# egpbos/barcode

Hardware: AMD Instinct MI355X
Metric: HMC leapfrog steps/sec on 256^3 grid (higher is better)
Workload: dtype f64; 1 GPU; 256^3 grid, L=200 Mpc/h, Gaussian prior, Zel'dovich + plane-parallel RSD (reference behaviour of '2LPT+RSD', SURVEY M3), likelihood=1, mass kernel mk=3 (3 = SPH), calc_h=2, mass_type=1, fp64; one trajectory of 817 leapfrog steps per chain; grid=256, chains=1, parallelism=independent chains, 1 per GPU, rehearsal_single_device=False, steps_done=817, finite=True

## Files before the change

barcode_amd/csrc/bchmc.hip:

```cpp
#include "../../include/bchmc.h"
#include "kernels.hpp"
#include "fft_host.hpp"
#include "owned.hpp"
#include "pass_launch.hpp"
#include "launch_grid.hpp"
#include "eval_plan.hpp"
#include "interp_plan.hpp"

#include <rocfft/rocfft.h>
#include <rocprofiler-sdk-roctx/roctx.h>

#include <algorithm>
#include <chrono>
#include <cmath>
#include <cfloat>
#include <cstdarg>
#include <cstdio>
#include <cstdlib>
#include <climits>
#include <cstring>
#include <mutex>
#include <string>
#include <thread>
#include <type_traits>
#include <vector>

using namespace bchmc;
using namespace owned;

namespace {

struct ProfRec {
  int cls;
  Event a, b;
};

}

struct bchmc_handle {
  bchmc_config c{};
  Geo g{};
  bool f32 = false;
  size_t esz = 8;
  int mass_fs = 0, mass_rs = 0;
  PathSwitches sw;
  bool no_tiles_low = false;
  std::string err;
  RocfftUser fft_user;
  Stream stream;

  DevBytes work;
  FftInfo info;
  FftPlan r2c1, c2r1, r2c3, c2r3;

  DevBytes in_arr[6];
  bool have[6] = {false, false, false, false, false, false};
  DevBuf<double> wS, wM;

  DevBytes qk, pk, gk;
  DevBytes qk2, pk2;
  DevBytes Ck;
  bool ck_pair = false;
  DevBytes tC;
  DevBytes psi;
  DevBytes V;
  DevBytes vrec;
  bool ck_vpair = false;
  bool vrec_eval = false;
  bool v_in_vrec = false;
  DevBytes rho, plike;
  DevBuf<long long> rho_fix;
  DevBuf<int> fix_sat;
  long long fix_sat_limit = 1ll << 62;
  bool fix = false;
  DevBytes ioq, iop;
  DevBytes gprior, glike;
  DevBytes conv;
  DevBuf<double> convF;
  DevBuf<double> dstage;
  DevBytes cq, cp;
  DevBuf<double> part6;
  bool have_cq = false, have_cp = false, have_prop = false;
  DevBytes cg;
  bool cg_valid = false, prop_g_valid = false;
  double c_like = 0., prop_like = 0.;
  DevBuf<double> rho_part, partA;
  DevBuf<double> guard;
  DevBuf<int> stop;
  DevBuf<unsigned long long> steps_done;
  PinnedBuf<double> h_part;
  struct MtDraw {
    long long S = 0, C = 0, G = 0;
    int B = 0;
    DevBuf<uint32_t> poly, win, words, st;
    DevBuf<unsigned long long> nz, nzoff, acc, accoff, lastend;
    DevBuf<unsigned long long> res;
    PinnedBuf<unsigned long long> h_io;
    DevBuf<double> gauss;
    double setup_ms = 0.;
  } mt;
  struct Mock {
    DevBuf<unsigned long long> cnt, off, gsum, goff, res;
  } mock;
  DevBuf<double> spec_bins;
  DevBytes cross_ak;
  struct Ens {
    struct Slot {
      uint64_t count = 0;
      DevBuf<double> mean, m2;
    } slot[BCHMC_ENS_SLOTS];
    int ncu = 0;
  } ens;
  struct Tweb {
    DevBytes t[6];
    DevBytes xk;
    DevBuf<unsigned char> type;
    DevBuf<double> lam;
    DevBuf<unsigned long long> part;
    DevBuf<unsigned int> cnt;
    bool have_t = false;
    uint64_t samples = 0;
    bool have_par = false;
    double R = 0., lambda_th = 0.;
  } tw;
  struct Bispec {
    DevBytes d[kBispecMaxShell];
    DevBytes xk;
    DevBuf<double> part;
    DevBuf<double> tab;
    bool have_tab = false;
    double k_min = 0., dk = 0.;
    int n_shell = 0;
  } bs;
  struct Corr1 {
    uint64_t n_bin = 0;
    DevBuf<unsigned long long> acc;
    std::vector<double> rmode;
    std::vector<uint64_t> nmode;
  } corr1;
  struct Corr2 {
    uint64_t n_bin = 0;
    int n = 0;
    double l_max = 0.;
    DevBuf<int> idx;
    DevBuf<int2> slices;
    DevBuf<double> part;
    DevBuf<double> out;
    int nrows = 0, nsl = 0, npb = 0, max_rows = 0;
    std::vector<uint64_t> row_cnt, par_cnt;
    std::vector<int> par_bin;
    std::vector<double> rsum;
  } corr2;
  struct Spec2 {
    uint64_t n_bin = 0;
    DevBuf<int> idx;
    DevBuf<int2> slices;
    DevBuf<double> part;
    DevBuf<double> out;
    int nsl = 0, npb = 0;
    std::vector<uint64_t> row_cnt, par_w;
    std::vector<int> par_bin;
    std::vector<double> ksum;
  } spec2;
  struct Mp {
    DevBuf<int> rows;
    DevBuf<int4> cls;
    DevBuf<double> part;
    DevBuf<double> out;
    DevBytes xk;
    int ncls = 0;
    struct Geom {
      uint64_t n_bin = 0;
      std::vector<double> tmode, leg;
      std::vector<uint64_t> nmode;
    } fourier, real;
  } mp;
  struct Upres {
    int n_out = 0;
    Geo g{};
    DevBytes real, half;
    DevBytes work;
    FftInfo info;
    FftPlan r2c, c2r;
    DevBuf<int> cell;
    DevBuf<double> dx;
    Corr2 bins;
  } up;
  struct Cat {
    DevBuf<double> cols;
    DevBuf<int> tile_of;
    DevBuf<CatRec> rec;
    DevBuf<unsigned> cnt, off, cursor;
    DevBuf<CatItem> items;
    DevBuf<unsigned long long> stat;
    PinnedBuf<unsigned long long> h_stat;
  } cat;
  struct Pois {
    DevBuf<unsigned long long> off;
    DevBuf<unsigned long long> cnt, boff, gsum, goff;
    DevBuf<unsigned long long> res, stat;
    DevBuf<double> cols;
    long long cells = 0;
    bool valid = false;
    uint64_t seed = 0, n_part = 0;
    uint32_t stream = 0, n_in = 0;
    double d_in = 0.;
  } pois;
  struct Itp {
    DevBytes src;
    int fields_held = 0;
    DevBuf<double> cols;
    DevBuf<double> out;
    DevBuf<int> tile_of;
// ... 273 lines not shown
  h->sorted_valid = false;
}

int realloc_slots(bchmc_handle *h, long long want) {
  HIPCHK(hipStreamSynchronize(h->stream));
  SlotPolicy &sl = h->plan.slots;
  const bool verbose = env_on("BCHMC_VERBOSE");
  const long long cap = sl.clamp_to_budget(want);
  if (!cap) {
    if (verbose) fprintf(stderr, "bchmc: record slots stay at %lld per tile (memory budget %lld): overflowing evaluations "
                                 "run the two-pass sort\n", sl.cap_alloc, sl.cap_budget);
    sl.after_realloc(SlotGot::kOldSize, cap);
    return BCHMC_OK;
  }
  (void)h->srec.release();
  h->sorted_valid = false;
  for (SlotGot got : {SlotGot::kWanted, SlotGot::kOldSize, SlotGot::kRecordsOnly}) {
    const size_t nrec = record_count(h->g.N, sl.rung(got, cap), h->plan.tp.ntiles);
    if (h->srec.alloc(nrec * 4 * h->esz) == hipSuccess) {
      if (got == SlotGot::kWanted) {
        if (verbose) fprintf(stderr, "bchmc: record array reallocated for %lld slots per tile\n", cap);
      } else {
        if (verbose) fprintf(stderr, "bchmc: no memory for %lld record slots per tile: %s\n", cap,
                             got == SlotGot::kOldSize ? "kept the old size, overflowing steps run the two-pass sort"
                                                      : "one-pass binning given up");
      }
      sl.after_realloc(got, cap);
      return BCHMC_OK;
    }
    (void)hipGetLastError();
  }
  return h->fail(BCHMC_ERR_NOMEM, "no device memory for the particle records");
}

int adapt_slots(bchmc_handle *h, int sticky, int maxc, bool may_realloc) {
  if (!h->plan.tiled) return BCHMC_OK;
  SlotPolicy &sl = h->plan.slots;
  const int old = sl.cap;
  const SlotAction a = sl.observe(sticky, maxc, may_realloc);
  if (a.kind == SlotAction::kRealloc) CHK(realloc_slots(h, a.cap));
  if (sl.cap == old) return BCHMC_OK;
  if (env_on("BCHMC_VERBOSE"))
    fprintf(stderr, "bchmc: record slots per tile %d -> %lld (largest (tile, octant) population %d%s)\n", old,
            (long long)sl.cap, maxc, a.overflowed ? ", a segment overflowed" : "");
  repartition(h);
  return BCHMC_OK;
}

int read_ctl(bchmc_handle *h, unsigned long long *steps_done) {
  unsigned long long sd = 0;
  int words[2] = {0, 0}, sat = 0;
  const bool slots = h->plan.tiled && h->plan.slots.sort_direct;
  if (steps_done) HIPCHK(hipMemcpyAsync(&sd, h->steps_done, sizeof sd, hipMemcpyDeviceToHost, h->stream));
  if (h->fix_sat) HIPCHK(hipMemcpyAsync(&sat, h->fix_sat, sizeof(int), hipMemcpyDeviceToHost, h->stream));
  if (slots) HIPCHK(hipMemcpyAsync(words, slot_words(h), sizeof words, hipMemcpyDeviceToHost, h->stream));
  HIPCHK(hipStreamSynchronize(h->stream));
  if (steps_done) *steps_done = sd;
  if (slots) {
    if (words[0] || words[1]) HIPCHK(hipMemsetAsync(slot_words(h), 0, sizeof words, h->stream));
    if (const long long want = h->plan.slots.pending()) {
      CHK(realloc_slots(h, want));
      repartition(h);
    }
    CHK(adapt_slots(h, words[0], words[1], true));
  }
  if (sat) {
    HIPCHK(hipMemsetAsync(h->fix_sat, 0, sizeof(int), h->stream));
    return h->fail(BCHMC_ERR_STATE,
                   "deterministic mode: a density cell exceeded the fixed-point range (more than 2^16 maximal "
                   "contributions in one cell); the results since the last read-back are not valid");
  }
  return BCHMC_OK;
}

constexpr uint64_t kSlotPoll = 4;
int poll_slots(bchmc_handle *h, uint64_t k) {
  if (!h->h_slots) {
    HIPCHK(h->h_slots.alloc(4));
    for (Event &e : h->slot_ev) HIPCHK(e.create(hipEventDisableTiming));
  }
  if (k >= 2) {
    const int b = (int)((k - 1) & 1);
    HIPCHK(hipEventSynchronize(h->slot_ev[b]));
    CHK(adapt_slots(h, h->h_slots[2 * b], h->h_slots[2 * b + 1], false));
  }
  const int b = (int)(k & 1);
  HIPCHK(hipMemcpyAsync(h->h_slots + 2 * b, slot_words(h), 2 * sizeof(int), hipMemcpyDeviceToHost, h->stream));
  HIPCHK(hipMemsetAsync(slot_words(h), 0, 2 * sizeof(int), h->stream));
  HIPCHK(hipEventRecord(h->slot_ev[b], h->stream));
  return BCHMC_OK;
}

int make_plans_2d(bchmc_handle *h, size_t batch, FftPlan &r2c, FftPlan &c2r) {
  const Geo &g = h->g;
  const rocfft_precision prec = h->f32 ? rocfft_precision_single : rocfft_precision_double;
  const size_t len2[2] = {(size_t)g.n, (size_t)g.n};
  const size_t rs2[2] = {1, (size_t)g.n}, cs2[2] = {1, (size_t)g.nhp};
  rocfft_plan_description f2 = nullptr, i2 = nullptr;
  bool ok2 = rocfft_plan_description_create(&f2) == rocfft_status_success &&
             rocfft_plan_description_create(&i2) == rocfft_status_success;
  ok2 = ok2 && rocfft_plan_description_set_data_layout(f2, rocfft_array_type_real, rocfft_array_type_hermitian_interleaved,
                                                       nullptr, nullptr, 2, rs2, (size_t)g.n * g.n, 2, cs2,
                                                       (size_t)g.n * g.nhp) == rocfft_status_success;
  ok2 = ok2 && rocfft_plan_description_set_data_layout(i2, rocfft_array_type_hermitian_interleaved, rocfft_array_type_real,
                                                       nullptr, nullptr, 2, cs2, (size_t)g.n * g.nhp, 2, rs2,
                                                       (size_t)g.n * g.n) == rocfft_status_success;
  ok2 = ok2 && r2c.create(rocfft_plan_create, rocfft_placement_notinplace, rocfft_transform_type_real_forward, prec, 2,
                          len2, batch, f2) == rocfft_status_success;
  ok2 = ok2 && c2r.create(rocfft_plan_create, rocfft_placement_notinplace, rocfft_transform_type_real_inverse, prec, 2,
                          len2, batch, i2) == rocfft_status_success;
  if (f2) rocfft_plan_description_destroy(f2);
  if (i2) rocfft_plan_description_destroy(i2);
  if (ok2 && h->info) {
    size_t need = 0;
    for (const FftPlan *p : {&r2c, &c2r}) {
      size_t wb = 0;
      if (rocfft_plan_get_work_buffer_size(*p, &wb) != rocfft_status_success) ok2 = false;
      need = std::max(need, wb);
    }
    if (ok2 && need > h->work.capacity()) {
      DevBytes nw;
      (void)hipStreamSynchronize(h->stream);
      if (nw.alloc(need) == hipSuccess &&
          rocfft_execution_info_set_work_buffer(h->info, nw, need) == rocfft_status_success) {
        h->work = std::move(nw);
      } else {
        (void)hipGetLastError();
        ok2 = false;
      }
    }
  }
  if (!ok2) {
    r2c.reset();
    c2r.reset();
    return BCHMC_ERR_ROCFFT;
  }
  return BCHMC_OK;
}

PathSwitches read_path_switches() {
  PathSwitches s;
  s.no_planes = env_on("BCHMC_NO_PLANES");
  s.no_planes_ends = env_on("BCHMC_NO_PLANES_ENDS");
  s.no_fuse = env_on("BCHMC_NO_FUSE");
  s.no_alpt_planes = env_on("BCHMC_NO_ALPT_PLANES");
  s.no_zbin = env_on("BCHMC_NO_ZBIN");
  s.zbin_128 = env_on("BCHMC_ZBIN_128");
  s.yfwd_f64 = env_on("BCHMC_YFWD_F64");
  s.bx_v1 = env_on("BCHMC_BX_V1");
  s.bx_v2 = env_on("BCHMC_BX_V2");
  s.no_pair = env_on("BCHMC_NO_PAIR");
  s.no_vpair = env_on("BCHMC_NO_VPAIR");
  s.no_vrec = env_on("BCHMC_NO_VREC");
  return s;
}

PathFacts path_facts(bchmc_handle *h, int rsd) {
  PathFacts f;
  f.n = h->g.n, f.esz = (int)h->esz, f.Nhp = h->g.Nhp;
  f.planes_ok = h->planes_ok && h->xtw;
  f.tiled = h->plan.tiled, f.sort_direct = h->plan.slots.sort_direct, f.std81 = h->plan.std81;
  f.mk = h->c.mk, f.calc_h = h->c.calc_h, f.likelihood = h->c.likelihood, f.sfmodel = h->c.sfmodel;
  f.rsd_model = h->c.rsd_model, f.mass_rs = h->mass_rs != 0;
  if (alpt_planes_wanted(f, h->sw, rsd) && !h->c2r2d_2 && !h->alpt_plans_failed &&
      make_plans_2d(h, 2 * (size_t)h->g.n, h->r2c2d_2, h->c2r2d_2) != BCHMC_OK)
    h->alpt_plans_failed = true;
  f.alpt_plans = h->c2r2d_2 != nullptr;
  return f;
}

int host_sum(bchmc_handle *h, const double *d_part, double *out) {
  HIPCHK(hipMemcpyAsync(h->h_part, d_part, kRedBlocks * sizeof(double), hipMemcpyDeviceToHost, h->stream));
  HIPCHK(hipStreamSynchronize(h->stream));
  double s = 0.;
  for (int i = 0; i < kRedBlocks; i++) s += h->h_part[i];
  *out = s;
  return BCHMC_OK;
}

void par_memcpy(void *dst, const void *src, size_t bytes, int nt) {
  if (nt <= 1 || bytes < ((size_t)4 << 20)) {
    std::memcpy(dst, src, bytes);
    return;
  }
  std::vector<std::thread> th;
  const size_t per = ((bytes / (size_t)nt) + 4095) & ~(size_t)4095;
  for (int t = 1; t < nt; t++) {
    const size_t off = per * (size_t)t;
    if (off >= bytes) break;
    const size_t len = std::min(per, bytes - off);
    th.emplace_back([=] { std::memcpy((char *)dst + off, (const char *)src + off, len); });
  }
  std::memcpy(dst, src, std::min(per, bytes));
  for (auto &t : th) t.join();
}

int stg_init(bchmc_handle *h) {
  if (h->stg[0]) return BCHMC_OK;
  size_t chunk = (size_t)16 << 20;
  if (const char *ev = std::getenv("BCHMC_STAGE_MB")) chunk = (size_t)std::max(1, atoi(ev)) << 20;
  int nt = (int)std::min(8u, std::max(1u, std::thread::hardware_concurrency() / 2));
  if (const char *ev = std::getenv("BCHMC_STAGE_THREADS")) nt = std::max(1, atoi(ev));
  for (int b = 0; b < 2; b++) {
    HIPCHK(h->stg[b].alloc(chunk));
    HIPCHK(h->stg_ev[b].create(hipEventDisableTiming));
  }
  h->stg_chunk = chunk;
  h->stg_threads = nt;
  return BCHMC_OK;
}

int h2d(bchmc_handle *h, void *dst, const void *src, size_t bytes, hipStream_t stream = nullptr) {
  if (!stream) stream = h->stream;
  if (bytes <= ((size_t)1 << 20)) {
    HIPCHK(hipMemcpyAsync(dst, src, bytes, hipMemcpyHostToDevice, stream));
    HIPCHK(hipStreamSynchronize(stream));
    return BCHMC_OK;
  }
  CHK(stg_init(h));
  const size_t chunk = h->stg_chunk;
  const size_t nch = (bytes + chunk - 1) / chunk;
  for (size_t c = 0; c < nch; c++) {
    const int b = (int)(c & 1);
    const size_t off = c * chunk, len = std::min(chunk, bytes - off);
    if (c >= 2) HIPCHK(hipEventSynchronize(h->stg_ev[b]));
    par_memcpy(h->stg[b], (const char *)src + off, len, h->stg_threads);
    HIPCHK(hipMemcpyAsync((char *)dst + off, h->stg[b], len, hipMemcpyHostToDevice, stream));
    HIPCHK(hipEventRecord(h->stg_ev[b], stream));
  }
  HIPCHK(hipEventSynchronize(h->stg_ev[0]));
  if (nch > 1) HIPCHK(hipEventSynchronize(h->stg_ev[1]));
  return BCHMC_OK;
}

int d2h(bchmc_handle *h, void *dst, const void *src, size_t bytes, hipStream_t stream = nullptr,
        hipEvent_t after = nullptr) {
  if (!stream) stream = h->stream;
  if (after) HIPCHK(hipStreamWaitEvent(stream, after, 0));
  if (bytes <= ((size_t)1 << 20)) {
    HIPCHK(hipMemcpyAsync(dst, src, bytes, hipMemcpyDeviceToHost, stream));
    HIPCHK(hipStreamSynchronize(stream));
    return BCHMC_OK;
  }
  CHK(stg_init(h));
  const size_t chunk = h->stg_chunk;
  const size_t nch = (bytes + chunk - 1) / chunk;
  for (size_t c = 0; c <= nch; c++) {
    const int b = (int)(c & 1);
    if (c < nch) {
      const size_t off = c * chunk, len = std::min(chunk, bytes - off);
      HIPCHK(hipMemcpyAsync(h->stg[b], (const char *)src + off, len, hipMemcpyDeviceToHost, stream));
      HIPCHK(hipEventRecord(h->stg_ev[b], stream));
    }
    if (c >= 1) {
      const size_t off = (c - 1) * chunk, len = std::min(chunk, bytes - off);
      HIPCHK(hipEventSynchronize(h->stg_ev[b ^ 1]));
      par_memcpy((char *)dst + off, h->stg[b ^ 1], len, h->stg_threads);
    }
  }
  return BCHMC_OK;
}

int build_conv_table(bchmc_handle *h) {
  const Geo &g = h->g;
  const double hh = h->c.particle_kernel_h;
  const double norm = (24. / (hh * hh * hh)) * (h->c.rho_c * g.L * g.L * g.L / (double)((size_t)g.n * g.n * g.n));
  std::vector<double> F((size_t)g.Nhp);
  auto kv = [&](int i) { return (i <= g.n / 2) ? g.kfac * (double)i : -g.kfac * (double)(g.n - i); };
  for (int i = 0; i < g.n; ++i) {
    const double kx = kv(i);
    for (int j = 0; j < g.n; ++j) {
      const double ky = kv(j);
      for (int k = 0; k < g.nh; ++k) {
        const double kz = kv(k);
        const double k_sq = kx * kx + ky * ky + kz * kz;
        double f;
        if (k_sq == 0.) {
          f = 1. / (hh * hh * hh);
        } else {
          const double kk = std::sqrt(k_sq);
          const double ksink = kk * std::sin(kk);
          f = norm * (3 + std::cos(2 * kk) - ksink + std::cos(kk) * (ksink - 4)) / (k_sq * k_sq * k_sq);
        }
        F[k + (size_t)g.nhp * (j + (size_t)g.n * i)] = f;
      }
    }
  }
  CHK(dev_alloc(h, h->convF, (size_t)g.Nhp));
  HIPCHK(hipMemcpyAsync(h->convF, F.data(), F.size() * sizeof(double), hipMemcpyHostToDevice, h->stream));
  HIPCHK(hipStreamSynchronize(h->stream));
  return BCHMC_OK;
}

double spectrum_dk(const Geo &g, uint64_t n_bin) {
  const double knyq = g.kfac * (double)(g.n / 2);
  const double kmax = std::sqrt(knyq * knyq + knyq * knyq + knyq * knyq);
  return kmax / (double)n_bin;
}

int spectrum_bins(bchmc_handle *h, const void *xk, uint64_t n_bin, double *kmode, double *power) {
  CHK(dev_reserve(h, h->spec_bins, 3 * (size_t)n_bin));
  double *bins = h->spec_bins;
  HIPCHK(hipMemsetAsync(bins, 0, 3 * (size_t)n_bin * sizeof(double), h->stream));
  const Geo &g = h->g;
  const double dk = spectrum_dk(g, n_bin);
  const int grid = std::min(nblk_stride(g.Nhp), 512);
  if (h->f32)
    k_spectrum<float><<<grid, 256, 3 * n_bin * sizeof(double), h->stream>>>(
        g, reinterpret_cast<const float2 *>(xk), (int)n_bin, dk, bins);
  else
    k_spectrum<double><<<grid, 256, 3 * n_bin * sizeof(double), h->stream>>>(
        g, reinterpret_cast<const double2 *>(xk), (int)n_bin, dk, bins);
  std::vector<double> hb(3 * n_bin);
  hipError_t e = hipGetLastError();
  if (e == hipSuccess) e = hipMemcpyAsync(hb.data(), bins, hb.size() * sizeof(double), hipMemcpyDeviceToHost, h->stream);
  if (e == hipSuccess) e = hipStreamSynchronize(h->stream);
// ... 706 lines not shown
      }
      if (h->c.likelihood == 1) {
        CHK(ensure_conv(h));
        CHK(fft_exec(h, h->r2c1, h->ioq, h->tC, BCHMC_K_FFT_R2C));
        {
          ProfScope ps(h, BCHMC_K_OTHER);
          k_gradfft_mult<T><<<nblk_stride(Nh), 256, 0, h->stream>>>(h->g, C(h->tC), C(h->Ck), 1. / (double)N);
          HIPCHK(hipGetLastError());
        }
        CHK(fft_exec(h, h->c2r3, h->Ck, h->conv, BCHMC_K_FFT_C2R));
        ProfScope ps(h, BCHMC_K_OTHER);
        k_mul3<T><<<nblk_stride(N), 256, 0, h->stream>>>(N, R(h->plike), R(h->conv), R(h->V));
        HIPCHK(hipGetLastError());
      } else {
        ProfScope ps(h, BCHMC_K_OTHER);
        k_findif_mul<T><<<nblk_stride(N), 256, 0, h->stream>>>(h->g, make_like(h), R(h->ioq), R(h->plike), R(h->V));
        HIPCHK(hipGetLastError());
      }
      if (transform) CHK(fft_exec(h, h->r2c3, h->V, h->Ck, BCHMC_K_FFT_R2C));
      *like_mode = 0;
      return BCHMC_OK;
    }
    if (h->c.calc_h == 3) {
      if (h->last_rsd && !h->c.planepar)
        return h->fail(BCHMC_ERR_RSD_NOT_PLANEPAR, "non-plane-parallel RSD is not implemented in calc_V");
      CHK(ensure_conv(h));
      if (!h->convF) CHK(build_conv_table(h));
      CHK(fft_exec(h, h->r2c1, h->plike, h->tC, BCHMC_K_FFT_R2C));
      const double hh = h->c.particle_kernel_h;
      {
        ProfScope ps(h, BCHMC_K_OTHER);
        k_conv_kernel<T><<<nblk_stride(Nh), 256, 0, h->stream>>>(h->g, C(h->tC), h->convF, C(h->Ck), hh, 1. / (double)N);
        HIPCHK(hipGetLastError());
      }
      CHK(fft_exec(h, h->c2r3, h->Ck, h->conv, BCHMC_K_FFT_C2R));
      {
        ProfScope ps(h, BCHMC_K_GATHER);
        if (h->plan.tiled && h->sorted_valid && !h->no_tiles_low) {
          const int grid = tile_grid(h);
          const size_t lds = 3 * (size_t)(h->plan.tp.tx + 2) * (h->plan.tp.ty + 2) * (h->plan.tp.tz + 2) * sizeof(T);
          k_interp_tsc_tile<T><<<grid, 256, lds, h->stream>>>(h->g, h->plan.tp, h->last_rsd, fgrow1(h->c.ascale, h->c.OM, h->c.OL),
                                                              recs(h), h->t_off, h->t_end, h->t_woff,
                                                              h->t_oct, h->t_seg, R(h->conv), R(h->V));
        } else {
          k_interp_tsc<T><<<nblk_full(N), 256, 0, h->stream>>>(h->g, make_pos(h, h->last_rsd),
                                                               fgrow1(h->c.ascale, h->c.OM, h->c.OL), R(h->psi),
                                                               R(h->conv), R(h->V));
        }
        HIPCHK(hipGetLastError());
      }
    } else {
      ProfScope ps(h, BCHMC_K_GATHER);
      HullPar hp = make_hull(h);
      if (h->plan.tiled && h->sorted_valid) {
        const int grid = tile_grid(h);
        if (h->plan.std81 && vrec) {
          k_gather_tile81<T, 12, 20, true><<<grid, kTile81Threads, tile_lds(h, 0, sizeof(T)), h->stream>>>(
              h->g, hp, h->plan.tp, h->last_rsd, recs(h), h->t_off, h->t_end, h->t_woff,
              h->t_oct, h->t_seg, R(h->plike), R(h->vrec));
          h->v_in_vrec = true;
        } else if (h->plan.std81)
          k_gather_tile81<T, 12, 20><<<grid, kTile81Threads, tile_lds(h, 0, sizeof(T)), h->stream>>>(
              h->g, hp, h->plan.tp, h->last_rsd, recs(h), h->t_off, h->t_end, h->t_woff,
              h->t_oct, h->t_seg, R(h->plike), R(h->V));
        else
          k_gather_tile<T><<<grid, 256, tile_lds(h, hp.ncol, sizeof(T)), h->stream>>>(
              h->g, hp, h->plan.tp, h->last_rsd, recs(h), h->t_off, h->t_end, h->t_woff,
              h->t_oct, h->t_seg, R(h->plike), R(h->V));
      } else {
        k_gather_sph<T><<<nblk_full(N), 256, hp.ncol * sizeof(int4), h->stream>>>(h->g, make_pos(h, h->last_rsd), hp,
                                                                                  R(h->psi), R(h->plike), R(h->V));
      }
      HIPCHK(hipGetLastError());
      if (vrec && !h->v_in_vrec) return h->fail(BCHMC_ERR_STATE, "V records were zeroed and no gather writes records");
    }
    const bool vpair = eval_vpair(path_facts(h, h->c.rsd_model), h->sw, m);
    if (transform && h->v_in_vrec && !vpair)
      return h->fail(BCHMC_ERR_STATE, "V was gathered as records, and a transform that reads three arrays");
    if (!transform) {
    } else if (vpair) {
      ProfScope ps(h, BCHMC_K_FFT_R2C);
      if (h->v_in_vrec) HIPCHK((launch_zr2c<T, true>(pass_ctx(h), R(h->vrec), C(h->Ck))));
      else HIPCHK(launch_zr2c<T>(pass_ctx(h), R(h->V), C(h->Ck)));
      HIPCHK(launch_ypass_fwd_pair<T>(pass_ctx(h), C(h->Ck)));
      h->ck_vpair = true;
    } else if (eval_yfwd(path_facts(h, h->c.rsd_model), h->sw, m)) {
      ProfScope ps(h, BCHMC_K_FFT_R2C);
      HIPCHK(launch_zr2c<T>(pass_ctx(h), R(h->V), C(h->Ck)));
      HIPCHK((launch_ypass<T, false>(pass_ctx(h), C(h->Ck))));
    } else {
      CHK(fft_exec(h, m.planes_r2c ? h->r2c2d : h->r2c3, h->V, h->Ck, BCHMC_K_FFT_R2C));
    }
    *like_mode = 0;
    return BCHMC_OK;
  }

  static int grf_force(bchmc_handle *h) {
    {
      ProfScope ps(h, BCHMC_K_OTHER);
      k_scale_c<T><<<nblk_stride(h->g.Nhp), 256, 0, h->stream>>>(h->g.Nhp, C(h->qk), C(h->tC), 1. / (double)h->g.N);
      HIPCHK(hipGetLastError());
    }
    CHK(fft_exec(h, h->c2r1, h->tC, h->plike, BCHMC_K_FFT_C2R));
    {
      ProfScope ps(h, BCHMC_K_OTHER);
      k_grf_grad<T><<<nblk_stride(h->g.N), 256, 0, h->stream>>>(h->g.N, R(h->plike), R(h->in_arr[BCHMC_F_NOBS]),
                                                                R(h->in_arr[BCHMC_F_NOISE]),
                                                                R(h->in_arr[BCHMC_F_WINDOW]), R(h->rho));
      HIPCHK(hipGetLastError());
    }
    CHK(fft_exec(h, h->r2c1, h->rho, h->Ck, BCHMC_K_FFT_R2C));
    h->have_eval = false;
    return BCHMC_OK;
  }

  static int force_sources(bchmc_handle *h, bool pre_za, EvalMode m, int *like_mode, double *b) {
    if (h->c.likelihood == 3) {
      CHK(grf_force(h));
      *like_mode = 1;
      *b = h->c.grad_psi_likeli_factor;
      return BCHMC_OK;
    }
    if (!pre_za) {
      CHK(displacement(h, h->c.deltaQ_factor, h->c.rsd_model, &m.planes_c2r));
    } else if (m.alpt_pending) {
      CHK(alpt_middle(h, true));
      m.planes_c2r = true;
    }
    CHK(forward_rest(h, h->c.rsd_model, m));
    CHK(like_force(h, m, like_mode));
    double norm = -1.;
    norm *= h->c.deltaQ_factor;
    if (h->c.correct_delta) norm *= h->c.D1;
    *b = h->c.grad_psi_likeli_factor * norm;
    return BCHMC_OK;
  }

  template <bool KICK>
  static int launch_assemble(bchmc_handle *h, double a, double b, int like_mode, double c_kick, double *guard_slot) {
    h->prop_g_valid = false;
    if (h->ck_vpair) return h->fail(BCHMC_ERR_STATE, "two arrays of V^ in Ck, and a kernel that reads three");
    ProfScope ps(h, BCHMC_K_KSPACE_FORCE_KICK);
    k_assemble<T, KICK><<<nblk_stride(h->g.Nhp), 256, 0, h->stream>>>(h->g, C(h->Ck), C(h->qk), h->wS, C(h->gk), C(h->pk),
                                                                     a, b, like_mode, c_kick, guard_slot, h->stop);
    HIPCHK(hipGetLastError());
    return BCHMC_OK;
  }

  static int r2c_state(bchmc_handle *h, const double *d_real, void *staging, void *out) {
    CHK(load_real(h, d_real, R(staging)));
    return fft_exec(h, h->r2c1, staging, out, BCHMC_K_FFT_R2C);
  }

  static int c2r_scaled(bchmc_handle *h, const void *xk, void *out_T) {
    {
      ProfScope ps(h, BCHMC_K_OTHER);
      k_scale_c<T><<<nblk_stride(h->g.Nhp), 256, 0, h->stream>>>(h->g.Nhp, reinterpret_cast<const CT *>(xk), C(h->tC),
                                                                1. / (double)h->g.N);
      HIPCHK(hipGetLastError());
    }
    return fft_exec(h, h->c2r1, h->tC, out_T, BCHMC_K_FFT_C2R);
  }

  static int c2r_state(bchmc_handle *h, const void *xk, void *scratch_T, double *d_out) {
    if (kDouble) return c2r_scaled(h, xk, d_out);
    CHK(c2r_scaled(h, xk, scratch_T));
    return store_real(h, R(scratch_T), d_out);
  }

  static int mass_rs_term(bchmc_handle *h) {
    CHK(c2r_scaled(h, h->pk, h->iop));
    {
      ProfScope ps(h, BCHMC_K_OTHER);
      k_div_mass_r<T><<<nblk_stride(h->g.N), 256, 0, h->stream>>>(h->g.N, R(h->iop), R(h->in_arr[BCHMC_F_MASS_R]),
                                                                  R(h->iop));
      HIPCHK(hipGetLastError());
    }
    return fft_exec(h, h->r2c1, h->iop, h->tC, BCHMC_K_FFT_R2C);
  }

  struct Tap {
    double *like_i, *like_f;
  };

  static int tap_loglike(bchmc_handle *h, double *partials) {
    k_loglike<T><<<kRedBlocks, 256, 0, h->stream>>>(h->g, make_like(h), R(h->rho), h->rho_part,
                                                    R(h->in_arr[BCHMC_F_NOBS]), R(h->in_arr[BCHMC_F_NOISE]),
                                                    R(h->in_arr[BCHMC_F_WINDOW]), partials);
    HIPCHK(hipGetLastError());
    return BCHMC_OK;
  }

  struct Traj {
    PathFacts f;
    TrajPlan p;
    double a, c_za;
    bool pair;
  };
  static Traj traj(bchmc_handle *h) {
    Traj t;
    t.f = path_facts(h, h->c.rsd_model);
    t.p = traj_plan(t.f, h->sw);
    t.a = h->c.grad_psi_prior_factor;
    t.c_za = (t.p.c_za == CZa::kAlptInput ? 1. : -h->c.D1) * h->c.deltaQ_factor / (double)h->g.N;
    t.pair = psi_pair(t.f, h->sw, t.p);
    return t;
  }

  template <int MODE, bool ALPT = false>
  static int launch_boundary_x(bchmc_handle *h, BoundaryX<T> bx) {
    if (MODE != BX_FIRST) {
      if (ALPT && h->ck_vpair) return h->fail(BCHMC_ERR_STATE, "two arrays of V^ in Ck, and a boundary that reads three");
      bx.vpair = h->ck_vpair;
      h->ck_vpair = false;
    }
    HIPCHK((launch_step_boundary_x<T, MODE, ALPT>(pass_ctx(h), C(h->Ck), h->wS, bx)));
    h->ck_pair = bx.pair && !ALPT && MODE != BX_LAST;
    return BCHMC_OK;
  }

  static int initial_force(bchmc_handle *h, const Traj &t, double *like_i, void *g0_out) {
    int like_mode = 2;
    double b = 0.;
    const InitialEval kind = initial_eval(t.f, h->sw, t.p);
    if (kind == InitialEval::k3d) {
      CHK(force_sources(h, false, EvalMode{}, &like_mode, &b));
      if (like_i) CHK(tap_loglike(h, like_i));
      CHK(launch_assemble<false>(h, t.a, b, like_mode, 0., nullptr));
    } else {
      StepCtl nc{h->stop, h->steps_done, nullptr, 0., 0};
      {
        ProfScope ps(h, BCHMC_K_KSPACE_DRIFT_ZA);
        BoundaryX<T> bx;
        bx.qi = C(h->qk), bx.c_za = t.c_za, bx.ctl = nc, bx.pair = t.pair;
        if (kind == InitialEval::kBxFirstAlpt) CHK((launch_boundary_x<BX_FIRST, true>(h, bx)));
        else CHK(launch_boundary_x<BX_FIRST>(h, bx));
      }
      EvalMode m;
      m.planes_c2r = m.planes_r2c = true;
      m.alpt_pending = t.p.alpt_x;
      CHK(force_sources(h, true, m, &like_mode, &b));
      if (like_mode != 0) return h->fail(BCHMC_ERR_STATE, "planes mode without the three V components");
      if (like_i) CHK(tap_loglike(h, like_i));
      h->prop_g_valid = false;
      ProfScope ps(h, BCHMC_K_KSPACE_FORCE_KICK);
      BoundaryX<T> bx;
      bx.qi = C(h->qk), bx.a = t.a, bx.b = b, bx.ctl = nc, bx.g_out = C(h->gk);
      CHK(launch_boundary_x<BX_LAST>(h, bx));
    }
    if (g0_out)
      HIPCHK(hipMemcpyAsync(g0_out, h->gk, 2 * (size_t)h->g.Nhp * sizeof(T), hipMemcpyDeviceToDevice, h->stream));
    return BCHMC_OK;
  }

  static int trajectory(bchmc_handle *h, double eps, uint64_t neps, const Tap *tap, const void *g0_in = nullptr,
                        void *g0_out = nullptr) {
    h->prop_g_valid = false;
    if (neps + 1 > h->guard.capacity())
      CHK(dev_reserve(h, h->guard, std::max<size_t>(4096, 2 * (neps + 1))));
    HIPCHK(hipMemsetAsync(h->guard, 0, (neps + 1) * sizeof(double), h->stream));
    k_init_ctl<<<1, 1, 0, h->stream>>>(h->stop, h->steps_done, (unsigned long long)neps);
    HIPCHK(hipGetLastError());

    const Traj t = traj(h);
    int like_mode = 2;
    double b = 0.;
    if (!g0_in) CHK(initial_force(h, t, tap ? tap->like_i : nullptr, g0_out));
    const void *g_first = g0_in ? g0_in : h->gk;
    if (neps == 0) return BCHMC_OK;

    if (t.p.fused) return trajectory_fused(h, eps, neps, tap, t, g_first);
    const double *wM = h->mass_fs ? h->wM : nullptr;
    const double guard_limit = 1e50 * (double)h->g.N;
    for (uint64_t s = 0; s < neps; s++) {
      StepCtl ctl{h->stop, h->steps_done, s > 0 ? h->guard + (s - 1) : nullptr, guard_limit, s};
      if (!h->mass_rs) {
        ProfScope ps(h, BCHMC_K_KSPACE_DRIFT_ZA);
        k_kick_drift_za<T, true><<<nblk_stride(h->g.Nhp), 256, 0, h->stream>>>(
            h->g, C(h->qk), C(h->pk), C(s == 0 ? g_first : h->gk), wM, nullptr, C(h->Ck), 0.5 * eps, eps, t.c_za, ctl);
        HIPCHK(hipGetLastError());
      } else {
        {
          ProfScope ps(h, BCHMC_K_KSPACE_DRIFT_ZA);
          k_kick_drift_za<T, true><<<nblk_stride(h->g.Nhp), 256, 0, h->stream>>>(
              h->g, C(h->qk), C(h->pk), C(s == 0 ? g_first : h->gk), nullptr, nullptr, C(h->Ck), 0.5 * eps, 0., t.c_za,
              ctl);
          HIPCHK(hipGetLastError());
        }
        CHK(mass_rs_term(h));
        StepCtl ctl2{h->stop, h->steps_done, nullptr, 0., s};
        ProfScope ps(h, BCHMC_K_KSPACE_DRIFT_ZA);
        k_kick_drift_za<T, true><<<nblk_stride(h->g.Nhp), 256, 0, h->stream>>>(h->g, C(h->qk), C(h->pk), C(h->gk), wM,
                                                                             C(h->tC), C(h->Ck), 0., eps, t.c_za, ctl2);
        HIPCHK(hipGetLastError());
      }
      CHK(force_sources(h, t.p.fused_za, EvalMode{}, &like_mode, &b));
      if (tap && tap->like_f && s + 1 == neps) CHK(tap_loglike(h, tap->like_f));
      CHK(launch_assemble<true>(h, t.a, b, like_mode, 0.5 * eps, h->guard + s));
    }
    return BCHMC_OK;
  }

  static int trajectory_fused(bchmc_handle *h, double eps, uint64_t neps, const Tap *tap, const Traj &t,
                              const void *g_first) {
    const double *wM = h->mass_fs ? h->wM : nullptr;
    const double guard_limit = 1e50 * (double)h->g.N, a = t.a, c_za = t.c_za;
    if (!h->qk2) {
      CHK(dev_alloc(h, h->qk2, 2 * (size_t)h->g.Nhp * sizeof(T)));
      CHK(dev_alloc(h, h->pk2, 2 * (size_t)h->g.Nhp * sizeof(T)));
    }
    void *const q0 = h->qk, *const p0 = h->pk, *const q1 = h->qk2, *const p1 = h->pk2;
    int like_mode = 2;
    double b = 0.;
    int cur = 0;
    {
      StepCtl ctl{h->stop, h->steps_done, nullptr, guard_limit, 0};
      ProfScope ps(h, BCHMC_K_KSPACE_DRIFT_ZA);
      BoundaryX<T> bx;
      bx.qi = bx.qo = C(q0), bx.pi = bx.po = C(p0), bx.wM = wM, bx.half_eps = 0.5 * eps, bx.eps = eps, bx.c_za = c_za;
      bx.ctl = ctl, bx.g_in = C(g_first), bx.pair = t.pair;
      switch (opening(t.f, h->sw, t.p)) {
        case Opening::kBxFirstAlpt: CHK((launch_boundary_x<BX_FIRST, true>(h, bx))); break;
        case Opening::kBxFirst: CHK(launch_boundary_x<BX_FIRST>(h, bx)); break;
        case Opening::kKickDriftZa:
          h->ck_pair = false;
          k_kick_drift_za<T, true><<<nblk_stride(h->g.Nhp), 256, 0, h->stream>>>(h->g, C(q0), C(p0), C(g_first), wM,
                                                                               nullptr, C(h->Ck), 0.5 * eps, eps, c_za, ctl);
          break;
      }
      HIPCHK(hipGetLastError());
    }
    for (uint64_t s = 0; s < neps; s++) {
      const bool last = (s + 1 == neps);
      if (last && h->early_q_dev && h->ev_q) {
        CHK(c2r_state(h, cur ? q1 : q0, h->ioq, h->early_q_dev));
        HIPCHK(hipEventRecord(h->ev_q, h->stream));
        h->early_q_done = true;
      }
      if (h->plan.slots.slot_watch && h->plan.tiled && h->plan.slots.sort_direct && s > 0 && s % kSlotPoll == 0)
        CHK(poll_slots(h, s / kSlotPoll));
      CHK(force_sources(h, true, step_mode(t.f, h->sw, t.p, s, neps), &like_mode, &b));
      if (tap && tap->like_f && last) CHK(tap_loglike(h, tap->like_f));
      StepCtl ctl{h->stop, h->steps_done, s > 0 ? h->guard + (s - 1) : nullptr, guard_limit, s};
      void *qi = cur ? q1 : q0, *pi = cur ? p1 : p0, *qo = cur ? q0 : q1, *po = cur ? p0 : p1;
      ProfScope ps(h, BCHMC_K_KSPACE_FORCE_KICK);
      BoundaryX<T> bx;
      bx.qi = C(qi), bx.pi = C(pi), bx.qo = C(qo), bx.po = C(po), bx.wM = wM, bx.a = a, bx.b = b, bx.half_eps = 0.5 * eps;
      bx.eps = eps, bx.c_za = c_za, bx.guard_slot = h->guard + s, bx.ctl = ctl, bx.pair = t.pair;
      switch (closing(t.f, h->sw, t.p, s, neps, like_mode)) {
        case Closing::kBxLast:
          bx.qo = nullptr, bx.po = C(pi), bx.g_out = C(h->gk);
          CHK(launch_boundary_x<BX_LAST>(h, bx));
          break;
        case Closing::kStepBoundaryLast:
          if (h->ck_vpair) return h->fail(BCHMC_ERR_STATE, "two arrays of V^ in Ck, and a boundary that reads three");
          k_step_boundary<T, true><<<nblk_stride(h->g.Nhp), 256, 0, h->stream>>>(
              h->g, C(h->Ck), C(qi), C(pi), C(qi), C(pi), C(h->gk), h->wS, wM, a, b, like_mode, 0.5 * eps, eps, c_za,
              h->guard + s, ctl);
          break;
        case Closing::kBxInteriorAlpt: CHK((launch_boundary_x<BX_INTERIOR, true>(h, bx))); break;
        case Closing::kBxInterior: CHK(launch_boundary_x<BX_INTERIOR>(h, bx)); break;
        case Closing::kBxInteriorTwoTile:
          bx.vpair = h->ck_vpair;
          h->ck_vpair = false;
          HIPCHK(launch_step_boundary_x2<T>(pass_ctx(h), C(h->Ck), h->wS, bx));
          h->ck_pair = bx.pair;
          break;
        case Closing::kStepBoundary:
          if (h->ck_vpair) return h->fail(BCHMC_ERR_STATE, "two arrays of V^ in Ck, and a boundary that reads three");
          k_step_boundary<T, false><<<nblk_stride(h->g.Nhp), 256, 0, h->stream>>>(
              h->g, C(h->Ck), C(qi), C(pi), C(qo), C(po), C(h->gk), h->wS, wM, a, b, like_mode, 0.5 * eps, eps, c_za,
              h->guard + s, ctl);
          break;
      }
      if (buffers_flip(s, neps)) cur ^= 1;
      HIPCHK(hipGetLastError());
    }
    {
      ProfScope ps(h, BCHMC_K_OTHER);
      k_rollback<T><<<nblk_stride(h->g.Nhp), 256, 0, h->stream>>>(h->g.Nhp, h->stop, h->steps_done, C(q0), C(p0), C(q1),
                                                                 C(p1), C(cur ? q1 : q0), C(cur ? p1 : p0));
      HIPCHK(hipGetLastError());
    }
    if (cur) {
      std::swap(h->qk, h->qk2);
      std::swap(h->pk, h->pk2);
    }
    return BCHMC_OK;
  }

  static int leapfrog_core(bchmc_handle *h, const double *d_q0, const double *d_p0, double *d_q1, double *d_p1,
                           double eps, uint64_t neps, bool prologue_done = false) {
    CHK(check_inputs(h));
    if (eps > 2.) eps = 2.;
    if (!prologue_done) CHK(r2c_state(h, d_q0, h->ioq, h->qk));
    CHK(r2c_state(h, d_p0, h->iop, h->pk));
    CHK(trajectory(h, eps, neps, nullptr, prologue_done ? h->gk : nullptr));
    if (!h->early_q_done) CHK(c2r_state(h, h->qk, h->ioq, d_q1));
    CHK(c2r_state(h, h->pk, h->iop, d_p1));
    return BCHMC_OK;
  }
  static int requeue_q(bchmc_handle *h, double *d_q1) { return c2r_state(h, h->qk, h->ioq, d_q1); }

  static int chain_alloc(bchmc_handle *h) {
    if (!h->cq) {
      CHK(dev_alloc(h, h->cq, 2 * (size_t)h->g.Nhp * sizeof(T)));
      CHK(dev_alloc(h, h->cp, 2 * (size_t)h->g.Nhp * sizeof(T)));
      CHK(dev_alloc(h, h->part6, (size_t)6 * kRedBlocks));
    }
    return BCHMC_OK;
  }

  static int chain_draw(bchmc_handle *h, uint64_t seed, uint64_t attempt) {
    const long long N = h->g.N, Nh = h->g.Nhp;
    const uint2 key = make_uint2((unsigned)seed, (unsigned)(seed >> 32));
    ProfScope ps(h, BCHMC_K_OTHER);
    if (h->mass_fs) {
      k_white_noise<T><<<nblk_stride((N + 1) / 2), 256, 0, h->stream>>>(N, key, (unsigned)attempt, 0u, nullptr, R(h->iop));
      HIPCHK(hipGetLastError());
      CHK(fft_exec(h, h->r2c1, h->iop, h->tC, BCHMC_K_FFT_R2C));
      k_color_momenta<T><<<nblk_stride(Nh), 256, 0, h->stream>>>(Nh, C(h->tC), h->wM, C(h->cp), 0);
      HIPCHK(hipGetLastError());
    } else {
      HIPCHK(hipMemsetAsync(h->cp, 0, 2 * (size_t)Nh * sizeof(T), h->stream));
    }
    if (h->mass_rs) {
      k_white_noise<T><<<nblk_stride((N + 1) / 2), 256, 0, h->stream>>>(N, key, (unsigned)attempt, 1u,
                                                                        R(h->in_arr[BCHMC_F_MASS_R]), R(h->iop));
      HIPCHK(hipGetLastError());
      CHK(fft_exec(h, h->r2c1, h->iop, h->tC, BCHMC_K_FFT_R2C));
      k_color_momenta<T><<<nblk_stride(Nh), 256, 0, h->stream>>>(Nh, C(h->tC), nullptr, C(h->cp), 1);
      HIPCHK(hipGetLastError());
    }
    return BCHMC_OK;
  }

  static bool attempt_is_fast(const bchmc_handle *h, uint64_t neps) {
    const bool like_shared = h->c.likelihood == 1 || ((h->c.likelihood == 0 || h->c.likelihood == 2) &&
                                                       h->c.deltaQ_factor == 1. && !h->c.rsd_model);
    return like_shared && !h->mass_rs && neps >= 1;
  }

  static int attempt_core(bchmc_handle *h, double eps, uint64_t neps, const double *d_q0, const double *d_p0,
                          const void *src_qk, const void *src_pk, double terms[6], uint64_t *steps_done,
                          const void *g0_in = nullptr, double like0 = 0., void *g0_out = nullptr, bool g0_ready = false,
                          double *host_q1 = nullptr) {
    CHK(check_inputs(h));
    if (eps > 2.) eps = 2.;
    const size_t cbytes = 2 * (size_t)h->g.Nhp * sizeof(T);
    const double N = (double)h->g.N;
    const bool fast = attempt_is_fast(h, neps);
    if (!h->part6) CHK(dev_alloc(h, h->part6, (size_t)6 * kRedBlocks));
    double *P = h->part6;
    if (!fast) {
      CHK(energies_core(h, d_q0, d_p0, terms));
      if (src_qk) {
        HIPCHK(hipMemcpyAsync(h->qk, src_qk, cbytes, hipMemcpyDeviceToDevice, h->stream));
        HIPCHK(hipMemcpyAsync(h->pk, src_pk, cbytes, hipMemcpyDeviceToDevice, h->stream));
      }
    } else {
      k_parseval<T><<<kRedBlocks, 256, 0, h->stream>>>(h->g, C(h->pk), h->wM, P);
      k_parseval<T><<<kRedBlocks, 256, 0, h->stream>>>(h->g, C(h->qk), h->wS, P + kRedBlocks);
      HIPCHK(hipGetLastError());
    }
    if (g0_ready && fast) g0_in = h->gk;
    Tap tap{g0_in ? nullptr : P + 2 * kRedBlocks, P + 5 * kRedBlocks};
    if (g0_in && !g0_ready) HIPCHK(hipMemsetAsync(P + 2 * kRedBlocks, 0, kRedBlocks * sizeof(double), h->stream));
    CHK(trajectory(h, eps, neps, fast ? &tap : nullptr, fast ? g0_in : nullptr, fast ? g0_out : nullptr));
    uint64_t done = 0;
    if (fast) {
      k_parseval<T><<<kRedBlocks, 256, 0, h->stream>>>(h->g, C(h->pk), h->wM, P + 3 * kRedBlocks);
      k_parseval<T><<<kRedBlocks, 256, 0, h->stream>>>(h->g, C(h->qk), h->wS, P + 4 * kRedBlocks);
      HIPCHK(hipGetLastError());
      if (host_q1) {
        if (!h->early_q_done) CHK(c2r_state(h, h->qk, h->ioq, h->dstage));
        CHK(c2r_state(h, h->pk, h->iop, h->dstage + h->g.N));
      }
      if (host_q1 && h->early_q_done)
        CHK(d2h(h, host_q1, h->dstage, (size_t)h->g.N * sizeof(double), h->copy_stream, h->ev_q));
      std::vector<double> hp(6 * kRedBlocks);
      unsigned long long sd = 0;
      HIPCHK(hipMemcpyAsync(hp.data(), P, hp.size() * sizeof(double), hipMemcpyDeviceToHost, h->stream));
      CHK(read_ctl(h, &sd));
      done = sd;
      for (int t = 0; t < 6; t++) {
        double s = 0.;
        for (int i = 0; i < kRedBlocks; i++) s += hp[(size_t)t * kRedBlocks + i];
        terms[t] = (t == 0 || t == 1 || t == 3 || t == 4) ? s / (2. * N) : s;
      }
      if (g0_in && !g0_ready) terms[2] = like0;
      if (done < neps) {
        if (host_q1 && h->early_q_done) {
          h->early_q_done = false;
          CHK(c2r_state(h, h->qk, h->ioq, h->dstage));
        }
        EvalMode m;
        CHK(displacement(h, h->c.likelihood == 1 ? h->c.deltaQ_factor : 1., h->c.likelihood == 1 ? h->c.rsd_model : 0,
                         &m.planes_c2r));
        CHK(forward_rest(h, h->c.likelihood == 1 ? h->c.rsd_model : 0, m));
        CHK(tap_loglike(h, P));
        CHK(host_sum(h, P, &terms[5]));
      }
    } else {
      unsigned long long sd = 0;
      CHK(read_ctl(h, &sd));
      done = sd;
      CHK(c2r_state(h, h->qk, h->ioq, h->dstage));
      CHK(c2r_state(h, h->pk, h->iop, h->dstage + h->g.N));
      CHK(energies_core(h, h->dstage, h->dstage + h->g.N, terms + 3));
    }
    if (steps_done) *steps_done = done;
    return BCHMC_OK;
  }

  static int chain_attempt(bchmc_handle *h, double eps, uint64_t neps, double terms[6], uint64_t *steps_done) {
    const size_t cbytes = 2 * (size_t)h->g.Nhp * sizeof(T);
    if (attempt_is_fast(h, neps)) {
      HIPCHK(hipMemcpyAsync(h->qk, h->cq, cbytes, hipMemcpyDeviceToDevice, h->stream));
      HIPCHK(hipMemcpyAsync(h->pk, h->cp, cbytes, hipMemcpyDeviceToDevice, h->stream));
      const bool use = !env_on("BCHMC_NO_FORCE_CARRY"), carry = use && h->cg_valid;
      if (use && !h->cg) CHK(dev_alloc(h, h->cg, cbytes));
      uint64_t done = 0;
      CHK(attempt_core(h, eps, neps, nullptr, nullptr, nullptr, nullptr, terms, &done, carry ? h->cg : nullptr,
                       h->c_like, (use && !carry) ? h->cg : nullptr));
      if (steps_done) *steps_done = done;
      if (use && !carry) {
        h->cg_valid = true;
        h->c_like = terms[2];
      }
      h->prop_g_valid = use && done == neps;
      h->prop_like = terms[5];
    } else {
      h->cg_valid = h->prop_g_valid = false;
      CHK(c2r_state(h, h->cq, h->ioq, h->dstage));
      CHK(c2r_state(h, h->cp, h->iop, h->dstage + h->g.N));
      CHK(attempt_core(h, eps, neps, h->dstage, h->dstage + h->g.N, h->cq, h->cp, terms, steps_done));
    }
    h->have_prop = true;
    return BCHMC_OK;
  }
// ... 528 lines not shown
      HIPCHK(hipMemcpyAsync(hs, w.out, cells * 3 * NS * sizeof(double), hipMemcpyDeviceToHost, h->stream));
    }
    HIPCHK(hipStreamSynchronize(h->stream));
    return BCHMC_OK;
  }
  static int mp_auto(bchmc_handle *h, const void *xk, uint64_t n_bin, double *hg, double *hs) {
    return mp_sums<1, false>(h, xk, nullptr, n_bin, hg, hs);
  }
  static int mp_cross(bchmc_handle *h, const void *ak, const void *bk, uint64_t n_bin, double *hg, double *hs) {
    return mp_sums<3, false>(h, ak, bk, n_bin, hg, hs);
  }
  static int mp_corr(bchmc_handle *h, uint64_t n_bin, double *hg, double *hs) {
    return mp_sums<1, true>(h, h->ioq, nullptr, n_bin, hg, hs);
  }

  static int gradient(bchmc_handle *h, const double *d_q, double *d_g) {
    const size_t N = (size_t)h->g.N;
    if (!h->gprior) {
      CHK(dev_alloc(h, h->gprior, N * sizeof(T)));
      CHK(dev_alloc(h, h->glike, N * sizeof(T)));
    }
    CHK(r2c_state(h, d_q, h->ioq, h->qk));
    int like_mode = 2;
    double b = 0.;
    CHK(force_sources(h, false, EvalMode{}, &like_mode, &b));
    CHK(launch_assemble<false>(h, h->c.grad_psi_prior_factor, 0., 2, 0., nullptr));
    CHK(c2r_scaled(h, h->gk, h->gprior));
    CHK(launch_assemble<false>(h, 0., b, like_mode, 0., nullptr));
    CHK(c2r_scaled(h, h->gk, h->glike));
    k_add_r<T><<<nblk_stride(h->g.N), 256, 0, h->stream>>>(h->g.N, R(h->gprior), R(h->glike), R(h->iop));
    HIPCHK(hipGetLastError());
    return store_real(h, R(h->iop), d_g);
  }

  static int fetch(bchmc_handle *h, bchmc_field field, double *d_out) {
    FieldSource fs;
    CHK(field_source(h, (int)field, &fs));
    if (fs.made == FieldSource::kOverdens)
      k_overdens<T><<<nblk_stride(h->g.N), 256, 0, h->stream>>>(h->g, R(h->rho), h->rho_part, R(h->ioq));
    if (fs.made == FieldSource::kPositions)
      k_positions<T><<<nblk_stride(h->g.N), 256, 0, h->stream>>>(h->g, make_pos(h, h->last_rsd), R(h->psi), R(h->ioq),
                                                                 (int)field - (int)BCHMC_F_POSX);
    if (fs.made == FieldSource::kVrec)
      k_vrec_unpack<T><<<nblk_stride(h->g.N), 256, 0, h->stream>>>(h->g.N, R(h->vrec), (int)field - (int)BCHMC_F_VX, R(h->ioq));
    if (fs.made != FieldSource::kAsHeld) HIPCHK(hipGetLastError());
    return store_real(h, R(fs.base) + fs.offset, d_out);
  }

  static int mt_place(bchmc_handle *h) {
    const long long N = h->g.N, Nh = h->g.Nhp;
    const int n = h->g.n;
    ProfScope ps(h, BCHMC_K_OTHER);
    HIPCHK(hipMemsetAsync(h->cp, 0, 2 * (size_t)Nh * sizeof(T), h->stream));
    if (h->mass_fs) {
      const long long cells = (long long)(n / 2 + 1) * (n / 2 + 1) * (n / 2 + 1);
      const double amp = (double)N * (double)N / (h->g.L * h->g.L * h->g.L);
      k_mt_place<T><<<nblk_stride(cells), 256, 0, h->stream>>>(n, h->g.nhp, h->mt.gauss, R(h->in_arr[BCHMC_F_MASS_F]),
                                                               amp, C(h->cp));
      HIPCHK(hipGetLastError());
    }
    if (h->mass_rs) {
      k_mt_real_space<T><<<nblk_stride(N), 256, 0, h->stream>>>(N, h->mt.gauss + (h->mass_fs ? 2 * N : 0),
                                                                R(h->in_arr[BCHMC_F_MASS_R]), R(h->iop));
      HIPCHK(hipGetLastError());
      CHK(fft_exec(h, h->r2c1, h->iop, h->tC, BCHMC_K_FFT_R2C));
      k_color_momenta<T><<<nblk_stride(Nh), 256, 0, h->stream>>>(Nh, C(h->tC), nullptr, C(h->cp), 1);
      HIPCHK(hipGetLastError());
    }
    return BCHMC_OK;
  }

  static int mock_place(bchmc_handle *h, void *dst) {
    const long long N = h->g.N;
    const int n = h->g.n;
    ProfScope ps(h, BCHMC_K_OTHER);
    HIPCHK(hipMemsetAsync(dst, 0, 2 * (size_t)h->g.Nhp * sizeof(T), h->stream));
    const long long cells = (long long)(n / 2 + 1) * (n / 2 + 1) * (n / 2 + 1);
    const double amp = (double)N * (double)N / (h->g.L * h->g.L * h->g.L);
    k_mt_place<T><<<nblk_stride(cells), 256, 0, h->stream>>>(n, h->g.nhp, h->mt.gauss, R(h->in_arr[BCHMC_F_SIGNAL_PS]),
                                                             amp, C(dst));
    HIPCHK(hipGetLastError());
    return BCHMC_OK;
  }

  static long long mock_tiles(const bchmc_handle *h) { return (h->g.N + kMockTile - 1) / kMockTile; }
  static long long mock_groups(const bchmc_handle *h) { return (mock_tiles(h) + kMtThreads - 1) / kMtThreads; }

  static int mock_alloc(bchmc_handle *h) {
    auto &k = h->mock;
    if (k.cnt) return BCHMC_OK;
    CHK(dev_alloc(h, k.cnt, (size_t)mock_tiles(h)));
    CHK(dev_alloc(h, k.off, (size_t)mock_tiles(h)));
    CHK(dev_alloc(h, k.gsum, (size_t)mock_groups(h)));
    CHK(dev_alloc(h, k.goff, (size_t)mock_groups(h)));
    CHK(dev_alloc(h, k.res, (size_t)2));
    return BCHMC_OK;
  }

  static int mock_window(bchmc_handle *h, int rsd, int window_type) {
    const long long N = h->g.N;
    auto &k = h->mock;
    CHK(c2r_state(h, h->qk, h->ioq, h->dstage));
    EvalMode m;
    CHK(displacement(h, 1., rsd, &m.planes_c2r));
    CHK(forward_rest(h, rsd, m));
    CHK(fetch(h, BCHMC_F_DELTAX, h->dstage + N));
    ProfScope ps(h, BCHMC_K_OTHER);
    HIPCHK(hipMemsetAsync(k.res, 0xff, 2 * sizeof(unsigned long long), h->stream));
    k_mock_window<T><<<(int)mock_tiles(h), kMockThreads, 0, h->stream>>>(N, window_type, h->dstage + N,
                                                                         R(h->in_arr[BCHMC_F_WINDOW]), k.cnt);
    k_mock_scan<<<(int)mock_groups(h), kMtThreads, 0, h->stream>>>(k.cnt, mock_tiles(h), k.off, k.gsum);
    k_mt_scan<<<1, kMtThreads, 0, h->stream>>>(k.gsum, (int)mock_groups(h), k.goff, k.res, 0, nullptr);
    HIPCHK(hipGetLastError());
    return BCHMC_OK;
  }

  static int mock_noise(bchmc_handle *h, const MockPar &mp) {
    const long long N = h->g.N;
    auto &k = h->mock;
    ProfScope ps(h, BCHMC_K_OTHER);
    k_mock_noise<T><<<(int)mock_tiles(h), kMockThreads, 0, h->stream>>>(
        N, mp, h->dstage, h->dstage + N, R(h->in_arr[BCHMC_F_WINDOW]), k.off, k.goff,
        reinterpret_cast<const double2 *>(h->mt.gauss.get()), R(h->in_arr[BCHMC_F_NOBS]), R(h->in_arr[BCHMC_F_NOISE]), k.res);
    HIPCHK(hipGetLastError());
    return BCHMC_OK;
  }

  static int mock_smooth(bchmc_handle *h, double smol) {
    double wtot = 0.;
    CHK(kernel_norm(h, smol, h->ioq, &wtot));
    ProfScope ps(h, BCHMC_K_OTHER);
    k_mock_smooth<T><<<nblk_stride(h->g.Nhp), 256, 0, h->stream>>>(h->g, C(h->cq), smol, 1. / wtot);
    HIPCHK(hipGetLastError());
    return BCHMC_OK;
  }

  static int mock_guess_noise(bchmc_handle *h, double sigma) {
    {
      ProfScope ps(h, BCHMC_K_OTHER);
      k_mock_guess_noise<<<nblk_stride(h->g.N), kMockThreads, 0, h->stream>>>(
          h->g.N, sigma, reinterpret_cast<const double2 *>(h->mt.gauss.get()), h->dstage);
      HIPCHK(hipGetLastError());
    }
    return r2c_state(h, h->dstage, h->ioq, h->cq);
  }

  static int upload(bchmc_handle *h, bchmc_field field, const double *d_src) {
    CHK(load_real(h, d_src, R(h->in_arr[field])));
    const double normFS = h->g.L * h->g.L * h->g.L / (double)h->g.N;
    if (field == BCHMC_F_SIGNAL_PS || field == BCHMC_F_MASS_F) {
      double *w = field == BCHMC_F_SIGNAL_PS ? h->wS : h->wM;
      k_prepare_mult<<<nblk_stride(h->g.Nhp), 256, 0, h->stream>>>(h->g, d_src, w, normFS);
      HIPCHK(hipGetLastError());
    }
    return BCHMC_OK;
  }

  static int mass_force_spectrum(bchmc_handle *h, uint64_t n_bin, double *kmode, double *power) {
    int like_mode = 2;
    double b = 0.;
    CHK(force_sources(h, false, EvalMode{}, &like_mode, &b));
    double norm = -1.;
    norm *= h->c.deltaQ_factor;
    if (h->c.correct_delta) norm *= h->c.D1;
    CHK(launch_assemble<false>(h, 0., norm, like_mode, 0., nullptr));
    return spectrum_bins(h, h->gk, n_bin, kmode, power);
  }

  static constexpr long long kJascheWork = 1ll << 32;

  static int mass_jasche(bchmc_handle *h, double *d_r) {
    const Geo &g = h->g;
    const long long N = g.N;
    DevBuf<double> G, acc;
    DevBuf<int> cnt, off;
    DevBuf<long long> total;
    DevBuf<JRec> rec;
    struct Drain {
      hipStream_t stream;
      ~Drain() { (void)hipStreamSynchronize(stream); }
    } drain{h->stream};
    CHK(dev_alloc(h, G, 3 * (size_t)N));
    CHK(dev_alloc(h, acc, (size_t)N));
    CHK(dev_alloc(h, cnt, (size_t)N));
    CHK(dev_alloc(h, off, (size_t)N + 1));
    CHK(dev_alloc(h, total, (size_t)1));
    {
      ProfScope ps(h, BCHMC_K_OTHER);
      k_glap_impulse<T><<<nblk_stride(g.Nhp), 256, 0, h->stream>>>(g, C(h->Ck));
      HIPCHK(hipGetLastError());
    }
    CHK(fft_exec(h, h->c2r3, h->Ck, h->psi, BCHMC_K_FFT_C2R));
    {
      ProfScope ps(h, BCHMC_K_OTHER);
      k_convert<T, double><<<nblk_stride(3 * N), 256, 0, h->stream>>>(3 * N, R(h->psi), G);
      HIPCHK(hipGetLastError());
    }
    const int rsd = h->c.rsd_model;
    EvalMode mode;
    CHK(displacement(h, 1., rsd, &mode.planes_c2r));
    CHK(forward_rest(h, rsd, mode));
    const PosPar pp = make_pos(h, rsd);
    JaschePar jp;
    jp.h = h->c.particle_kernel_h;
    const double h2 = jp.h * jp.h;
    jp.norm = 1. / (M_PI * (h2 * h2 * jp.h));
    jp.reach = (int)(2. * jp.h / g.d) + 1;
    const T *window = R(h->in_arr[BCHMC_F_WINDOW]), *noise = R(h->in_arr[BCHMC_F_NOISE]);
    {
      ProfScope ps(h, BCHMC_K_OTHER);
      k_jasche_pairs<T, false><<<nblk_stride(N), 256, 0, h->stream>>>(g, pp, jp, R(h->psi), window, cnt, nullptr, nullptr);
      k_jasche_scan<<<1, 1024, 0, h->stream>>>(N, cnt, total, off);
      HIPCHK(hipGetLastError());
    }
    long long npairs = 0;
    HIPCHK(hipMemcpyAsync(&npairs, total, sizeof npairs, hipMemcpyDeviceToHost, h->stream));
    HIPCHK(hipStreamSynchronize(h->stream));
    if (npairs >= 0x7fffffffLL)
      return h->fail(BCHMC_ERR_UNSUPPORTED, "Jasche mass: %lld (particle, cell) pairs exceed the 32-bit offsets", npairs);
    CHK(dev_alloc(h, rec, (size_t)std::max(npairs, 1ll)));
    HIPCHK(hipMemsetAsync(cnt, 0, (size_t)N * sizeof(int), h->stream));
    {
      ProfScope ps(h, BCHMC_K_OTHER);
      k_jasche_pairs<T, true><<<nblk_stride(N), 256, 0, h->stream>>>(g, pp, jp, R(h->psi), window, cnt, off, rec);
      k_jasche_sort<<<nblk_stride(N), 256, 0, h->stream>>>(N, off, rec);
      HIPCHK(hipGetLastError());
    }
    std::vector<int> hoff((size_t)N + 1);
    HIPCHK(hipMemcpyAsync(hoff.data(), off, hoff.size() * sizeof(int), hipMemcpyDeviceToHost, h->stream));
    HIPCHK(hipStreamSynchronize(h->stream));
    const long long budget = std::max(kJascheWork / N, 1ll);
    for (long long l0 = 0; l0 < N;) {
      long long l1 = l0 + 1;
      while (l1 < N && (long long)(hoff[l1 + 1] - hoff[l0]) + (l1 + 1 - l0) <= budget) l1++;
      ProfScope ps(h, BCHMC_K_OTHER);
      k_jasche_accum<<<nblk_full(N), 256, 0, h->stream>>>(g, rec, off, l0, l1, G, acc);
      HIPCHK(hipGetLastError());
      l0 = l1;
    }
    const double m = h->c.rho_c * (g.L * g.L * g.L) / (double)N;
    ProfScope ps(h, BCHMC_K_OTHER);
    k_jasche_final<T><<<nblk_stride(N), 256, 0, h->stream>>>(N, acc, window, noise, m * m, d_r);
    HIPCHK(hipGetLastError());
    return BCHMC_OK;
  }

  static int mass_build(bchmc_handle *h, bool from_chain, const bchmc_mass_opts &o, bool force, bool jasche) {
    const int t = h->c.mass_type;
    const long long N = h->g.N;
    double *d_f = h->dstage, *d_r = h->dstage + N;
    if (force || jasche) {
      if (from_chain)
        HIPCHK(hipMemcpyAsync(h->qk, h->cq, 2 * (size_t)h->g.Nhp * sizeof(T), hipMemcpyDeviceToDevice, h->stream));
      else
        CHK(r2c_state(h, h->dstage, h->ioq, h->qk));
    }
    double dk = 0., fbar = 0.;
    std::vector<double> kmode, power;
    if (force) {
      kmode.resize(o.n_bin);
      power.resize(o.n_bin);
      CHK(mass_force_spectrum(h, o.n_bin, kmode.data(), power.data()));
      dk = spectrum_dk(h->g, o.n_bin);
      if (t == 3) {
        double fm = 0., kv = 0.;
        for (uint64_t i = 0; i < o.n_bin; i++) fm += 4. * M_PI * kmode[i] * kmode[i] * dk * power[i];
        for (uint64_t i = 0; i < o.n_bin; i++) kv += 4. * M_PI * kmode[i] * kmode[i] * dk;
        fbar = fm / kv;
      } else {
        HIPCHK(hipMemcpyAsync(h->spec_bins, power.data(), o.n_bin * sizeof(double), hipMemcpyHostToDevice, h->stream));
      }
    }
    if (h->mass_fs) {
      const int mode = (t == 1 || t == 5) ? MASS_INVP : t == 2 ? MASS_FORCE : t == 3 ? MASS_MEAN : MASS_PS;
      ProfScope ps(h, BCHMC_K_OTHER);
      k_mass_elementwise<T><<<nblk_stride(N), 256, 0, h->stream>>>(h->g, mode, R(h->in_arr[BCHMC_F_SIGNAL_PS]),
                                                                   h->spec_bins, (int)o.n_bin, dk, fbar, o.mass_factor,
                                                                   d_f);
      HIPCHK(hipGetLastError());
    }
    if (h->mass_rs) {
      if (jasche) {
        CHK(mass_jasche(h, d_r));
      } else {
        ProfScope ps(h, BCHMC_K_OTHER);
        k_mass_elementwise<T><<<nblk_stride(N), 256, 0, h->stream>>>(h->g, MASS_ONE, nullptr, nullptr, 0, 0., 0., 1., d_r);
        HIPCHK(hipGetLastError());
      }
    }
    if (h->mass_fs) CHK(upload(h, BCHMC_F_MASS_F, d_f));
    if (h->mass_rs) CHK(upload(h, BCHMC_F_MASS_R, d_r));
    HIPCHK(hipStreamSynchronize(h->stream));
    return BCHMC_OK;
  }

  static int pois_counts(bchmc_handle *h, int src, long long cells, const double *xd, const bchmc_poisson_opts &o,
                         double *cd, bool resident) {
    auto &k = h->pois;
    if (!xd) CHK(upres_real(h, src));
    const long long nb = (cells + kPoisThreads - 1) / kPoisThreads, ng = (nb + kMtThreads - 1) / kMtThreads;
    const uint2 key = make_uint2((unsigned)o.seed, (unsigned)(o.seed >> 32));
    const T *win = o.use_window ? R(h->in_arr[BCHMC_F_WINDOW]) : nullptr;
    unsigned long long *off = resident ? k.off.get() : nullptr, *cnt = resident ? k.cnt.get() : nullptr;
    ProfScope ps(h, BCHMC_K_OTHER);
    HIPCHK(hipMemsetAsync(k.stat, 0, kPoisWords * sizeof(unsigned long long), h->stream));
    HIPCHK(hipMemsetAsync(k.stat + kPoisBad, 0xff, sizeof(unsigned long long), h->stream));
// ... 2328 lines not shown
```

barcode_amd/csrc/eval_plan.hpp:

```cpp
#pragma once

#include "pass_launch.hpp"

namespace bchmc {

struct PathSwitches {
  bool no_planes = false;
  bool no_planes_ends = false;
  bool no_fuse = false;
  bool no_alpt_planes = false;
  bool no_zbin = false;
  bool zbin_128 = false;
  bool yfwd_f64 = false;
  bool bx_v1 = false;
  bool bx_v2 = false;
  bool no_pair = false;
  bool no_vpair = false;
  bool no_vrec = false;
};

struct PathFacts {
  int n = 0, esz = 8;
  long long Nhp = 0;
  bool planes_ok = false;
  bool tiled = false;
  bool sort_direct = false;
  int mk = 3, calc_h = 2, likelihood = 1, sfmodel = 1, rsd_model = 0;
  bool mass_rs = false;
  bool alpt_plans = false;
  bool std81 = false;
};

struct EvalMode {
  bool planes_c2r = false;
  bool planes_r2c = false;
  bool alpt_pending = false;
  bool psi_unread = false;
};

constexpr bool planes_on(const PathFacts &f, const PathSwitches &s) {
  return f.planes_ok && x_shape(f.esz, f.n).nt && f.calc_h == 2 && f.mk == 3 && !s.no_planes;
}
constexpr bool planes_at_ends(const PathFacts &f, const PathSwitches &s) { return planes_on(f, s) && !s.no_planes_ends; }

constexpr bool uses_alpt(const PathFacts &f, int rsd) { return !rsd && f.sfmodel != 1; }
constexpr bool alpt_planes_wanted(const PathFacts &f, const PathSwitches &s, int rsd) {
  return uses_alpt(f, rsd) && planes_at_ends(f, s) && !s.no_alpt_planes;
}
constexpr bool alpt_on_planes(const PathFacts &f, const PathSwitches &s, int rsd) {
  return alpt_planes_wanted(f, s, rsd) && f.alpt_plans;
}

enum class ZbinWhyNot { kNone, kSwitchedOff, kNeeds128Switch, kGridSize, kNotSphAdjoint, kNoOnePassBinning, kNoPlanes };

constexpr ZbinWhyNot zbin_why_not(const PathFacts &f, const PathSwitches &s) {
  if (s.no_zbin) return ZbinWhyNot::kSwitchedOff;
  if (f.n == 128 && !s.zbin_128) return ZbinWhyNot::kNeeds128Switch;
  if (!z_shape(f.esz, f.n).nt) return ZbinWhyNot::kGridSize;
  if (f.mk != 3 || f.calc_h != 2) return ZbinWhyNot::kNotSphAdjoint;
  if (!f.tiled || !f.sort_direct) return ZbinWhyNot::kNoOnePassBinning;
  if (!f.planes_ok) return ZbinWhyNot::kNoPlanes;
  return ZbinWhyNot::kNone;
}
constexpr const char *zbin_why_not_text(ZbinWhyNot w) {
  switch (w) {
    case ZbinWhyNot::kNone: return nullptr;
    case ZbinWhyNot::kSwitchedOff: return "BCHMC_NO_ZBIN is set";
    case ZbinWhyNot::kNeeds128Switch: return "Nx = 128 takes it with BCHMC_ZBIN_128=1 only";
    case ZbinWhyNot::kGridSize: return "it exists for Nx = 128, 256 and 512";
    case ZbinWhyNot::kNotSphAdjoint: return "it needs masskernel 3 with calc_h 2";
    case ZbinWhyNot::kNoOnePassBinning: return "the one-pass tile binning is not in use";
    case ZbinWhyNot::kNoPlanes: break;
  }
  return "the planes-mode transforms are not available";
}
constexpr bool zbin_ok(const PathFacts &f, const PathSwitches &s) { return zbin_why_not(f, s) == ZbinWhyNot::kNone; }
constexpr bool eval_zbin(const PathFacts &f, const PathSwitches &s, const EvalMode &m) { return m.planes_c2r && zbin_ok(f, s); }

constexpr bool yfwd_ok(const PathFacts &f, const PathSwitches &s) {
  return f.n == 512 && (f.esz == 4 || s.yfwd_f64) && f.planes_ok;
}
constexpr bool eval_yfwd(const PathFacts &f, const PathSwitches &s, const EvalMode &m) { return m.planes_r2c && yfwd_ok(f, s); }

constexpr bool interior_two_tile(const PathFacts &f, const PathSwitches &s) {
  const bool want = (f.esz == 4 && !s.bx_v1) || (f.esz == 8 && f.n <= 256 && s.bx_v2);
  return x2_shape(f.esz, f.n).nt && want && (unsigned long long)f.Nhp * 2 * f.esz < (1ull << 32);
}

enum class CZa {
  kZeldovich,
  kAlptInput
};
struct TrajPlan {
  bool alpt_x = false, fused_za = false, fused = false;
  CZa c_za = CZa::kZeldovich;
};

constexpr bool psi_pair(const PathFacts &f, const PathSwitches &s, const TrajPlan &tp) {
  return !s.no_pair && !tp.alpt_x && planes_on(f, s) && zbin_ok(f, s) && ypair_shape(f.esz, f.n).nt;
}
constexpr TrajPlan traj_plan(const PathFacts &f, const PathSwitches &s) {
  TrajPlan tp;
  const bool alpt = uses_alpt(f, f.rsd_model) && f.likelihood != 3;
  tp.alpt_x = alpt && !f.mass_rs && !s.no_fuse && alpt_on_planes(f, s, f.rsd_model);
  tp.fused_za = f.likelihood != 3 && !alpt;
  tp.c_za = tp.alpt_x ? CZa::kAlptInput : CZa::kZeldovich;
  tp.fused = (tp.fused_za || tp.alpt_x) && !f.mass_rs && !s.no_fuse;
  return tp;
}

constexpr bool v_pair(const PathFacts &f, const PathSwitches &s, const TrajPlan &tp) {
  return !s.no_vpair && !tp.alpt_x && f.n != 512 && planes_on(f, s) && zbin_ok(f, s) && f.std81 &&
         y_shape(f.esz, f.n).nt && z_shape(f.esz, f.n).nt && yfwd_pair_shape(f.esz, f.n).nt;
}
constexpr bool eval_vpair(const PathFacts &f, const PathSwitches &s, const EvalMode &m) {
  return m.planes_r2c && v_pair(f, s, traj_plan(f, s));
}
constexpr bool v_rec(const PathFacts &f, const PathSwitches &s) { return v_pair(f, s, traj_plan(f, s)) && !s.no_vrec; }
constexpr bool eval_vrec(const PathFacts &f, const PathSwitches &s, const EvalMode &m) {
  return eval_vpair(f, s, m) && !s.no_vrec;
}

enum class InitialEval { k3d, kBxFirst, kBxFirstAlpt };
constexpr InitialEval initial_eval(const PathFacts &f, const PathSwitches &s, const TrajPlan &tp) {
  if (!(tp.fused && planes_at_ends(f, s))) return InitialEval::k3d;
  return tp.alpt_x ? InitialEval::kBxFirstAlpt : InitialEval::kBxFirst;
}

enum class Opening { kKickDriftZa, kBxFirst, kBxFirstAlpt };
constexpr Opening opening(const PathFacts &f, const PathSwitches &s, const TrajPlan &tp) {
  if (!planes_at_ends(f, s)) return Opening::kKickDriftZa;
  return tp.alpt_x ? Opening::kBxFirstAlpt : Opening::kBxFirst;
}
constexpr EvalMode step_mode(const PathFacts &f, const PathSwitches &s, const TrajPlan &tp, unsigned long long step,
                             unsigned long long neps) {
  const bool planes = planes_on(f, s), ends = planes_at_ends(f, s), last = step + 1 == neps;
  EvalMode m;
  m.planes_c2r = planes && (step > 0 || ends);
  m.planes_r2c = planes && (!last || ends);
  m.alpt_pending = tp.alpt_x;
  m.psi_unread = !last;
  return m;
}
enum class Closing { kBxLast, kStepBoundaryLast, kBxInterior, kBxInteriorTwoTile, kBxInteriorAlpt, kStepBoundary };
constexpr Closing closing(const PathFacts &f, const PathSwitches &s, const TrajPlan &tp, unsigned long long step,
                          unsigned long long neps, int like_mode) {
  const bool last = step + 1 == neps, xmode = step_mode(f, s, tp, step, neps).planes_r2c && like_mode == 0;
  if (last) return xmode ? Closing::kBxLast : Closing::kStepBoundaryLast;
  if (!xmode) return Closing::kStepBoundary;
  if (tp.alpt_x) return Closing::kBxInteriorAlpt;
  return interior_two_tile(f, s) ? Closing::kBxInteriorTwoTile : Closing::kBxInterior;
}
constexpr bool buffers_flip(unsigned long long step, unsigned long long neps) { return step + 1 != neps; }

}
```

barcode_amd/csrc/fft_probe.hip:

```cpp
#include "kernels.hpp"
#include "fft_host.hpp"
#include "pass_launch.hpp"
#include "launch_grid.hpp"

#include <cmath>
#include <cstring>
#include <vector>

using namespace bchmc;

namespace {

constexpr size_t kCanary = 64 * 1024;
constexpr unsigned char kCanaryByte = 0x5b;

template <typename T, int NT>
__global__ void __launch_bounds__(NT)
k_probe_xfft(int n, int log2n, int kb, int inverse, const C2<T> *__restrict__ twiddle, C2<T> *data) {
  extern __shared__ __attribute__((aligned(16))) unsigned char s_raw_p[];
  C2<T> *s = reinterpret_cast<C2<T> *>(s_raw_p);
  C2<T> *tw = s + (size_t)n * kb;
  for (int t = threadIdx.x; t < n / 2; t += NT) tw[t] = twiddle[t];
  C2<T> *col = data + (long long)blockIdx.x * n * kb;
  const int shift = 32 - log2n;
  for (int e = threadIdx.x; e < n * kb; e += NT) {
    const int i = e / kb, c = e % kb;
    s[(int)(__brev((unsigned)i) >> shift) * kb + c] = col[e];
  }
  __syncthreads();
  xfft_inplace<T>(s, tw, n, log2n, kb, inverse != 0);
  for (int e = threadIdx.x; e < n * kb; e += NT) col[e] = s[e];
}

int ilog2(int n) {
  int l = 0;
  while ((1 << l) < n) l++;
  return (1 << l) == n ? l : -1;
}

struct Probe {
  std::vector<void *> bufs;
  std::vector<size_t> sizes;
  int err = 0;

  ~Probe() {
    for (void *p : bufs) (void)hipFree(p);
  }
  bool ok(hipError_t e) {
    if (e != hipSuccess && !err) err = -2;
    return e == hipSuccess;
  }
  void *alloc(size_t bytes, const void *host) {
    void *d = nullptr;
    if (!ok(hipMalloc(&d, bytes + kCanary))) return nullptr;
    bufs.push_back(d);
    sizes.push_back(bytes);
    ok(hipMemset(static_cast<char *>(d) + bytes, kCanaryByte, kCanary));
    if (host) ok(hipMemcpy(d, host, bytes, hipMemcpyHostToDevice));
    return d;
  }
  int finish(const std::vector<std::pair<int, void *>> &outs) {
    if (err) return err;
    if (!ok(hipGetLastError()) || !ok(hipDeviceSynchronize())) return err;
    for (const auto &o : outs)
      if (!ok(hipMemcpy(o.second, bufs[o.first], sizes[o.first], hipMemcpyDeviceToHost))) return err;
    std::vector<unsigned char> c(kCanary);
    for (size_t i = 0; i < bufs.size(); i++) {
      if (!ok(hipMemcpy(c.data(), static_cast<char *>(bufs[i]) + sizes[i], kCanary, hipMemcpyDeviceToHost))) return err;
      for (unsigned char b : c)
        if (b != kCanaryByte) return (int)i + 1;
    }
    return 0;
  }
  template <typename T> const C2<T> *twiddles(int n) {
    const std::vector<T> tw = fft_twiddles<T>(n);
    return static_cast<const C2<T> *>(alloc(tw.size() * sizeof(T), tw.data()));
  }
  template <typename T> PassCtx<T> ctx(const Geo &g) { return {nullptr, g, ilog2(g.n), twiddles<T>(g.n)}; }
};

Geo probe_geo(int n, int esz, double L = 0.) {
  Geo g;
  g.n = n;
  g.nh = n / 2 + 1;
  g.nhp = fft_row_stride(n, esz);
  g.N = (long long)n * n * n;
  g.Nh = (long long)n * n * g.nh;
  g.Nhp = (long long)n * n * g.nhp;
  g.L = L > 0. ? L : (double)n;
  g.d = g.L / n;
  g.kfac = 2. * M_PI / g.L;
  return g;
}

template <typename T, int NT>
void launch_xfft(Probe &pr, int groups, int n, int kb, int inverse, const C2<T> *tw, C2<T> *d) {
  const size_t lds = ((size_t)n * kb + n / 2) * sizeof(C2<T>);
  pr.ok(launch_dyn_lds(nullptr, k_probe_xfft<T, NT>, groups, NT, lds, n, ilog2(n), kb, inverse, tw, d));
}

template <typename T> int xfft(int n, int kb, int inverse, int groups, void *data) {
  if (ilog2(n) < 5 || n > 512 || groups < 1 || (kb != pass_kb(sizeof(T)) && kb != 6)) return -1;
  const int nt = kb == 6 ? n : x_shape(sizeof(T), n).nt;
  Probe pr;
  const size_t bytes = (size_t)groups * n * kb * sizeof(C2<T>);
  const C2<T> *tw = pr.twiddles<T>(n);
  C2<T> *d = static_cast<C2<T> *>(pr.alloc(bytes, data));
  if (pr.err) return pr.err;
  switch (nt) {
    case 32: launch_xfft<T, 32>(pr, groups, n, kb, inverse, tw, d); break;
    case 64: launch_xfft<T, 64>(pr, groups, n, kb, inverse, tw, d); break;
    case 128: launch_xfft<T, 128>(pr, groups, n, kb, inverse, tw, d); break;
    case 256: launch_xfft<T, 256>(pr, groups, n, kb, inverse, tw, d); break;
    case 512: launch_xfft<T, 512>(pr, groups, n, kb, inverse, tw, d); break;
    case 1024: launch_xfft<T, 1024>(pr, groups, n, kb, inverse, tw, d); break;
    default: return -1;
  }
  return pr.finish({{1, data}});
}

template <typename T> int ypass(int n, int inverse, void *ck) {
  if (!y_shape(sizeof(T), n).nt) return -1;
  const Geo g = probe_geo(n, (int)sizeof(T));
  if (g.nhp % pass_kb(sizeof(T))) return -1;
  Probe pr;
  const PassCtx<T> x = pr.ctx<T>(g);
  C2<T> *d = static_cast<C2<T> *>(pr.alloc((size_t)3 * g.Nhp * sizeof(C2<T>), ck));
  if (pr.err) return pr.err;
  pr.ok(inverse ? launch_ypass<T>(x, d) : launch_ypass<T, false>(x, d));
  return pr.finish({{1, ck}});
}

template <typename T> int ypass_pair(int n, double box_len, void *ck) {
  if (!ypair_shape(sizeof(T), n).nt) return -1;
  const Geo g = probe_geo(n, (int)sizeof(T), box_len);
  if (g.nhp % pass_kb(sizeof(T))) return -1;
  Probe pr;
  const PassCtx<T> x = pr.ctx<T>(g);
  C2<T> *d = static_cast<C2<T> *>(pr.alloc((size_t)3 * g.Nhp * sizeof(C2<T>), ck));
  if (pr.err) return pr.err;
  pr.ok(launch_ypass_pair<T>(x, d));
  return pr.finish({{1, ck}});
}

template <typename T> int ypass_fwd_pair(int n, double box_len, void *ck) {
  if (!yfwd_pair_shape(sizeof(T), n).nt) return -1;
  const Geo g = probe_geo(n, (int)sizeof(T), box_len);
  if (g.nhp % pass_kb(sizeof(T))) return -1;
  Probe pr;
  const PassCtx<T> x = pr.ctx<T>(g);
  C2<T> *d = static_cast<C2<T> *>(pr.alloc((size_t)3 * g.Nhp * sizeof(C2<T>), ck));
  if (pr.err) return pr.err;
  pr.ok(launch_ypass_fwd_pair<T>(x, d));
  return pr.finish({{1, ck}});
}

template <typename T, bool REC = false> int zr2c(int n, const void *V, void *ck) {
  if (!z_shape(sizeof(T), n).nt) return -1;
  const Geo g = probe_geo(n, (int)sizeof(T));
  Probe pr;
  const PassCtx<T> x = pr.ctx<T>(g);
  const T *dv = static_cast<const T *>(pr.alloc((size_t)(REC ? 4 : 3) * g.N * sizeof(T), V));
  C2<T> *dc = static_cast<C2<T> *>(pr.alloc((size_t)3 * g.Nhp * sizeof(C2<T>), ck));
  if (pr.err) return pr.err;
  pr.ok((launch_zr2c<T, REC>(x, dv, dc)));
  return pr.finish({{2, ck}});
}

template <typename T> int zc2r(int n, const void *ck, void *psi) {
  if (!z_shape(sizeof(T), n).nt) return -1;
  const Geo g = probe_geo(n, (int)sizeof(T));
  Probe pr;
  const PassCtx<T> x = pr.ctx<T>(g);
  const C2<T> *dc = static_cast<const C2<T> *>(pr.alloc((size_t)3 * g.Nhp * sizeof(C2<T>), ck));
  const int ovf_h[3] = {1, 0, 0};
  int *ovf = static_cast<int *>(pr.alloc(sizeof(ovf_h), ovf_h));
  T *dp = static_cast<T *>(pr.alloc((size_t)3 * g.N * sizeof(T), nullptr));
  if (pr.err) return pr.err;
  pr.ok((launch_zbin<T, true>(x, PosPar{}, SphPar{}, TilePar{}, dc, nullptr, ovf, nullptr, nullptr, nullptr, nullptr, nullptr,
                              dp, nullptr)));
  return pr.finish({{3, psi}});
}


struct CtlArgs {
  int *stop;
  unsigned long long *steps_done;
  const double *guard_prev;
  double guard_limit;
  unsigned long long step_index;
};
struct CtlDev {
  StepCtl ctl{};
  int i_stop = -1, i_done = -1;
};
CtlDev ctl_alloc(Probe &pr, const CtlArgs &c) {
  CtlDev d;
  d.ctl.stop = static_cast<int *>(pr.alloc(sizeof(int), c.stop));
  d.i_stop = (int)pr.bufs.size() - 1;
  d.ctl.steps_done = static_cast<unsigned long long *>(pr.alloc(sizeof(unsigned long long), c.steps_done));
  d.i_done = (int)pr.bufs.size() - 1;
  d.ctl.guard_prev = c.guard_prev ? static_cast<const double *>(pr.alloc(sizeof(double), c.guard_prev)) : nullptr;
  d.ctl.guard_limit = c.guard_limit;
  d.ctl.step_index = c.step_index;
  return d;
}

template <typename U> U *opt(Probe &pr, size_t bytes, const void *host, int *idx = nullptr) {
  if (!host) return nullptr;
  U *d = static_cast<U *>(pr.alloc(bytes, host));
  if (idx) *idx = (int)pr.bufs.size() - 1;
  return d;
}

using Outs = std::vector<std::pair<int, void *>>;
void out(Outs &o, int idx, void *host) {
  if (host && idx >= 0) o.push_back({idx, host});
}

template <typename T>
int step_boundary_x(int n, double L, int mode, int alpt, int two_tile, void *Ck, const void *q_in, const void *p_in,
                    const void *g_in, void *q_out, void *p_out, void *g_out, const double *wS, const double *wM,
                    const double *scal, double *guard_slot, const CtlArgs &ca, int vpair = 0) {
  if (mode < BX_INTERIOR || mode > BX_LAST || (alpt && mode == BX_LAST)) return -1;
  if (vpair && (alpt || mode == BX_FIRST)) return -1;
  if (two_tile ? (!x2_shape(sizeof(T), n).nt || mode != BX_INTERIOR || alpt) : !x_shape(sizeof(T), n).nt) return -1;
  const Geo g = probe_geo(n, (int)sizeof(T), L);
  if (g.nhp % pass_kb(sizeof(T)) || !Ck || !q_in || !scal) return -1;
  const bool first_kick = mode == BX_FIRST && g_in, last_kick = mode == BX_LAST && p_out;
  if (mode == BX_INTERIOR && !(p_in && q_out && p_out && guard_slot)) return -1;
  if (first_kick && !(p_in && q_out && p_out)) return -1;
  if (mode == BX_LAST && (!g_out || (last_kick && !(p_in && guard_slot)))) return -1;
  if (mode != BX_FIRST && scal[0] != 0. && !wS) return -1;
  Probe pr;
  const PassCtx<T> x = pr.ctx<T>(g);
  const size_t cb = (size_t)g.Nhp * sizeof(C2<T>), db = (size_t)g.Nhp * sizeof(double);
  int i_ck, i_qo = -1, i_po = -1, i_go = -1, i_gs = -1;
  C2<T> *d_ck = opt<C2<T>>(pr, 3 * cb, Ck, &i_ck);
  BoundaryX<T> a;
  a.qi = opt<const C2<T>>(pr, cb, q_in);
  a.pi = opt<const C2<T>>(pr, cb, p_in);
  a.g_in = opt<const C2<T>>(pr, cb, g_in);
  a.qo = opt<C2<T>>(pr, cb, q_out, &i_qo);
  a.po = opt<C2<T>>(pr, cb, p_out, &i_po);
  a.g_out = opt<C2<T>>(pr, cb, g_out, &i_go);
  const double *d_ws = opt<const double>(pr, db, wS);
  a.wM = opt<const double>(pr, db, wM);
  a.a = scal[0], a.b = scal[1], a.half_eps = scal[2], a.eps = scal[3], a.c_za = scal[4];
  a.guard_slot = opt<double>(pr, sizeof(double), guard_slot, &i_gs);
  const CtlDev cd = ctl_alloc(pr, ca);
  a.ctl = cd.ctl;
  a.vpair = vpair != 0;
  if (pr.err) return pr.err;
  hipError_t e = hipErrorInvalidConfiguration;
  if (two_tile) e = launch_step_boundary_x2<T>(x, d_ck, d_ws, a);
  else if (mode == BX_INTERIOR) e = alpt ? launch_step_boundary_x<T, BX_INTERIOR, true>(x, d_ck, d_ws, a)
                                         : launch_step_boundary_x<T, BX_INTERIOR, false>(x, d_ck, d_ws, a);
  else if (mode == BX_FIRST) e = alpt ? launch_step_boundary_x<T, BX_FIRST, true>(x, d_ck, d_ws, a)
                                      : launch_step_boundary_x<T, BX_FIRST, false>(x, d_ck, d_ws, a);
  else e = launch_step_boundary_x<T, BX_LAST, false>(x, d_ck, d_ws, a);
  pr.ok(e);
  Outs o;
  out(o, i_ck, Ck), out(o, i_qo, q_out), out(o, i_po, p_out), out(o, i_go, g_out), out(o, i_gs, guard_slot);
  out(o, cd.i_stop, ca.stop), out(o, cd.i_done, ca.steps_done);
  return pr.finish(o);
}

template <typename T> int alpt_mix_x(int n, double L, void *Ck, double smol, double inv_wtot, double inv_n) {
  if (!x_shape(sizeof(T), n).nt) return -1;
  const Geo g = probe_geo(n, (int)sizeof(T), L);
  if (g.nhp % pass_kb(sizeof(T))) return -1;
  Probe pr;
  const PassCtx<T> x = pr.ctx<T>(g);
  C2<T> *d = static_cast<C2<T> *>(pr.alloc((size_t)3 * g.Nhp * sizeof(C2<T>), Ck));
  if (pr.err) return pr.err;
  pr.ok(launch_alpt_mix_x<T>(x, d, smol, inv_wtot, inv_n));
  return pr.finish({{1, Ck}});
}

bool ok3d(int n) { return n >= 2 && n <= 512; }

template <typename T>
int kick_drift_za(int n, double L, int drift, void *qk, void *pk, const void *gk, const double *wM, const void *extra,
                  void *Ck, const double *scal, const CtlArgs &ca) {
  if (!ok3d(n) || !qk || !Ck || !scal || (drift && !(pk && gk))) return -1;
  const Geo g = probe_geo(n, (int)sizeof(T), L);
  Probe pr;
  const size_t cb = (size_t)g.Nhp * sizeof(C2<T>);
  int i_q, i_p = -1, i_ck;
  C2<T> *dq = opt<C2<T>>(pr, cb, qk, &i_q), *dp = opt<C2<T>>(pr, cb, pk, &i_p);
  const C2<T> *dg = opt<const C2<T>>(pr, cb, gk);
  const double *dw = opt<const double>(pr, (size_t)g.Nhp * sizeof(double), wM);
  const C2<T> *dx = opt<const C2<T>>(pr, cb, extra);
  C2<T> *dc = opt<C2<T>>(pr, 3 * cb, Ck, &i_ck);
  const CtlDev cd = ctl_alloc(pr, ca);
  if (pr.err) return pr.err;
  if (drift)
    k_kick_drift_za<T, true><<<nblk_stride(g.Nhp), 256>>>(g, dq, dp, dg, dw, dx, dc, scal[0], scal[1], scal[2], cd.ctl);
  else
    k_kick_drift_za<T, false><<<nblk_stride(g.Nhp), 256>>>(g, dq, dp, dg, dw, dx, dc, scal[0], scal[1], scal[2], cd.ctl);
  Outs o;
  out(o, i_q, qk), out(o, i_p, pk), out(o, i_ck, Ck), out(o, cd.i_stop, ca.stop), out(o, cd.i_done, ca.steps_done);
  return pr.finish(o);
}

template <typename T>
int assemble(int n, double L, int kick, const void *Ck, const void *qk, const double *wS, void *gk, void *pk,
             const double *scal, int like_mode, double *guard_slot, int *stop) {
  if (!ok3d(n) || !Ck || !gk || !scal || like_mode < 0 || like_mode > 2 || (scal[0] != 0. && !(qk && wS))) return -1;
  if (kick && !(pk && guard_slot && stop)) return -1;
  const Geo g = probe_geo(n, (int)sizeof(T), L);
  Probe pr;
  const size_t cb = (size_t)g.Nhp * sizeof(C2<T>);
  int i_g, i_p = -1, i_gs = -1;
  const C2<T> *dc = opt<const C2<T>>(pr, 3 * cb, Ck), *dq = opt<const C2<T>>(pr, cb, qk);
  const double *dw = opt<const double>(pr, (size_t)g.Nhp * sizeof(double), wS);
  C2<T> *dg = opt<C2<T>>(pr, cb, gk, &i_g), *dp = opt<C2<T>>(pr, cb, pk, &i_p);
  double *dgs = opt<double>(pr, sizeof(double), guard_slot, &i_gs);
  const int *ds = opt<const int>(pr, sizeof(int), stop);
  if (pr.err) return pr.err;
  if (kick)
    k_assemble<T, true><<<nblk_stride(g.Nhp), 256>>>(g, dc, dq, dw, dg, dp, scal[0], scal[1], like_mode, scal[2], dgs, ds);
  else
    k_assemble<T, false><<<nblk_stride(g.Nhp), 256>>>(g, dc, dq, dw, dg, dp, scal[0], scal[1], like_mode, scal[2], dgs, ds);
  Outs o;
  out(o, i_g, gk), out(o, i_p, pk), out(o, i_gs, guard_slot);
  return pr.finish(o);
}

template <typename T>
int step_boundary(int n, double L, int last, void *Ck, const void *q_in, const void *p_in, void *q_out, void *p_out,
                  void *gk, const double *wS, const double *wM, const double *scal, int like_mode, double *guard_slot,
                  const CtlArgs &ca) {
  if (!ok3d(n) || !Ck || !q_in || !p_in || !p_out || !scal || !guard_slot || like_mode < 0 || like_mode > 2) return -1;
  if ((last && !gk) || (!last && !q_out) || (scal[0] != 0. && !wS)) return -1;
  const Geo g = probe_geo(n, (int)sizeof(T), L);
  Probe pr;
  const size_t cb = (size_t)g.Nhp * sizeof(C2<T>), db = (size_t)g.Nhp * sizeof(double);
  int i_ck, i_qo = -1, i_po, i_g = -1, i_gs;
  C2<T> *dc = opt<C2<T>>(pr, 3 * cb, Ck, &i_ck);
  const C2<T> *dqi = opt<const C2<T>>(pr, cb, q_in), *dpi = opt<const C2<T>>(pr, cb, p_in);
  C2<T> *dqo = opt<C2<T>>(pr, cb, q_out, &i_qo), *dpo = opt<C2<T>>(pr, cb, p_out, &i_po), *dg = opt<C2<T>>(pr, cb, gk, &i_g);
  const double *dws = opt<const double>(pr, db, wS), *dwm = opt<const double>(pr, db, wM);
  double *dgs = opt<double>(pr, sizeof(double), guard_slot, &i_gs);
  const CtlDev cd = ctl_alloc(pr, ca);
  if (pr.err) return pr.err;
  if (last)
    k_step_boundary<T, true><<<nblk_stride(g.Nhp), 256>>>(g, dc, dqi, dpi, dqo, dpo, dg, dws, dwm, scal[0], scal[1], like_mode,
                                                         scal[2], scal[3], scal[4], dgs, cd.ctl);
  else
    k_step_boundary<T, false><<<nblk_stride(g.Nhp), 256>>>(g, dc, dqi, dpi, dqo, dpo, dg, dws, dwm, scal[0], scal[1],
                                                          like_mode, scal[2], scal[3], scal[4], dgs, cd.ctl);
  Outs o;
  out(o, i_ck, Ck), out(o, i_qo, q_out), out(o, i_po, p_out), out(o, i_g, gk), out(o, i_gs, guard_slot);
  out(o, cd.i_stop, ca.stop), out(o, cd.i_done, ca.steps_done);
  return pr.finish(o);
}

template <typename T> int alpt_poisson(int n, double L, const void *qk, void *d1k, void *phik, double scale) {
  if (!ok3d(n) || !qk || !d1k || !phik) return -1;
  const Geo g = probe_geo(n, (int)sizeof(T), L);
  Probe pr;
  const size_t cb = (size_t)g.Nhp * sizeof(C2<T>);
  const C2<T> *dq = static_cast<const C2<T> *>(pr.alloc(cb, qk));
  C2<T> *d1 = static_cast<C2<T> *>(pr.alloc(cb, d1k)), *dph = static_cast<C2<T> *>(pr.alloc(cb, phik));
  if (pr.err) return pr.err;
  k_alpt_poisson<T><<<nblk_stride(g.Nhp), 256>>>(g, dq, d1, dph, scale);
  return pr.finish({{1, d1k}, {2, phik}});
}

template <typename T> int alpt_mix(int n, double L, void *Ck, double smol, double inv_wtot, double inv_n) {
  if (!ok3d(n) || !Ck) return -1;
  const Geo g = probe_geo(n, (int)sizeof(T), L);
  Probe pr;
  C2<T> *d = static_cast<C2<T> *>(pr.alloc((size_t)3 * g.Nhp * sizeof(C2<T>), Ck));
  if (pr.err) return pr.err;
  k_alpt_mix<T><<<nblk_stride(g.Nhp), 256>>>(g, d, smol, inv_wtot, inv_n);
  return pr.finish({{0, Ck}});
}

int prepare_mult(int n, int esz, const double *corr, double *mult, double normFS) {
  if (!ok3d(n) || !corr || !mult) return -1;
  const Geo g = probe_geo(n, esz);
  Probe pr;
  const double *dc = static_cast<const double *>(pr.alloc((size_t)g.N * sizeof(double), corr));
  double *dm = static_cast<double *>(pr.alloc((size_t)g.Nhp * sizeof(double), mult));
  if (pr.err) return pr.err;
  k_prepare_mult<<<nblk_stride(g.Nhp), 256>>>(g, dc, dm, normFS);
  return pr.finish({{1, mult}});
}

template <typename T> int parseval(int n, const void *xk, const double *w, double *partials) {
  if (!ok3d(n) || !xk || !w || !partials) return -1;
  const Geo g = probe_geo(n, (int)sizeof(T));
  Probe pr;
  const C2<T> *dx = static_cast<const C2<T> *>(pr.alloc((size_t)g.Nhp * sizeof(C2<T>), xk));
  const double *dw = static_cast<const double *>(pr.alloc((size_t)g.Nhp * sizeof(double), w));
  double *dp = static_cast<double *>(pr.alloc((size_t)kRedBlocks * sizeof(double), partials));
  if (pr.err) return pr.err;
  k_parseval<T><<<kRedBlocks, 256>>>(g, dx, dw, dp);
  return pr.finish({{2, partials}});
}

template <typename T>
int rollback(long long count, const int *stop, const unsigned long long *steps_done, const void *q0, const void *p0,
             const void *q1, const void *p1, void *q_dst, void *p_dst) {
  if (count < 1 || count > (1ll << 28) || !stop || !steps_done || !q0 || !p0 || !q1 || !p1 || !q_dst || !p_dst) return -1;
  if (*stop && *steps_done < 1) return -1;
// ... 96 lines not shown

template <typename T>
int interp_tsc(int n, double L, int rsd, const double *pos, double f1, const void *psi, const void *conv, void *V) {
  if (!ok3d(n) || !pos || !psi || !conv || !V || (rsd != 0 && rsd != 1)) return -1;
  const Geo g = probe_geo(n, (int)sizeof(T), L);
  PosPar pp{};
  pp.d = g.d, pp.L = g.L, pp.cpecvel = pos[0], pp.v_norm = pos[1], pp.rsd = rsd, pp.periodic = 1;
  Probe pr;
  const T *dp = static_cast<const T *>(pr.alloc((size_t)3 * g.N * sizeof(T), psi));
  const T *dc = static_cast<const T *>(pr.alloc((size_t)3 * g.N * sizeof(T), conv));
  T *dv = static_cast<T *>(pr.alloc((size_t)3 * g.N * sizeof(T), V));
  if (pr.err) return pr.err;
  k_interp_tsc<T><<<nblk_full(g.N), 256>>>(g, pp, f1, dp, dc, dv);
  return pr.finish({{2, V}});
}

template <typename T>
int tweb_eigen(long long count, const void *t6, const double *x, double lambda_th, double *lam, unsigned char *type,
               unsigned long long *res) {
  if (count < 1 || count > (1ll << 27) || !t6 || !type || !res) return -1;
  Probe pr;
  const T *dt = static_cast<const T *>(pr.alloc((size_t)6 * count * sizeof(T), t6));
  const double *dx = opt<double>(pr, (size_t)count * sizeof(double), x);
  int i_lam = -1;
  double *dl = opt<double>(pr, (size_t)3 * count * sizeof(double), lam, &i_lam);
  unsigned char *dty = static_cast<unsigned char *>(pr.alloc((size_t)count, type));
  const int i_ty = (int)pr.bufs.size() - 1;
  const int nblk = nblk_stride(count);
  unsigned long long *dp = static_cast<unsigned long long *>(pr.alloc(((size_t)nblk + 1) * kTwebWords * sizeof(unsigned long long), nullptr));
  if (pr.err) return pr.err;
  TwebTensor t;
  for (int c = 0; c < 6; c++) t.c[c] = dt + (size_t)c * count;
  k_tweb_eigen<T, double><<<nblk, kTwebBlock>>>(count, t, dx, lambda_th, dl, dty, dp);
  k_tweb_reduce<<<kTwebWords, kWave>>>(nblk, dp, dp + (size_t)nblk * kTwebWords);
  Outs o{{i_ty, type}};
  out(o, i_lam, lam);
  const int rc = pr.finish(o);
  if (rc) return rc;
  if (!pr.ok(hipMemcpy(res, dp + (size_t)nblk * kTwebWords, kTwebWords * sizeof(unsigned long long), hipMemcpyDeviceToHost)))
    return pr.err;
  return 0;
}

template <typename T>
int bispec_triple(int n_shell, long long count, const void *arrays, const unsigned char *s3_end, double *sums, float *ms) {
  if (n_shell < 1 || n_shell > kBispecMaxShell || count < 1 || count > (1ll << 27) || !arrays || !sums) return -1;
  Probe pr;
  const T *da = static_cast<const T *>(pr.alloc((size_t)n_shell * count * sizeof(T), arrays));
  const int grid = bispec_grid(count), W = bispec_triplets(n_shell);
  double *dp = static_cast<double *>(pr.alloc(((size_t)grid + 1) * W * sizeof(double), nullptr));
  if (pr.err) return pr.err;
  const BispecPlan plan = bispec_plan(n_shell, reinterpret_cast<const unsigned char(*)[kBispecMaxShell]>(s3_end));
  BispecArrays arr{};
  for (int s = 0; s < n_shell; s++) arr.a[s] = da + (size_t)s * count;
  hipEvent_t e0 = nullptr, e1 = nullptr;
  if (ms && (!pr.ok(hipEventCreate(&e0)) || !pr.ok(hipEventCreate(&e1)))) return pr.err;
  if (ms) pr.ok(hipEventRecord(e0, nullptr));
  pr.ok(launch_bispec_triple<T>(nullptr, count, n_shell, arr, plan, dp, dp + (size_t)grid * W));
  if (ms) pr.ok(hipEventRecord(e1, nullptr));
  int rc = pr.finish({});
  if (!rc && ms && !pr.ok(hipEventElapsedTime(ms, e0, e1))) rc = pr.err;
  if (e0) (void)hipEventDestroy(e0);
  if (e1) (void)hipEventDestroy(e1);
  if (rc) return rc;
  if (!pr.ok(hipMemcpy(sums, dp + (size_t)grid * W, (size_t)W * sizeof(double), hipMemcpyDeviceToHost))) return pr.err;
  return 0;
}

template <typename T>
int white_noise(long long n, unsigned seed_lo, unsigned seed_hi, unsigned attempt, unsigned stream, const void *var, void *out_) {
  if (n < 1 || n > (1ll << 27) || !out_) return -1;
  Probe pr;
  const T *dv = opt<const T>(pr, (size_t)n * sizeof(T), var);
  T *dout = static_cast<T *>(pr.alloc((size_t)n * sizeof(T), out_));
  const int i_out = (int)pr.bufs.size() - 1;
  if (pr.err) return pr.err;
  k_white_noise<T><<<nblk_stride((n + 1) / 2), 256>>>(n, make_uint2(seed_lo, seed_hi), attempt, stream, dv, dout);
  return pr.finish({{i_out, out_}});
}

template <typename T> int color_momenta(long long nh, const void *wk, const double *wM, void *pk, int accumulate) {
  if (nh < 1 || nh > (1ll << 27) || !wk || !pk) return -1;
  Probe pr;
  const C2<T> *dw = static_cast<const C2<T> *>(pr.alloc((size_t)nh * sizeof(C2<T>), wk));
  const double *dm = opt<const double>(pr, (size_t)nh * sizeof(double), wM);
  C2<T> *dp = static_cast<C2<T> *>(pr.alloc((size_t)nh * sizeof(C2<T>), pk));
  const int i_pk = (int)pr.bufs.size() - 1;
  if (pr.err) return pr.err;
  k_color_momenta<T><<<nblk_stride(nh), 256>>>(nh, dw, dm, dp, accumulate);
  return pr.finish({{i_pk, pk}});
}

}

extern "C" {

int fftp_row_stride(int n, int prec) { return fft_row_stride(n, prec ? 4 : 8); }

int fftp_xfft(int prec, int n, int kb, int inverse, int groups, void *data) {
  return prec ? xfft<float>(n, kb, inverse, groups, data) : xfft<double>(n, kb, inverse, groups, data);
}

int fftp_ypass(int prec, int n, int inverse, void *ck) {
  return prec ? ypass<float>(n, inverse, ck) : ypass<double>(n, inverse, ck);
}

int fftp_ypass_pair(int prec, int n, double box_len, void *ck) {
  return prec ? ypass_pair<float>(n, box_len, ck) : ypass_pair<double>(n, box_len, ck);
}

int fftp_zr2c(int prec, int n, const void *V, void *ck) {
  return prec ? zr2c<float>(n, V, ck) : zr2c<double>(n, V, ck);
}

int fftp_zr2c_rec(int prec, int n, const void *V, void *ck) {
  return prec ? zr2c<float, true>(n, V, ck) : zr2c<double, true>(n, V, ck);
}

int fftp_ypass_fwd_pair(int prec, int n, double box_len, void *ck) {
  return prec ? ypass_fwd_pair<float>(n, box_len, ck) : ypass_fwd_pair<double>(n, box_len, ck);
}

int fftp_zc2r(int prec, int n, const void *ck, void *psi) {
  return prec ? zc2r<float>(n, ck, psi) : zc2r<double>(n, ck, psi);
}


int fftp_step_boundary_x(int prec, int n, double box_len, int mode, int alpt, int two_tile, void *Ck, const void *q_in,
                         const void *p_in, const void *g_in, void *q_out, void *p_out, void *g_out, const double *wS,
                         const double *wM, const double *scal, double *guard_slot, int *stop,
                         unsigned long long *steps_done, const double *guard_prev, double guard_limit,
                         unsigned long long step_index) {
  const CtlArgs ca{stop, steps_done, guard_prev, guard_limit, step_index};
  if (!stop || !steps_done) return -1;
  return prec ? step_boundary_x<float>(n, box_len, mode, alpt, two_tile, Ck, q_in, p_in, g_in, q_out, p_out, g_out, wS, wM,
                                       scal, guard_slot, ca)
              : step_boundary_x<double>(n, box_len, mode, alpt, two_tile, Ck, q_in, p_in, g_in, q_out, p_out, g_out, wS, wM,
                                        scal, guard_slot, ca);
}

int fftp_step_boundary_x_vpair(int prec, int n, double box_len, int mode, int alpt, int two_tile, void *Ck, const void *q_in,
                               const void *p_in, const void *g_in, void *q_out, void *p_out, void *g_out, const double *wS,
                               const double *wM, const double *scal, double *guard_slot, int *stop,
                               unsigned long long *steps_done, const double *guard_prev, double guard_limit,
                               unsigned long long step_index, int vpair) {
  const CtlArgs ca{stop, steps_done, guard_prev, guard_limit, step_index};
  if (!stop || !steps_done) return -1;
  return prec ? step_boundary_x<float>(n, box_len, mode, alpt, two_tile, Ck, q_in, p_in, g_in, q_out, p_out, g_out, wS, wM,
                                       scal, guard_slot, ca, vpair)
              : step_boundary_x<double>(n, box_len, mode, alpt, two_tile, Ck, q_in, p_in, g_in, q_out, p_out, g_out, wS, wM,
                                        scal, guard_slot, ca, vpair);
}

int fftp_alpt_mix_x(int prec, int n, double box_len, void *Ck, double smol, double inv_wtot, double inv_n) {
  return prec ? alpt_mix_x<float>(n, box_len, Ck, smol, inv_wtot, inv_n)
              : alpt_mix_x<double>(n, box_len, Ck, smol, inv_wtot, inv_n);
}

int fftp_kick_drift_za(int prec, int n, double box_len, int drift, void *qk, void *pk, const void *gk, const double *wM,
                       const void *extra, void *Ck, const double *scal, int *stop, unsigned long long *steps_done,
                       const double *guard_prev, double guard_limit, unsigned long long step_index) {
  const CtlArgs ca{stop, steps_done, guard_prev, guard_limit, step_index};
  if (!stop || !steps_done) return -1;
  return prec ? kick_drift_za<float>(n, box_len, drift, qk, pk, gk, wM, extra, Ck, scal, ca)
              : kick_drift_za<double>(n, box_len, drift, qk, pk, gk, wM, extra, Ck, scal, ca);
}

int fftp_assemble(int prec, int n, double box_len, int kick, const void *Ck, const void *qk, const double *wS, void *gk,
                  void *pk, const double *scal, int like_mode, double *guard_slot, int *stop) {
  return prec ? assemble<float>(n, box_len, kick, Ck, qk, wS, gk, pk, scal, like_mode, guard_slot, stop)
              : assemble<double>(n, box_len, kick, Ck, qk, wS, gk, pk, scal, like_mode, guard_slot, stop);
}

int fftp_step_boundary(int prec, int n, double box_len, int last, void *Ck, const void *q_in, const void *p_in, void *q_out,
                       void *p_out, void *gk, const double *wS, const double *wM, const double *scal, int like_mode,
                       double *guard_slot, int *stop, unsigned long long *steps_done, const double *guard_prev,
                       double guard_limit, unsigned long long step_index) {
  const CtlArgs ca{stop, steps_done, guard_prev, guard_limit, step_index};
  if (!stop || !steps_done) return -1;
  return prec ? step_boundary<float>(n, box_len, last, Ck, q_in, p_in, q_out, p_out, gk, wS, wM, scal, like_mode, guard_slot, ca)
              : step_boundary<double>(n, box_len, last, Ck, q_in, p_in, q_out, p_out, gk, wS, wM, scal, like_mode, guard_slot,
                                      ca);
}

int fftp_alpt_poisson(int prec, int n, double box_len, const void *qk, void *d1k, void *phik, double scale) {
  return prec ? alpt_poisson<float>(n, box_len, qk, d1k, phik, scale) : alpt_poisson<double>(n, box_len, qk, d1k, phik, scale);
}

int fftp_alpt_mix(int prec, int n, double box_len, void *Ck, double smol, double inv_wtot, double inv_n) {
  return prec ? alpt_mix<float>(n, box_len, Ck, smol, inv_wtot, inv_n) : alpt_mix<double>(n, box_len, Ck, smol, inv_wtot, inv_n);
}

int fftp_prepare_mult(int prec, int n, const double *corr, double *mult, double normFS) {
  return prepare_mult(n, prec ? 4 : 8, corr, mult, normFS);
}

int fftp_parseval_blocks(void) { return kRedBlocks; }
int fftp_parseval(int prec, int n, const void *xk, const double *w, double *partials) {
  return prec ? parseval<float>(n, xk, w, partials) : parseval<double>(n, xk, w, partials);
}

int fftp_rollback(int prec, long long count, const int *stop, const unsigned long long *steps_done, const void *q0,
                  const void *p0, const void *q1, const void *p1, void *q_dst, void *p_dst) {
  return prec ? rollback<float>(count, stop, steps_done, q0, p0, q1, p1, q_dst, p_dst)
              : rollback<double>(count, stop, steps_done, q0, p0, q1, p1, q_dst, p_dst);
}


int fftp_stencil_grid(int n) { return stencil_grid(n); }

int fftp_alpt_grad(int prec, int n, double box_len, const void *phi, void *g3) {
  return prec ? alpt_grad<float>(n, box_len, phi, g3) : alpt_grad<double>(n, box_len, phi, g3);
}

int fftp_alpt_sources(int prec, int n, double box_len, int layout, const void *g3, void *d1, void *other, double D1, double D2) {
  return prec ? alpt_sources<float>(n, box_len, layout, g3, d1, other, D1, D2)
              : alpt_sources<double>(n, box_len, layout, g3, d1, other, D1, D2);
}

int fftp_alpt_kernel_table(int prec, int n, double box_len, void *tab, double smol) {
  return prec ? alpt_kernel_table<float>(n, box_len, tab, smol) : alpt_kernel_table<double>(n, box_len, tab, smol);
}

int fftp_findif_mul(int prec, int n, double box_len, int likelihood, double rho_c, double delta_min, const void *dX,
                    const void *plike, void *V) {
  return prec ? findif_mul<float>(n, box_len, likelihood, rho_c, delta_min, dX, plike, V)
              : findif_mul<double>(n, box_len, likelihood, rho_c, delta_min, dX, plike, V);
}

int fftp_gradfft_mult(int prec, int n, double box_len, const void *fk, void *Ck, double inv_n) {
  return prec ? gradfft_mult<float>(n, box_len, fk, Ck, inv_n) : gradfft_mult<double>(n, box_len, fk, Ck, inv_n);
}

int fftp_conv_kernel(int prec, int n, double box_len, const void *pl, const double *F, void *Ck, double hh, double inv_n) {
  return prec ? conv_kernel<float>(n, box_len, pl, F, Ck, hh, inv_n) : conv_kernel<double>(n, box_len, pl, F, Ck, hh, inv_n);
}

int fftp_mul3(int prec, long long count, const void *a, const void *b3, void *out3) {
  return prec ? mul3<float>(count, a, b3, out3) : mul3<double>(count, a, b3, out3);
}

int fftp_interp_tsc(int prec, int n, double box_len, int rsd, const double *pos, double f1, const void *psi,
                    const void *conv, void *V) {
  return prec ? interp_tsc<float>(n, box_len, rsd, pos, f1, psi, conv, V)
              : interp_tsc<double>(n, box_len, rsd, pos, f1, psi, conv, V);
}

int fftp_tweb_eigen(int prec, long long count, const void *t6, const double *x, double lambda_th, double *lam,
                    unsigned char *type, unsigned long long *res) {
  return prec ? tweb_eigen<float>(count, t6, x, lambda_th, lam, type, res)
              : tweb_eigen<double>(count, t6, x, lambda_th, lam, type, res);
}

int fftp_bispec_triple(int prec, int n_shell, long long count, const void *arrays, const unsigned char *s3_end, double *sums,
                       float *ms) {
  return prec ? bispec_triple<float>(n_shell, count, arrays, s3_end, sums, ms)
              : bispec_triple<double>(n_shell, count, arrays, s3_end, sums, ms);
}

int fftp_white_noise(int prec, long long n, unsigned seed_lo, unsigned seed_hi, unsigned attempt, unsigned stream,
                     const void *var, void *out) {
  return prec ? white_noise<float>(n, seed_lo, seed_hi, attempt, stream, var, out)
              : white_noise<double>(n, seed_lo, seed_hi, attempt, stream, var, out);
}

int fftp_color_momenta(int prec, long long nh, const void *wk, const double *wM, void *pk, int accumulate) {
  return prec ? color_momenta<float>(nh, wk, wM, pk, accumulate) : color_momenta<double>(nh, wk, wM, pk, accumulate);
}

}
```

barcode_amd/csrc/pass_launch.hpp:

```cpp
#pragma once

#include <cstddef>

namespace bchmc {

constexpr int pass_kb(int esz) { return 128 / (2 * esz); }
constexpr int pass_nt_big(int esz) { return esz == 8 ? 256 : 512; }
constexpr int pass_nt_small(int esz) { return pass_nt_big(esz) / 4; }

struct PassShape {
  int nt = 0;
  int per = 0;
};

constexpr PassShape x_shape(int esz, int n) {
  const int big = pass_nt_big(esz), small = pass_nt_small(esz);
  switch (n) {
    case 32: return {small, 4};
    case 64: return {small, 8};
    case 128: return {big, 4};
    case 256: return {2 * big, 4};
    case 512: return {2 * big, 8};
    default: return {};
  }
}
constexpr PassShape x2_shape(int esz, int n) { return n == 128 || n == 256 ? x_shape(esz, n) : PassShape{}; }
constexpr PassShape y_shape(int esz, int n) {
  const int nt = n == 128 ? 256 : 512;
  return n == 128 || n == 256 || n == 512 ? PassShape{nt, n * pass_kb(esz) / nt} : PassShape{};
}
constexpr PassShape ypair_shape(int esz, int n) { return y_shape(esz, n); }
constexpr int ypair_comps = 2;
constexpr PassShape yfwd_pair_shape(int esz, int n) { return ypair_shape(esz, n); }
constexpr PassShape z_shape(int , int n) { return n == 128 || n == 256 || n == 512 ? PassShape{n, 6} : PassShape{}; }

constexpr size_t col_lds(int esz, int n, int tiles = 1) { return ((size_t)tiles * n * pass_kb(esz) + n / 2) * 2 * esz; }
constexpr size_t zrow_lds(int esz, int n) { return ((size_t)n * 6 + n / 2) * 2 * esz; }

constexpr int col_grid(int esz, int n, int nhp, int comps = 1) { return comps * n * (nhp / pass_kb(esz)); }
constexpr int row_grid(int n) { return (n / 2) * (n / 2); }
constexpr int ypair_grid(int esz, int n, int nhp) { return col_grid(esz, n, nhp, ypair_comps); }

}

#ifdef __HIPCC__
#include "kernels.hpp"

#include <type_traits>

namespace bchmc {

template <typename... P, typename... A>
hipError_t launch_dyn_lds(hipStream_t stream, void (*kern)(P...), int grid, int threads, size_t lds, const A &...args) {
  if (lds > 48 * 1024) {
    const hipError_t e =
        hipFuncSetAttribute(reinterpret_cast<const void *>(kern), hipFuncAttributeMaxDynamicSharedMemorySize, (int)lds);
    if (e != hipSuccess) return e;
  }
  kern<<<grid, threads, lds, stream>>>(args...);
  return hipGetLastError();
}

template <PassShape (*TABLE)(int, int), typename T, int N, typename F>
hipError_t pass_row(int n, F &f) {
  constexpr PassShape s = TABLE((int)sizeof(T), N);
  if constexpr (s.nt != 0) {
    if (n == N) return f(std::integral_constant<int, s.nt>{}, std::integral_constant<int, s.per>{});
  }
  return hipErrorInvalidConfiguration;
}
template <PassShape (*TABLE)(int, int), typename T, typename F>
hipError_t pass_dispatch(int n, F f) {
  switch (n) {
    case 32: return pass_row<TABLE, T, 32>(n, f);
    case 64: return pass_row<TABLE, T, 64>(n, f);
    case 128: return pass_row<TABLE, T, 128>(n, f);
    case 256: return pass_row<TABLE, T, 256>(n, f);
    case 512: return pass_row<TABLE, T, 512>(n, f);
    default: return hipErrorInvalidConfiguration;
  }
}

template <typename T>
struct PassCtx {
  hipStream_t stream;
  Geo g;
  int log2n;
  const C2<T> *tw;
  int col_grid(int comps = 1) const { return bchmc::col_grid(sizeof(T), g.n, g.nhp, comps); }
  size_t col_lds(int tiles = 1) const { return bchmc::col_lds(sizeof(T), g.n, tiles); }
};

template <typename T, bool INV = true>
hipError_t launch_ypass(const PassCtx<T> &x, C2<T> *ck) {
  return pass_dispatch<y_shape, T>(x.g.n, [&](auto nt, auto per) {
    return launch_dyn_lds(x.stream, k_ypass<T, nt, per, BCHMC_YPASS_NT, INV>, x.col_grid(3), nt, x.col_lds(), x.g, x.log2n,
                          x.tw, ck);
  });
}

template <typename T>
hipError_t launch_ypass_fwd_pair(const PassCtx<T> &x, C2<T> *ck) {
  return pass_dispatch<yfwd_pair_shape, T>(x.g.n, [&](auto nt, auto per) {
    return launch_dyn_lds(x.stream, k_ypass_fwd_pair<T, nt, per>, ypair_grid(sizeof(T), x.g.n, x.g.nhp),
                          nt, x.col_lds(), x.g, x.log2n, x.tw, ck);
  });
}

template <typename T>
hipError_t launch_ypass_pair(const PassCtx<T> &x, C2<T> *ck) {
  return pass_dispatch<ypair_shape, T>(x.g.n, [&](auto nt, auto per) {
    return launch_dyn_lds(x.stream, k_ypass_pair<T, nt, per, BCHMC_YPASS_NT>, ypair_grid(sizeof(T), x.g.n, x.g.nhp), nt,
                          x.col_lds(), x.g, x.log2n, x.tw, ck);
  });
}

template <typename T, bool REC = false>
hipError_t launch_zr2c(const PassCtx<T> &x, const T *V, C2<T> *ck) {
  return pass_dispatch<z_shape, T>(x.g.n, [&](auto nz, auto) {
    return launch_dyn_lds(x.stream, k_zr2c<T, nz, REC>, row_grid(x.g.n), nz, zrow_lds(sizeof(T), x.g.n), x.g, x.log2n, x.tw, V,
                          ck);
  });
}

template <typename T, bool PSI_ONLY = false, typename... A>
hipError_t launch_zbin(const PassCtx<T> &x, const PosPar &pp, const SphPar &sp, const TilePar &tp, const C2<T> *ck,
                       const A &...out) {
  return pass_dispatch<z_shape, T>(x.g.n, [&](auto nz, auto) {
    return launch_dyn_lds(x.stream, k_zbin_direct<T, nz, PSI_ONLY>, row_grid(x.g.n), nz, zbin_lds<T>(x.g.n), x.g, pp, sp, tp,
                          x.log2n, x.tw, ck, out...);
  });
}

template <typename T>
hipError_t launch_alpt_mix_x(const PassCtx<T> &x, C2<T> *Ck, double smol, double inv_wtot, double inv_n) {
  return pass_dispatch<x_shape, T>(x.g.n, [&](auto nt, auto per) {
    return launch_dyn_lds(x.stream, k_alpt_mix_x<T, nt, per>, x.col_grid(), nt, x.col_lds(), x.g, x.log2n, x.tw, Ck, smol,
                          inv_wtot, inv_n);
  });
}

template <typename T>
struct BoundaryX {
  const C2<T> *qi = nullptr, *pi = nullptr;
  C2<T> *qo = nullptr, *po = nullptr;
  const double *wM = nullptr;
  double a = 0., b = 0., half_eps = 0., eps = 0., c_za = 0.;
  double *guard_slot = nullptr;
  StepCtl ctl{};
  const C2<T> *g_in = nullptr;
  C2<T> *g_out = nullptr;
  bool pair = false;
  bool vpair = false;
};

template <typename T, int MODE, bool ALPT>
hipError_t launch_step_boundary_x(const PassCtx<T> &x, C2<T> *Ck, const double *wS, const BoundaryX<T> &a) {
  return pass_dispatch<x_shape, T>(x.g.n, [&](auto nt, auto per) {
    return launch_dyn_lds(x.stream, k_step_boundary_x<T, nt, per, MODE, ALPT>, x.col_grid(), nt, x.col_lds(), x.g, x.log2n,
                          x.tw, Ck, a.qi, a.pi, a.qo, a.po, wS, a.wM, a.a, a.b, a.half_eps, a.eps, a.c_za, a.guard_slot,
                          a.ctl, a.g_in, a.g_out, a.pair && !ALPT && MODE != BX_LAST,
                          a.vpair && !ALPT && MODE != BX_FIRST);
  });
}

template <typename T>
hipError_t launch_step_boundary_x2(const PassCtx<T> &x, C2<T> *Ck, const double *wS, const BoundaryX<T> &a) {
  return pass_dispatch<x2_shape, T>(x.g.n, [&](auto nt, auto per) {
    return launch_dyn_lds(x.stream, k_step_boundary_x2<T, nt, per>, x.col_grid(), nt, x.col_lds(2), x.g, x.log2n, x.tw, Ck,
                          a.qi, a.pi, a.qo, a.po, wS, a.wM, a.a, a.b, a.half_eps, a.eps, a.c_za, a.guard_slot, a.ctl, a.pair,
                          a.vpair);
  });
}

}
#endif
```

barcode_amd/csrc/step_boundary_x.hpp:

```cpp
#pragma once
#include "common.hpp"

#ifndef BCHMC_BX_WAVES
#define BCHMC_BX_WAVES 4
#endif

namespace bchmc {

#ifndef BCHMC_BX_NT
#define BCHMC_BX_NT 2
#endif
typedef double bx_dv2 __attribute__((ext_vector_type(2)));
typedef float bx_fv2 __attribute__((ext_vector_type(2)));
__device__ __forceinline__ void bx_store(double2 *p, const double2 v) {
  if (BCHMC_BX_NT) {
    bx_dv2 t = {v.x, v.y};
    __builtin_nontemporal_store(t, reinterpret_cast<bx_dv2 *>(p));
  } else {
    *p = v;
  }
}
__device__ __forceinline__ void bx_store(float2 *p, const float2 v) {
  if (BCHMC_BX_NT) {
    bx_fv2 t = {v.x, v.y};
    __builtin_nontemporal_store(t, reinterpret_cast<bx_fv2 *>(p));
  } else {
    *p = v;
  }
}

__device__ __forceinline__ double2 bx_load(const double2 *p) {
  if (BCHMC_BX_NT >= 2) {
    const bx_dv2 t = __builtin_nontemporal_load(reinterpret_cast<const bx_dv2 *>(p));
    return make_double2(t.x, t.y);
  }
  return *p;
}
__device__ __forceinline__ float2 bx_load(const float2 *p) {
  if (BCHMC_BX_NT >= 2) {
    const bx_fv2 t = __builtin_nontemporal_load(reinterpret_cast<const bx_fv2 *>(p));
    return make_float2(t.x, t.y);
  }
  return *p;
}
__device__ __forceinline__ double bx_load(const double *p) {
  return BCHMC_BX_NT >= 2 ? __builtin_nontemporal_load(p) : *p;
}

template <typename T>
__device__ __forceinline__ C2<T> cmul(const C2<T> a, const C2<T> b) {
  C2<T> r;
  r.x = a.x * b.x - a.y * b.y;
  r.y = a.x * b.y + a.y * b.x;
  return r;
}

template <typename T>
__device__ __forceinline__ C2<T> bx_w_of(double ky, double kz, const C2<T> vy, const C2<T> vz) {
  C2<T> w;
  w.x = (T)(ky * (double)vy.x + kz * (double)vz.x);
  w.y = (T)(ky * (double)vy.y + kz * (double)vz.y);
  return w;
}

template <typename T>
__device__ __forceinline__ void xfft_inplace(C2<T> *__restrict__ s, const C2<T> *__restrict__ tw, int n, int log2n,
                                             int KB, bool inverse) {
  int st = 1;
  if (log2n & 1) {
    const int nb = (n >> 1) * KB;
    for (int b = threadIdx.x; b < nb; b += blockDim.x) {
      const int c = b % KB, i0 = (b / KB) << 1;
      const C2<T> a = s[i0 * KB + c], x = s[(i0 + 1) * KB + c];
      C2<T> o0, o1;
      o0.x = a.x + x.x; o0.y = a.y + x.y;
      o1.x = a.x - x.x; o1.y = a.y - x.y;
      s[i0 * KB + c] = o0;
      s[(i0 + 1) * KB + c] = o1;
    }
    __syncthreads();
    st = 2;
  }
  const int nq = (n >> 2) * KB;
  for (; st < log2n; st += 2) {
    const int half = 1 << (st - 1);
    const int t1 = n >> st, t2 = n >> (st + 1);
    for (int b = threadIdx.x; b < nq; b += blockDim.x) {
      const int c = b % KB, bf = b / KB;
      const int r = bf & (half - 1), grp = bf >> (st - 1);
      const int j = (grp << (st + 1)) + r;
      C2<T> w1 = tw[r * t1], w2 = tw[r * t2];
      if (inverse) {
        w1.y = -w1.y;
        w2.y = -w2.y;
      }
      const C2<T> e0 = s[j * KB + c], e1 = s[(j + half) * KB + c], e2 = s[(j + 2 * half) * KB + c],
                  e3 = s[(j + 3 * half) * KB + c];
      const C2<T> m1 = cmul<T>(w1, e1), m3 = cmul<T>(w1, e3);
      C2<T> a0, a1, a2, a3;
      a0.x = e0.x + m1.x; a0.y = e0.y + m1.y;
      a1.x = e0.x - m1.x; a1.y = e0.y - m1.y;
      a2.x = e2.x + m3.x; a2.y = e2.y + m3.y;
      a3.x = e2.x - m3.x; a3.y = e2.y - m3.y;
      const C2<T> n2 = cmul<T>(w2, a2), n3 = cmul<T>(w2, a3);
      C2<T> r3;
      if (inverse) {
        r3.x = -n3.y; r3.y = n3.x;
      } else {
        r3.x = n3.y; r3.y = -n3.x;
      }
      C2<T> o0, o1, o2, o3;
      o0.x = a0.x + n2.x; o0.y = a0.y + n2.y;
      o2.x = a0.x - n2.x; o2.y = a0.y - n2.y;
      o1.x = a1.x + r3.x; o1.y = a1.y + r3.y;
      o3.x = a1.x - r3.x; o3.y = a1.y - r3.y;
      s[j * KB + c] = o0;
      s[(j + half) * KB + c] = o1;
      s[(j + 2 * half) * KB + c] = o2;
      s[(j + 3 * half) * KB + c] = o3;
    }
    __syncthreads();
  }
}

enum { BX_INTERIOR = 0, BX_FIRST = 1, BX_LAST = 2 };

template <typename T, int NT, int PER, int MODE = BX_INTERIOR, bool ALPT = false>
__global__ void __launch_bounds__(NT, BCHMC_BX_WAVES)
k_step_boundary_x(Geo g, int log2n, const C2<T> *__restrict__ twiddle, C2<T> *Ck, const C2<T> *q_in, const C2<T> *p_in,
                  C2<T> *q_out, C2<T> *p_out, const double *__restrict__ wS, const double *__restrict__ wM, double a,
                  double b, double half_eps, double eps, double c_za, double *guard_slot, StepCtl ctl,
                  const C2<T> *g_in = nullptr, C2<T> *g_out = nullptr, bool pair = false, bool vpair = false) {
  constexpr int KB = 128 / (int)sizeof(C2<T>);
  constexpr int kMaxPer = PER;
  extern __shared__ __attribute__((aligned(16))) unsigned char s_raw_x[];
  __shared__ double red[NT / 64];
  const bool controlled = MODE == BX_INTERIOR || (MODE == BX_FIRST && g_in) || (MODE == BX_LAST && p_out);
  if (controlled) {
    if (*ctl.stop) return;
    if (ctl.guard_prev && fabs(*ctl.guard_prev) > ctl.guard_limit) {
      if (blockIdx.x == 0 && threadIdx.x == 0) {
        *ctl.steps_done = ctl.step_index;
        __threadfence();
        *ctl.stop = 1;
      }
      return;
    }
  }
  const int n = g.n;
  C2<T> *s = reinterpret_cast<C2<T> *>(s_raw_x);
  C2<T> *tw = s + (size_t)n * KB;
  for (int t = threadIdx.x; t < n / 2; t += blockDim.x) tw[t] = twiddle[t];
  const int ntk = g.nhp / KB;
  int bid = (int)blockIdx.x;
  if ((gridDim.x & 7) == 0) bid = (bid & 7) * (int)(gridDim.x >> 3) + (bid >> 3);
  const int j = bid / ntk, k0 = (bid % ntk) * KB;
  const int c = threadIdx.x % KB, irow = threadIdx.x / KB;
  constexpr int rows = NT / KB, per = PER;
  const int k = k0 + c;
  const long long plane = (long long)g.n * g.nhp;
  const long long col = k + (long long)g.nhp * j;
  const double ky = kval(j, g.n, g.kfac), kz = kval(k, g.n, g.kfac);
  const int shift = 32 - log2n;
  double2 hk[kMaxPer];
  for (int pass = 0; pass < (MODE == BX_FIRST ? 0 : 2); pass++) {
    __syncthreads();
#pragma unroll
    for (int m = 0; m < kMaxPer; m++) {
      const int i = irow + rows * m;
      const long long e = col + plane * i;
      C2<T> v;
      if (pass == 0) {
        v = bx_load(Ck + e);
      } else if (vpair) {
        v = bx_load(Ck + e + g.Nhp);
      } else {
        const C2<T> vy = bx_load(Ck + e + g.Nhp), vz = bx_load(Ck + e + 2 * g.Nhp);
        v = bx_w_of<T>(ky, kz, vy, vz);
      }
      s[(int)(__brev((unsigned)i) >> shift) * KB + c] = v;
    }
    __syncthreads();
    xfft_inplace<T>(s, tw, n, log2n, KB, false);
#pragma unroll
    for (int m = 0; m < kMaxPer; m++) {
      const int i = irow + rows * m;
      const C2<T> v = s[i * KB + c];
      if (pass == 0) {
        const double kx = kval(i, g.n, g.kfac);
        hk[m] = make_double2(kx * (double)v.y, -(kx * (double)v.x));
      } else {
        hk[m].x += (double)v.y;
        hk[m].y -= (double)v.x;
      }
    }
  }
  double gsum = 0.;
  C2<T> qkeep[kMaxPer];
  __syncthreads();
#pragma unroll
  for (int m = 0; m < kMaxPer; m++) {
    const int i = irow + rows * m;
    const long long idx = col + plane * i;
    const double kx = kval(i, g.n, g.kfac);
    const double ksq = kx * kx + ky * ky + kz * kz;
    const bool nyq = (i == g.n / 2) || (j == g.n / 2) || (k == g.n / 2);
    double2 q;
    if (MODE == BX_INTERIOR) {
      const C2<T> t = bx_load(q_in + idx);
      q = make_double2((double)t.x, (double)t.y);
    } else q = ld2<T>(q_in, idx);
    if (MODE == BX_FIRST) {
      if (g_in) {
        double2 p = ld2<T>(p_in, idx);
        const double2 g0 = ld2<T>(g_in, idx);
        p.x -= half_eps * g0.x;
        p.y -= half_eps * g0.y;
        st2<T>(p_out, idx, p.x, p.y);
        if (wM) {
          const double w = wM[idx];
          q.x += eps * (w * p.x);
          q.y += eps * (w * p.y);
        }
        st2<T>(q_out, idx, q.x, q.y);
      }
    } else {
      double2 gg = make_double2(0., 0.);
      if (ksq > 0 && !nyq) {
        const double f = b * (1 / ksq);
        gg = make_double2(f * hk[m].x, f * hk[m].y);
      }
      if (a != 0.) {
        const double w = a * bx_load(wS + idx);
        gg.x += w * q.x;
        gg.y += w * q.y;
      }
      C2<T> gs;
      gs.x = (T)gg.x;
      gs.y = (T)gg.y;
      if (MODE == BX_LAST) {
        g_out[idx] = gs;
        if (p_out) {
          const double2 p = ld2<T>(p_in, idx);
          C2<T> pe;
          pe.x = (T)(p.x - half_eps * gg.x);
          pe.y = (T)(p.y - half_eps * gg.y);
          const double hw = (k == 0 || ((g.n & 1) == 0 && k == g.n / 2)) ? 1. : 2.;
          if (k < g.nh) gsum += hw * (double)pe.x;
          p_out[idx] = pe;
        }
        continue;
      }
      const C2<T> pt = bx_load(p_in + idx);
      double2 p = make_double2((double)pt.x, (double)pt.y);
      C2<T> pe;
      pe.x = (T)(p.x - half_eps * gg.x);
      pe.y = (T)(p.y - half_eps * gg.y);
      const double hw = (k == 0 || ((g.n & 1) == 0 && k == g.n / 2)) ? 1. : 2.;
      if (k < g.nh) gsum += hw * (double)pe.x;
      p.x = (double)pe.x - half_eps * (double)gs.x;
      p.y = (double)pe.y - half_eps * (double)gs.y;
      {
        C2<T> t;
        t.x = (T)p.x;
        t.y = (T)p.y;
        bx_store(p_out + idx, t);
      }
      if (wM) {
        const double w = bx_load(wM + idx);
        q.x += eps * (w * p.x);
        q.y += eps * (w * p.y);
      }
      {
        C2<T> t;
        t.x = (T)q.x;
        t.y = (T)q.y;
        bx_store(q_out + idx, t);
      }
    }
    qkeep[m].x = (T)q.x;
    qkeep[m].y = (T)q.y;
    C2<T> o;
    o.x = T(0);
    o.y = T(0);
    if (ALPT) {
      o.x = (T)(c_za * q.x);
      o.y = (T)(c_za * q.y);
    } else if (ksq > 1.e-14 && !nyq) {
      const double f = (1. / ksq) * kx;
      o.x = (T)(f * (c_za * q.y));
      o.y = (T)(f * -(c_za * q.x));
    }
    s[(int)(__brev((unsigned)i) >> shift) * KB + c] = o;
  }
  if (MODE == BX_LAST) {
    if (p_out) {
      gsum = block_sum(gsum, red);
      if (threadIdx.x == 0) atomic_add_r(guard_slot, gsum);
    }
    return;
  }
  __syncthreads();
  xfft_inplace<T>(s, tw, n, log2n, KB, true);
  for (int m = 0; m < per; m++) {
    const int i = irow + rows * m;
    bx_store(Ck + col + plane * i, s[i * KB + c]);
  }
  __syncthreads();
#pragma unroll
  for (int m = 0; m < kMaxPer; m++) {
    const int i = irow + rows * m;
    const double kx = kval(i, g.n, g.kfac);
    const double ksq = kx * kx + ky * ky + kz * kz;
    const bool nyq = (i == g.n / 2) || (j == g.n / 2) || (k == g.n / 2);
    C2<T> o;
    o.x = T(0);
    o.y = T(0);
    if (ALPT) {
      const double f = (ksq > 0.) ? -1. / ksq : 0.;
      o.x = (T)(f * (c_za * (double)qkeep[m].x));
      o.y = (T)(f * (c_za * (double)qkeep[m].y));
    } else if (ksq > 1.e-14 && !nyq) {
      const double2 qn = make_double2((double)qkeep[m].x, (double)qkeep[m].y);
      const double f = 1. / ksq;
      o.x = (T)(f * (c_za * qn.y));
      o.y = (T)(f * -(c_za * qn.x));
    }
    s[(int)(__brev((unsigned)i) >> shift) * KB + c] = o;
  }
  __syncthreads();
  xfft_inplace<T>(s, tw, n, log2n, KB, true);
  for (int m = 0; m < per; m++) {
    const int i = irow + rows * m;
    const C2<T> v = s[i * KB + c];
    if (ALPT) {
      bx_store(Ck + col + plane * i + g.Nhp, v);
      continue;
    }
    if (pair) {
      bx_store(Ck + col + plane * i + g.Nhp, v);
      continue;
    }
    C2<T> oy, oz;
    oy.x = (T)(ky * (double)v.x);
    oy.y = (T)(ky * (double)v.y);
    oz.x = (T)(kz * (double)v.x);
    oz.y = (T)(kz * (double)v.y);
    bx_store(Ck + col + plane * i + g.Nhp, oy);
    bx_store(Ck + col + plane * i + 2 * g.Nhp, oz);
  }
  if (MODE == BX_INTERIOR) {
    gsum = block_sum(gsum, red);
    if (threadIdx.x == 0) atomic_add_r(guard_slot, gsum);
  }
}


template <typename T, bool INV>
__device__ __forceinline__ void xfft_r4(C2<T> *__restrict__ s, int j, int half, int KB, int c, C2<T> w1, C2<T> w2) {
  const C2<T> e0 = s[j * KB + c], e1 = s[(j + half) * KB + c], e2 = s[(j + 2 * half) * KB + c],
              e3 = s[(j + 3 * half) * KB + c];
  const C2<T> m1 = cmul<T>(w1, e1), m3 = cmul<T>(w1, e3);
  C2<T> a0, a1, a2, a3;
  a0.x = e0.x + m1.x; a0.y = e0.y + m1.y;
  a1.x = e0.x - m1.x; a1.y = e0.y - m1.y;
  a2.x = e2.x + m3.x; a2.y = e2.y + m3.y;
  a3.x = e2.x - m3.x; a3.y = e2.y - m3.y;
  const C2<T> n2 = cmul<T>(w2, a2), n3 = cmul<T>(w2, a3);
  C2<T> r3;
  if (INV) {
    r3.x = -n3.y; r3.y = n3.x;
  } else {
    r3.x = n3.y; r3.y = -n3.x;
  }
  C2<T> o0, o1, o2, o3;
  o0.x = a0.x + n2.x; o0.y = a0.y + n2.y;
  o2.x = a0.x - n2.x; o2.y = a0.y - n2.y;
  o1.x = a1.x + r3.x; o1.y = a1.y + r3.y;
  o3.x = a1.x - r3.x; o3.y = a1.y - r3.y;
  s[j * KB + c] = o0;
  s[(j + half) * KB + c] = o1;
  s[(j + 2 * half) * KB + c] = o2;
  s[(j + 3 * half) * KB + c] = o3;
}

template <typename T, bool INV>
__device__ __forceinline__ void xfft_inplace2(C2<T> *__restrict__ sa, C2<T> *__restrict__ sb,
                                              const C2<T> *__restrict__ tw, int n, int log2n, int KB) {
  int st = 1;
  if (log2n & 1) {
    const int nb = (n >> 1) * KB;
    for (int b = threadIdx.x; b < nb; b += blockDim.x) {
      const int c = b % KB, i0 = (b / KB) << 1;
#pragma unroll
      for (int u = 0; u < 2; u++) {
        C2<T> *s = u ? sb : sa;
        const C2<T> a = s[i0 * KB + c], x = s[(i0 + 1) * KB + c];
        C2<T> o0, o1;
        o0.x = a.x + x.x; o0.y = a.y + x.y;
        o1.x = a.x - x.x; o1.y = a.y - x.y;
        s[i0 * KB + c] = o0;
        s[(i0 + 1) * KB + c] = o1;
      }
    }
    __syncthreads();
    st = 2;
  }
  const int nq = (n >> 2) * KB;
  for (; st < log2n; st += 2) {
    const int half = 1 << (st - 1);
    const int t1 = n >> st, t2 = n >> (st + 1);
    for (int b = threadIdx.x; b < nq; b += blockDim.x) {
      const int c = b % KB, bf = b / KB;
      const int r = bf & (half - 1), grp = bf >> (st - 1);
      const int j = (grp << (st + 1)) + r;
      C2<T> w1 = tw[r * t1], w2 = tw[r * t2];
      if (INV) {
        w1.y = -w1.y;
        w2.y = -w2.y;
      }
      xfft_r4<T, INV>(sa, j, half, KB, c, w1, w2);
      xfft_r4<T, INV>(sb, j, half, KB, c, w1, w2);
    }
    __syncthreads();
  }
}

template <typename T, int NT, int PER>
__global__ void __launch_bounds__(NT, BCHMC_BX_WAVES)
k_step_boundary_x2(Geo g, int log2n, const C2<T> *__restrict__ twiddle, C2<T> *Ck, const C2<T> *q_in, const C2<T> *p_in,
                   C2<T> *q_out, C2<T> *p_out, const double *__restrict__ wS, const double *__restrict__ wM, double a,
                   double b, double half_eps, double eps, double c_za, double *guard_slot, StepCtl ctl, bool pair = false,
                   bool vpair = false) {
  constexpr int KB = 128 / (int)sizeof(C2<T>);
  extern __shared__ __attribute__((aligned(16))) unsigned char s_raw_x2[];
  __shared__ double red[NT / 64];
  if (*ctl.stop) return;
  if (ctl.guard_prev && fabs(*ctl.guard_prev) > ctl.guard_limit) {
    if (blockIdx.x == 0 && threadIdx.x == 0) {
      *ctl.steps_done = ctl.step_index;
      __threadfence();
      *ctl.stop = 1;
    }
    return;
  }
  const int n = g.n;
  C2<T> *sa = reinterpret_cast<C2<T> *>(s_raw_x2);
  C2<T> *sb = sa + (size_t)n * KB;
  C2<T> *tw = sb + (size_t)n * KB;
  for (int t = threadIdx.x; t < n / 2; t += blockDim.x) tw[t] = twiddle[t];
  const int ntk = g.nhp / KB;
  int bid = (int)blockIdx.x;
  if ((gridDim.x & 7) == 0) bid = (bid & 7) * (int)(gridDim.x >> 3) + (bid >> 3);
  const int j = bid / ntk, k0 = (bid % ntk) * KB;
  const int c = threadIdx.x % KB, irow = threadIdx.x / KB;
  constexpr int rows = NT / KB;
  const int k = k0 + c;
  const long long plane = (long long)g.n * g.nhp;
  const long long col = k + (long long)g.nhp * j;
  const double ky = kval(j, g.n, g.kfac), kz = kval(k, g.n, g.kfac);
  const int shift = 32 - log2n;
  unsigned boff[PER];
#pragma unroll
  for (int m = 0; m < PER; m++) boff[m] = (unsigned)((col + plane * (irow + rows * m)) * (long long)sizeof(C2<T>));
  auto at_c = [](const C2<T> *base, unsigned off) {
    return reinterpret_cast<const C2<T> *>(reinterpret_cast<const char *>(base) + off);
  };
  auto at_cw = [](C2<T> *base, unsigned off) {
    return reinterpret_cast<C2<T> *>(reinterpret_cast<char *>(base) + off);
  };
  auto at_d = [](const double *base, unsigned off) {
    return reinterpret_cast<const double *>(reinterpret_cast<const char *>(base) + off);
  };
  C2<T> *const Ck1 = Ck + g.Nhp, *const Ck2 = Ck + 2 * g.Nhp;
  {
    C2<T> vx[PER], vy[PER], vz[PER];
#pragma unroll
    for (int m = 0; m < PER; m++) {
      vx[m] = bx_load(at_c(Ck, boff[m]));
      vy[m] = bx_load(at_c(Ck1, boff[m]));
      if (!vpair) vz[m] = bx_load(at_c(Ck2, boff[m]));
    }
#pragma unroll
    for (int m = 0; m < PER; m++) {
      const int i = irow + rows * m;
      const int r = (int)(__brev((unsigned)i) >> shift) * KB + c;
      sa[r] = vx[m];
      sb[r] = vpair ? vy[m] : bx_w_of<T>(ky, kz, vy[m], vz[m]);
    }
  }
  C2<T> qv[PER], pv[PER];
  double ws[PER], wm[PER];
#pragma unroll
  for (int m = 0; m < PER; m++) {
    const unsigned woff = sizeof(C2<T>) == 16 ? boff[m] / 2 : boff[m];
    qv[m] = bx_load(at_c(q_in, boff[m]));
    pv[m] = bx_load(at_c(p_in, boff[m]));
    ws[m] = (a != 0.) ? bx_load(at_d(wS, woff)) : 0.;
    wm[m] = wM ? bx_load(at_d(wM, woff)) : 0.;
  }
  __syncthreads();
  xfft_inplace2<T, false>(sa, sb, tw, n, log2n, KB);
  double2 hk[PER];
#pragma unroll
  for (int m = 0; m < PER; m++) {
    const int i = irow + rows * m;
    const C2<T> v = sa[i * KB + c], w = sb[i * KB + c];
    const double kx = kval(i, g.n, g.kfac);
    hk[m] = make_double2(kx * (double)v.y, -(kx * (double)v.x));
    hk[m].x += (double)w.y;
    hk[m].y -= (double)w.x;
  }
  __syncthreads();
  double gsum = 0.;
#pragma unroll
  for (int m = 0; m < PER; m++) {
    const int i = irow + rows * m;
    const double kx = kval(i, g.n, g.kfac);
    const double ksq = kx * kx + ky * ky + kz * kz;
    const bool nyq = (i == g.n / 2) || (j == g.n / 2) || (k == g.n / 2);
    double2 q = make_double2((double)qv[m].x, (double)qv[m].y);
    double2 gg = make_double2(0., 0.);
    if (ksq > 0 && !nyq) {
      const double f = b * (1 / ksq);
      gg = make_double2(f * hk[m].x, f * hk[m].y);
    }
    if (a != 0.) {
      const double w = a * ws[m];
      gg.x += w * q.x;
      gg.y += w * q.y;
    }
    C2<T> gs;
    gs.x = (T)gg.x;
    gs.y = (T)gg.y;
    double2 p = make_double2((double)pv[m].x, (double)pv[m].y);
    C2<T> pe;
    pe.x = (T)(p.x - half_eps * gg.x);
    pe.y = (T)(p.y - half_eps * gg.y);
    const double hw = (k == 0 || ((g.n & 1) == 0 && k == g.n / 2)) ? 1. : 2.;
    if (k < g.nh) gsum += hw * (double)pe.x;
    p.x = (double)pe.x - half_eps * (double)gs.x;
    p.y = (double)pe.y - half_eps * (double)gs.y;
    {
      C2<T> t;
      t.x = (T)p.x;
      t.y = (T)p.y;
      bx_store(at_cw(p_out, boff[m]), t);
    }
    if (wM) {
      q.x += eps * (wm[m] * p.x);
      q.y += eps * (wm[m] * p.y);
    }
    C2<T> qs;
    qs.x = (T)q.x;
    qs.y = (T)q.y;
    bx_store(at_cw(q_out, boff[m]), qs);
    C2<T> o, o2;
    o.x = o.y = o2.x = o2.y = T(0);
    if (ksq > 1.e-14 && !nyq) {
      const double f = (1. / ksq) * kx;
      o.x = (T)(f * (c_za * q.y));
      o.y = (T)(f * -(c_za * q.x));
      const double f2 = 1. / ksq;
      o2.x = (T)(f2 * (c_za * (double)qs.y));
      o2.y = (T)(f2 * -(c_za * (double)qs.x));
    }
    const int r = (int)(__brev((unsigned)i) >> shift) * KB + c;
    sa[r] = o;
    sb[r] = o2;
  }
  __syncthreads();
  xfft_inplace2<T, true>(sa, sb, tw, n, log2n, KB);
#pragma unroll
  for (int m = 0; m < PER; m++) {
    const int i = irow + rows * m;
    bx_store(at_cw(Ck, boff[m]), sa[i * KB + c]);
    const C2<T> v = sb[i * KB + c];
    if (pair) {
      bx_store(at_cw(Ck1, boff[m]), v);
      continue;
    }
    C2<T> oy, oz;
    oy.x = (T)(ky * (double)v.x);
    oy.y = (T)(ky * (double)v.y);
    oz.x = (T)(kz * (double)v.x);
    oz.y = (T)(kz * (double)v.y);
    bx_store(at_cw(Ck1, boff[m]), oy);
    bx_store(at_cw(Ck2, boff[m]), oz);
  }
  gsum = block_sum(gsum, red);
  if (threadIdx.x == 0) atomic_add_r(guard_slot, gsum);
}

}
```

Baseline: 391.3 steps/s.

## Keep k-space q/p state in x-tiled layout across leapfrog boundary kernels

Result: faster. 397.6 steps/s (median of 6 runs) (+1.6%).

```diff
diff --git a/barcode_amd/csrc/bchmc.hip b/barcode_amd/csrc/bchmc.hip
--- a/barcode_amd/csrc/bchmc.hip
+++ b/barcode_amd/csrc/bchmc.hip
@@ -5,6 +5,7 @@
 #include "pass_launch.hpp"
 #include "launch_grid.hpp"
 #include "eval_plan.hpp"
+#include "xtile_kernels.hpp"
 #include "interp_plan.hpp"
 
 #include <rocfft/rocfft.h>
@@ -56,9 +57,12 @@
   DevBytes in_arr[6];
   bool have[6] = {false, false, false, false, false, false};
   DevBuf<double> wS, wM;
+  DevBuf<double2> wpair;
+  unsigned long long w_gen = 1, wpair_gen = 0;
 
   DevBytes qk, pk, gk;
   DevBytes qk2, pk2;
+  XLayout qk_layout = XLayout::kNatural;
   DevBytes Ck;
   bool ck_pair = false;
   DevBytes tC;
@@ -638,6 +642,7 @@
   s.no_pair = env_on("BCHMC_NO_PAIR");
   s.no_vpair = env_on("BCHMC_NO_VPAIR");
   s.no_vrec = env_on("BCHMC_NO_VREC");
+  s.no_xtile = env_on("BCHMC_NO_XTILE");
   return s;
 }
 
@@ -647,7 +652,7 @@
   f.planes_ok = h->planes_ok && h->xtw;
   f.tiled = h->plan.tiled, f.sort_direct = h->plan.slots.sort_direct, f.std81 = h->plan.std81;
   f.mk = h->c.mk, f.calc_h = h->c.calc_h, f.likelihood = h->c.likelihood, f.sfmodel = h->c.sfmodel;
-  f.rsd_model = h->c.rsd_model, f.mass_rs = h->mass_rs != 0;
+  f.rsd_model = h->c.rsd_model, f.mass_rs = h->mass_rs != 0, f.mass_fs = h->mass_fs != 0;
   if (alpt_planes_wanted(f, h->sw, rsd) && !h->c2r2d_2 && !h->alpt_plans_failed &&
       make_plans_2d(h, 2 * (size_t)h->g.n, h->r2c2d_2, h->c2r2d_2) != BCHMC_OK)
     h->alpt_plans_failed = true;
@@ -1660,19 +1665,23 @@
     return fft_exec(h, h->r2c1, staging, out, BCHMC_K_FFT_R2C);
   }
 
-  static int c2r_scaled(bchmc_handle *h, const void *xk, void *out_T) {
+  static int c2r_scaled(bchmc_handle *h, const void *xk, void *out_T, bool xtiled = false) {
     {
       ProfScope ps(h, BCHMC_K_OTHER);
-      k_scale_c<T><<<nblk_stride(h->g.Nhp), 256, 0, h->stream>>>(h->g.Nhp, reinterpret_cast<const CT *>(xk), C(h->tC),
-                                                                1. / (double)h->g.N);
+      if (xtiled)
+        k_xtile_scale_c<T><<<nblk_stride(h->g.Nhp), 256, 0, h->stream>>>(h->g, reinterpret_cast<const CT *>(xk), C(h->tC),
+                                                                        1. / (double)h->g.N);
+      else
+        k_scale_c<T><<<nblk_stride(h->g.Nhp), 256, 0, h->stream>>>(h->g.Nhp, reinterpret_cast<const CT *>(xk), C(h->tC),
+                                                                  1. / (double)h->g.N);
       HIPCHK(hipGetLastError());
     }
     return fft_exec(h, h->c2r1, h->tC, out_T, BCHMC_K_FFT_C2R);
   }
 
-  static int c2r_state(bchmc_handle *h, const void *xk, void *scratch_T, double *d_out) {
-    if (kDouble) return c2r_scaled(h, xk, d_out);
-    CHK(c2r_scaled(h, xk, scratch_T));
+  static int c2r_state(bchmc_handle *h, const void *xk, void *scratch_T, double *d_out, bool xtiled = false) {
+    if (kDouble) return c2r_scaled(h, xk, d_out, xtiled);
+    CHK(c2r_scaled(h, xk, scratch_T, xtiled));
     return store_real(h, R(scratch_T), d_out);
   }
 
@@ -1704,6 +1713,7 @@
     TrajPlan p;
     double a, c_za;
     bool pair;
+    bool xt;
   };
   static Traj traj(bchmc_handle *h) {
     Traj t;
@@ -1712,17 +1722,18 @@
     t.a = h->c.grad_psi_prior_factor;
     t.c_za = (t.p.c_za == CZa::kAlptInput ? 1. : -h->c.D1) * h->c.deltaQ_factor / (double)h->g.N;
     t.pair = psi_pair(t.f, h->sw, t.p);
+    t.xt = x_tiles(t.f, h->sw, t.p);
     return t;
   }
 
-  template <int MODE, bool ALPT = false>
+  template <int MODE, bool ALPT = false, bool XT = false>
   static int launch_boundary_x(bchmc_handle *h, BoundaryX<T> bx) {
     if (MODE != BX_FIRST) {
       if (ALPT && h->ck_vpair) return h->fail(BCHMC_ERR_STATE, "two arrays of V^ in Ck, and a boundary that reads three");
       bx.vpair = h->ck_vpair;
       h->ck_vpair = false;
     }
-    HIPCHK((launch_step_boundary_x<T, MODE, ALPT>(pass_ctx(h), C(h->Ck), h->wS, bx)));
+    HIPCHK((launch_step_boundary_x<T, MODE, ALPT, XT>(pass_ctx(h), C(h->Ck), h->wS, bx)));
     h->ck_pair = bx.pair && !ALPT && MODE != BX_LAST;
     return BCHMC_OK;
   }
@@ -1817,22 +1828,32 @@
       CHK(dev_alloc(h, h->qk2, 2 * (size_t)h->g.Nhp * sizeof(T)));
       CHK(dev_alloc(h, h->pk2, 2 * (size_t)h->g.Nhp * sizeof(T)));
     }
-    void *const q0 = h->qk, *const p0 = h->pk, *const q1 = h->qk2, *const p1 = h->pk2;
+    const bool xt = t.xt;
+    const char *const wrong_layout = "a k-space state pair in one layout, and a kernel that reads the other";
+    if (h->qk_layout != XLayout::kNatural) return h->fail(BCHMC_ERR_STATE, wrong_layout);
+    if (xt) CHK(tiled_weights(h));
+    XPairs xp;
+    void *const qb[2] = {h->qk, h->qk2}, *const pb[2] = {h->pk, h->pk2};
     int like_mode = 2;
     double b = 0.;
-    int cur = 0;
     {
+      const Opening op = opening(t.f, h->sw, t.p);
+      if (!xp.open(xt, op == Opening::kBxFirst)) return h->fail(BCHMC_ERR_STATE, wrong_layout);
       StepCtl ctl{h->stop, h->steps_done, nullptr, guard_limit, 0};
       ProfScope ps(h, BCHMC_K_KSPACE_DRIFT_ZA);
       BoundaryX<T> bx;
-      bx.qi = bx.qo = C(q0), bx.pi = bx.po = C(p0), bx.wM = wM, bx.half_eps = 0.5 * eps, bx.eps = eps, bx.c_za = c_za;
+      bx.qi = C(qb[0]), bx.pi = C(pb[0]), bx.qo = C(qb[xp.cur]), bx.po = C(pb[xp.cur]), bx.wM = wM, bx.wpair = h->wpair;
+      bx.half_eps = 0.5 * eps, bx.eps = eps, bx.c_za = c_za;
       bx.ctl = ctl, bx.g_in = C(g_first), bx.pair = t.pair;
-      switch (opening(t.f, h->sw, t.p)) {
+      switch (op) {
         case Opening::kBxFirstAlpt: CHK((launch_boundary_x<BX_FIRST, true>(h, bx))); break;
-        case Opening::kBxFirst: CHK(launch_boundary_x<BX_FIRST>(h, bx)); break;
+        case Opening::kBxFirst:
+          if (xt) CHK((launch_boundary_x<BX_FIRST, false, true>(h, bx)));
+          else CHK(launch_boundary_x<BX_FIRST>(h, bx));
+          break;
         case Opening::kKickDriftZa:
           h->ck_pair = false;
-          k_kick_drift_za<T, true><<<nblk_stride(h->g.Nhp), 256, 0, h->stream>>>(h->g, C(q0), C(p0), C(g_first), wM,
+          k_kick_drift_za<T, true><<<nblk_stride(h->g.Nhp), 256, 0, h->stream>>>(h->g, C(qb[0]), C(pb[0]), C(g_first), wM,
                                                                                nullptr, C(h->Ck), 0.5 * eps, eps, c_za, ctl);
           break;
       }
@@ -1841,7 +1862,7 @@
     for (uint64_t s = 0; s < neps; s++) {
       const bool last = (s + 1 == neps);
       if (last && h->early_q_dev && h->ev_q) {
-        CHK(c2r_state(h, cur ? q1 : q0, h->ioq, h->early_q_dev));
+        CHK(c2r_state(h, qb[xp.cur], h->ioq, h->early_q_dev, xp.q[xp.cur] == XLayout::kTiled));
         HIPCHK(hipEventRecord(h->ev_q, h->stream));
         h->early_q_done = true;
       }
@@ -1850,15 +1871,19 @@
       CHK(force_sources(h, true, step_mode(t.f, h->sw, t.p, s, neps), &like_mode, &b));
       if (tap && tap->like_f && last) CHK(tap_loglike(h, tap->like_f));
       StepCtl ctl{h->stop, h->steps_done, s > 0 ? h->guard + (s - 1) : nullptr, guard_limit, s};
-      void *qi = cur ? q1 : q0, *pi = cur ? p1 : p0, *qo = cur ? q0 : q1, *po = cur ? p0 : p1;
+      const Closing cl = closing(t.f, h->sw, t.p, s, neps, like_mode);
+      const int src = xp.cur, dst = xp.dst(xt, last);
+      if (!xp.close(xt, cl, last)) return h->fail(BCHMC_ERR_STATE, wrong_layout);
+      void *qi = qb[src], *pi = pb[src], *qo = qb[src ^ 1], *po = pb[src ^ 1];
       ProfScope ps(h, BCHMC_K_KSPACE_FORCE_KICK);
       BoundaryX<T> bx;
       bx.qi = C(qi), bx.pi = C(pi), bx.qo = C(qo), bx.po = C(po), bx.wM = wM, bx.a = a, bx.b = b, bx.half_eps = 0.5 * eps;
-      bx.eps = eps, bx.c_za = c_za, bx.guard_slot = h->guard + s, bx.ctl = ctl, bx.pair = t.pair;
-      switch (closing(t.f, h->sw, t.p, s, neps, like_mode)) {
+      bx.eps = eps, bx.c_za = c_za, bx.guard_slot = h->guard + s, bx.ctl = ctl, bx.pair = t.pair, bx.wpair = h->wpair;
+      switch (cl) {
         case Closing::kBxLast:
-          bx.qo = nullptr, bx.po = C(pi), bx.g_out = C(h->gk);
-          CHK(launch_boundary_x<BX_LAST>(h, bx));
+          bx.qo = nullptr, bx.po = C(pb[dst]), bx.g_out = C(h->gk);
+          if (xt) CHK((launch_boundary_x<BX_LAST, false, true>(h, bx)));
+          else CHK(launch_boundary_x<BX_LAST>(h, bx));
           break;
         case Closing::kStepBoundaryLast:
           if (h->ck_vpair) return h->fail(BCHMC_ERR_STATE, "two arrays of V^ in Ck, and a boundary that reads three");
@@ -1867,11 +1892,15 @@
               h->guard + s, ctl);
           break;
         case Closing::kBxInteriorAlpt: CHK((launch_boundary_x<BX_INTERIOR, true>(h, bx))); break;
-        case Closing::kBxInterior: CHK(launch_boundary_x<BX_INTERIOR>(h, bx)); break;
+        case Closing::kBxInterior:
+          if (xt) CHK((launch_boundary_x<BX_INTERIOR, false, true>(h, bx)));
+          else CHK(launch_boundary_x<BX_INTERIOR>(h, bx));
+          break;
         case Closing::kBxInteriorTwoTile:
           bx.vpair = h->ck_vpair;
           h->ck_vpair = false;
-          HIPCHK(launch_step_boundary_x2<T>(pass_ctx(h), C(h->Ck), h->wS, bx));
+          if (xt) HIPCHK((launch_step_boundary_x2<T, true>(pass_ctx(h), C(h->Ck), h->wS, bx)));
+          else HIPCHK(launch_step_boundary_x2<T>(pass_ctx(h), C(h->Ck), h->wS, bx));
           h->ck_pair = bx.pair;
           break;
         case Closing::kStepBoundary:
@@ -1881,19 +1910,39 @@
               h->guard + s, ctl);
           break;
       }
-      if (buffers_flip(s, neps)) cur ^= 1;
       HIPCHK(hipGetLastError());
     }
+    const int fin = xp.cur, res = xp.result(xt);
+    if (!xp.finish(xt)) return h->fail(BCHMC_ERR_STATE, wrong_layout);
     {
       ProfScope ps(h, BCHMC_K_OTHER);
-      k_rollback<T><<<nblk_stride(h->g.Nhp), 256, 0, h->stream>>>(h->g.Nhp, h->stop, h->steps_done, C(q0), C(p0), C(q1),
-                                                                 C(p1), C(cur ? q1 : q0), C(cur ? p1 : p0));
+      if (xt) {
+        CT *const sq = C(h->Ck), *const sp = C(h->Ck) + h->g.Nhp;
+        k_xtile_finish<T><<<nblk_stride(h->g.Nhp), 256, 0, h->stream>>>(h->g, h->stop, h->steps_done, C(qb[0]), C(pb[0]),
+                                                                       C(qb[1]), C(pb[1]), fin, C(qb[res]), sq, sp);
+        HIPCHK(hipGetLastError());
+        k_xtile_restore<T><<<nblk_stride(h->g.Nhp), 256, 0, h->stream>>>(h->g.Nhp, h->stop, sq, sp, C(qb[res]), C(pb[res]));
+      } else {
+        k_rollback<T><<<nblk_stride(h->g.Nhp), 256, 0, h->stream>>>(h->g.Nhp, h->stop, h->steps_done, C(qb[0]), C(pb[0]),
+                                                                   C(qb[1]), C(pb[1]), C(qb[res]), C(pb[res]));
+      }
       HIPCHK(hipGetLastError());
     }
-    if (cur) {
+    h->qk_layout = xp.q[res];
+    if (res) {
       std::swap(h->qk, h->qk2);
       std::swap(h->pk, h->pk2);
     }
+    return BCHMC_OK;
+  }
+
+  static int tiled_weights(bchmc_handle *h) {
+    if (!h->wpair) CHK(dev_alloc(h, h->wpair, (size_t)h->g.Nhp));
+    else if (h->wpair_gen == h->w_gen) return BCHMC_OK;
+    ProfScope ps(h, BCHMC_K_OTHER);
+    k_xtile_weights<<<nblk_stride(h->g.Nhp), 256, 0, h->stream>>>(h->g, pass_kb((int)sizeof(T)), h->wS, h->wM, h->wpair);
+    HIPCHK(hipGetLastError());
+    h->wpair_gen = h->w_gen;
     return BCHMC_OK;
   }
 
@@ -2728,6 +2777,7 @@
       double *w = field == BCHMC_F_SIGNAL_PS ? h->wS : h->wM;
       k_prepare_mult<<<nblk_stride(h->g.Nhp), 256, 0, h->stream>>>(h->g, d_src, w, normFS);
       HIPCHK(hipGetLastError());
+      h->w_gen++;
     }
     return BCHMC_OK;
   }
diff --git a/barcode_amd/csrc/eval_plan.hpp b/barcode_amd/csrc/eval_plan.hpp
--- a/barcode_amd/csrc/eval_plan.hpp
+++ b/barcode_amd/csrc/eval_plan.hpp
@@ -17,6 +17,7 @@
   bool no_pair = false;
   bool no_vpair = false;
   bool no_vrec = false;
+  bool no_xtile = false;
 };
 
 struct PathFacts {
@@ -29,6 +30,7 @@
   bool mass_rs = false;
   bool alpt_plans = false;
   bool std81 = false;
+  bool mass_fs = false;
 };
 
 struct EvalMode {
diff --git a/barcode_amd/csrc/fft_probe.hip b/barcode_amd/csrc/fft_probe.hip
--- a/barcode_amd/csrc/fft_probe.hip
+++ b/barcode_amd/csrc/fft_probe.hip
@@ -2,6 +2,7 @@
 #include "fft_host.hpp"
 #include "pass_launch.hpp"
 #include "launch_grid.hpp"
+#include "xtile_kernels.hpp"
 
 #include <cmath>
 #include <cstring>
@@ -221,8 +222,10 @@
 template <typename T>
 int step_boundary_x(int n, double L, int mode, int alpt, int two_tile, void *Ck, const void *q_in, const void *p_in,
                     const void *g_in, void *q_out, void *p_out, void *g_out, const double *wS, const double *wM,
-                    const double *scal, double *guard_slot, const CtlArgs &ca, int vpair = 0) {
+                    const double *scal, double *guard_slot, const CtlArgs &ca, int vpair = 0, const void *wpair = nullptr) {
   if (mode < BX_INTERIOR || mode > BX_LAST || (alpt && mode == BX_LAST)) return -1;
+  const bool xt = wpair != nullptr;
+  if (xt && (alpt || !wM || !p_in || (mode != BX_LAST && !q_out) || !p_out || (mode == BX_FIRST && !g_in))) return -1;
   if (vpair && (alpt || mode == BX_FIRST)) return -1;
   if (two_tile ? (!x2_shape(sizeof(T), n).nt || mode != BX_INTERIOR || alpt) : !x_shape(sizeof(T), n).nt) return -1;
   const Geo g = probe_geo(n, (int)sizeof(T), L);
@@ -251,9 +254,14 @@
   const CtlDev cd = ctl_alloc(pr, ca);
   a.ctl = cd.ctl;
   a.vpair = vpair != 0;
+  a.wpair = opt<const double2>(pr, (size_t)g.Nhp * sizeof(double2), wpair);
   if (pr.err) return pr.err;
   hipError_t e = hipErrorInvalidConfiguration;
-  if (two_tile) e = launch_step_boundary_x2<T>(x, d_ck, d_ws, a);
+  if (xt && two_tile) e = launch_step_boundary_x2<T, true>(x, d_ck, d_ws, a);
+  else if (xt && mode == BX_INTERIOR) e = launch_step_boundary_x<T, BX_INTERIOR, false, true>(x, d_ck, d_ws, a);
+  else if (xt && mode == BX_FIRST) e = launch_step_boundary_x<T, BX_FIRST, false, true>(x, d_ck, d_ws, a);
+  else if (xt) e = launch_step_boundary_x<T, BX_LAST, false, true>(x, d_ck, d_ws, a);
+  else if (two_tile) e = launch_step_boundary_x2<T>(x, d_ck, d_ws, a);
   else if (mode == BX_INTERIOR) e = alpt ? launch_step_boundary_x<T, BX_INTERIOR, true>(x, d_ck, d_ws, a)
                                          : launch_step_boundary_x<T, BX_INTERIOR, false>(x, d_ck, d_ws, a);
   else if (mode == BX_FIRST) e = alpt ? launch_step_boundary_x<T, BX_FIRST, true>(x, d_ck, d_ws, a)
@@ -656,6 +664,33 @@
                                         scal, guard_slot, ca, vpair);
 }
 
+int fftp_step_boundary_x_xtile(int prec, int n, double box_len, int mode, int two_tile, void *Ck, const void *q_in,
+                               const void *p_in, const void *g_in, void *q_out, void *p_out, void *g_out, const double *wS,
+                               const double *wM, const double *scal, double *guard_slot, int *stop,
+                               unsigned long long *steps_done, const double *guard_prev, double guard_limit,
+                               unsigned long long step_index, int vpair, const void *wpair) {
+  const CtlArgs ca{stop, steps_done, guard_prev, guard_limit, step_index};
+  if (!stop || !steps_done || !wpair) return -1;
+  return prec ? step_boundary_x<float>(n, box_len, mode, 0, two_tile, Ck, q_in, p_in, g_in, q_out, p_out, g_out, wS, wM,
+                                       scal, guard_slot, ca, vpair, wpair)
+              : step_boundary_x<double>(n, box_len, mode, 0, two_tile, Ck, q_in, p_in, g_in, q_out, p_out, g_out, wS, wM,
+                                        scal, guard_slot, ca, vpair, wpair);
+}
+
+int fftp_xtile_weights(int prec, int n, const double *wS, const double *wM, void *pair) {
+  const int esz = prec ? 4 : 8;
+  if (!x_shape(esz, n).nt || !wS || !wM || !pair) return -1;
+  const Geo g = probe_geo(n, esz);
+  if (g.nhp % pass_kb(esz)) return -1;
+  Probe pr;
+  const size_t db = (size_t)g.Nhp * sizeof(double);
+  const double *d_ws = static_cast<const double *>(pr.alloc(db, wS)), *d_wm = static_cast<const double *>(pr.alloc(db, wM));
+  double2 *d_pair = static_cast<double2 *>(pr.alloc(2 * db, pair));
+  if (pr.err) return pr.err;
+  k_xtile_weights<<<nblk_stride(g.Nhp), 256>>>(g, pass_kb(esz), d_ws, d_wm, d_pair);
+  return pr.finish({{2, pair}});
+}
+
 int fftp_alpt_mix_x(int prec, int n, double box_len, void *Ck, double smol, double inv_wtot, double inv_n) {
   return prec ? alpt_mix_x<float>(n, box_len, Ck, smol, inv_wtot, inv_n)
               : alpt_mix_x<double>(n, box_len, Ck, smol, inv_wtot, inv_n);
diff --git a/barcode_amd/csrc/pass_launch.hpp b/barcode_amd/csrc/pass_launch.hpp
--- a/barcode_amd/csrc/pass_launch.hpp
+++ b/barcode_amd/csrc/pass_launch.hpp
@@ -152,24 +152,27 @@
   C2<T> *g_out = nullptr;
   bool pair = false;
   bool vpair = false;
+  const double2 *wpair = nullptr;
 };
 
-template <typename T, int MODE, bool ALPT>
+template <typename T, int MODE, bool ALPT, bool XT = false>
 hipError_t launch_step_boundary_x(const PassCtx<T> &x, C2<T> *Ck, const double *wS, const BoundaryX<T> &a) {
+  if (XT && (!a.wpair || !a.wM || a.po == a.pi || a.qo == a.qi)) return hipErrorInvalidValue;
   return pass_dispatch<x_shape, T>(x.g.n, [&](auto nt, auto per) {
-    return launch_dyn_lds(x.stream, k_step_boundary_x<T, nt, per, MODE, ALPT>, x.col_grid(), nt, x.col_lds(), x.g, x.log2n,
-                          x.tw, Ck, a.qi, a.pi, a.qo, a.po, wS, a.wM, a.a, a.b, a.half_eps, a.eps, a.c_za, a.guard_slot,
-                          a.ctl, a.g_in, a.g_out, a.pair && !ALPT && MODE != BX_LAST,
-                          a.vpair && !ALPT && MODE != BX_FIRST);
+    return launch_dyn_lds(x.stream, k_step_boundary_x<T, nt, per, MODE, ALPT, XT>, x.col_grid(), nt, x.col_lds(), x.g,
+                          x.log2n, x.tw, Ck, a.qi, a.pi, a.qo, a.po, wS, a.wM, a.a, a.b, a.half_eps, a.eps, a.c_za,
+                          a.guard_slot, a.ctl, a.g_in, a.g_out, a.pair && !ALPT && MODE != BX_LAST,
+                          a.vpair && !ALPT && MODE != BX_FIRST, a.wpair);
   });
 }
 
-template <typename T>
+template <typename T, bool XT = false>
 hipError_t launch_step_boundary_x2(const PassCtx<T> &x, C2<T> *Ck, const double *wS, const BoundaryX<T> &a) {
+  if (XT && (!a.wpair || !a.wM || a.po == a.pi || a.qo == a.qi)) return hipErrorInvalidValue;
   return pass_dispatch<x2_shape, T>(x.g.n, [&](auto nt, auto per) {
-    return launch_dyn_lds(x.stream, k_step_boundary_x2<T, nt, per>, x.col_grid(), nt, x.col_lds(2), x.g, x.log2n, x.tw, Ck,
-                          a.qi, a.pi, a.qo, a.po, wS, a.wM, a.a, a.b, a.half_eps, a.eps, a.c_za, a.guard_slot, a.ctl, a.pair,
-                          a.vpair);
+    return launch_dyn_lds(x.stream, k_step_boundary_x2<T, nt, per, XT>, x.col_grid(), nt, x.col_lds(2), x.g, x.log2n, x.tw,
+                          Ck, a.qi, a.pi, a.qo, a.po, wS, a.wM, a.a, a.b, a.half_eps, a.eps, a.c_za, a.guard_slot, a.ctl,
+                          a.pair, a.vpair, a.wpair);
   });
 }
 
diff --git a/barcode_amd/csrc/step_boundary_x.hpp b/barcode_amd/csrc/step_boundary_x.hpp
--- a/barcode_amd/csrc/step_boundary_x.hpp
+++ b/barcode_amd/csrc/step_boundary_x.hpp
@@ -45,6 +45,15 @@
 }
 __device__ __forceinline__ double bx_load(const double *p) {
   return BCHMC_BX_NT >= 2 ? __builtin_nontemporal_load(p) : *p;
+}
+
+template <typename U>
+__device__ __forceinline__ const U *bx_at(const U *base, unsigned off) {
+  return reinterpret_cast<const U *>(reinterpret_cast<const char *>(base) + off);
+}
+template <typename U>
+__device__ __forceinline__ U *bx_at(U *base, unsigned off) {
+  return reinterpret_cast<U *>(reinterpret_cast<char *>(base) + off);
 }
 
 template <typename T>
@@ -125,12 +134,14 @@
 
 enum { BX_INTERIOR = 0, BX_FIRST = 1, BX_LAST = 2 };
 
-template <typename T, int NT, int PER, int MODE = BX_INTERIOR, bool ALPT = false>
+template <typename T, int NT, int PER, int MODE = BX_INTERIOR, bool ALPT = false, bool XT = false>
 __global__ void __launch_bounds__(NT, BCHMC_BX_WAVES)
 k_step_boundary_x(Geo g, int log2n, const C2<T> *__restrict__ twiddle, C2<T> *Ck, const C2<T> *q_in, const C2<T> *p_in,
                   C2<T> *q_out, C2<T> *p_out, const double *__restrict__ wS, const double *__restrict__ wM, double a,
                   double b, double half_eps, double eps, double c_za, double *guard_slot, StepCtl ctl,
-                  const C2<T> *g_in = nullptr, C2<T> *g_out = nullptr, bool pair = false, bool vpair = false) {
+                  const C2<T> *g_in = nullptr, C2<T> *g_out = nullptr, bool pair = false, bool vpair = false,
+                  const double2 *__restrict__ wpair = nullptr) {
+  static_assert(!(XT && ALPT), "the ALPT boundary has no tiled form");
   constexpr int KB = 128 / (int)sizeof(C2<T>);
   constexpr int kMaxPer = PER;
   extern __shared__ __attribute__((aligned(16))) unsigned char s_raw_x[];
@@ -162,6 +173,10 @@
   const long long col = k + (long long)g.nhp * j;
   const double ky = kval(j, g.n, g.kfac), kz = kval(k, g.n, g.kfac);
   const int shift = 32 - log2n;
+  const long long tbase = XT ? (long long)bid * n * KB : 0;
+  const C2<T> *const qt_in = q_in + tbase, *const pt_in = p_in + tbase;
+  C2<T> *const qt_out = q_out + tbase, *const pt_out = p_out + tbase;
+  const double2 *const wt = wpair + tbase;
   double2 hk[kMaxPer];
   for (int pass = 0; pass < (MODE == BX_FIRST ? 0 : 2); pass++) {
     __syncthreads();
@@ -205,24 +220,41 @@
     const double kx = kval(i, g.n, g.kfac);
     const double ksq = kx * kx + ky * ky + kz * kz;
     const bool nyq = (i == g.n / 2) || (j == g.n / 2) || (k == g.n / 2);
+    const unsigned te = (unsigned)(i * KB + c);
+    const unsigned tb = te * (unsigned)sizeof(C2<T>), wb = te * 16u;
     double2 q;
     if (MODE == BX_INTERIOR) {
-      const C2<T> t = bx_load(q_in + idx);
+      const C2<T> t = XT ? bx_load(bx_at(qt_in, tb)) : bx_load(q_in + idx);
+      q = make_double2((double)t.x, (double)t.y);
+    } else if (XT && MODE == BX_LAST) {
+      const C2<T> t = *bx_at(qt_in, tb);
       q = make_double2((double)t.x, (double)t.y);
     } else q = ld2<T>(q_in, idx);
+    double2 w2 = make_double2(0., 0.);
+    if (XT && MODE == BX_INTERIOR) w2 = bx_load(bx_at(wt, wb));
     if (MODE == BX_FIRST) {
       if (g_in) {
         double2 p = ld2<T>(p_in, idx);
         const double2 g0 = ld2<T>(g_in, idx);
         p.x -= half_eps * g0.x;
         p.y -= half_eps * g0.y;
-        st2<T>(p_out, idx, p.x, p.y);
+        if (XT) {
+          C2<T> t;
+          t.x = (T)p.x;
+          t.y = (T)p.y;
+          *bx_at(pt_out, tb) = t;
+        } else st2<T>(p_out, idx, p.x, p.y);
         if (wM) {
-          const double w = wM[idx];
+          const double w = XT ? bx_at(wt, wb)->y : wM[idx];
           q.x += eps * (w * p.x);
           q.y += eps * (w * p.y);
         }
-        st2<T>(q_out, idx, q.x, q.y);
+        if (XT) {
+          C2<T> t;
+          t.x = (T)q.x;
+          t.y = (T)q.y;
+          *bx_at(qt_out, tb) = t;
+        } else st2<T>(q_out, idx, q.x, q.y);
       }
     } else {
       double2 gg = make_double2(0., 0.);
@@ -231,7 +263,7 @@
         gg = make_double2(f * hk[m].x, f * hk[m].y);
       }
       if (a != 0.) {
-        const double w = a * bx_load(wS + idx);
+        const double w = a * (XT ? (MODE == BX_INTERIOR ? w2.x : bx_load(&bx_at(wt, wb)->x)) : bx_load(wS + idx));
         gg.x += w * q.x;
         gg.y += w * q.y;
       }
@@ -241,7 +273,11 @@
       if (MODE == BX_LAST) {
         g_out[idx] = gs;
         if (p_out) {
-          const double2 p = ld2<T>(p_in, idx);
+          double2 p;
+          if (XT) {
+            const C2<T> t = *bx_at(pt_in, tb);
+            p = make_double2((double)t.x, (double)t.y);
+          } else p = ld2<T>(p_in, idx);
           C2<T> pe;
           pe.x = (T)(p.x - half_eps * gg.x);
           pe.y = (T)(p.y - half_eps * gg.y);
@@ -251,7 +287,7 @@
         }
         continue;
       }
-      const C2<T> pt = bx_load(p_in + idx);
+      const C2<T> pt = XT ? bx_load(bx_at(pt_in, tb)) : bx_load(p_in + idx);
       double2 p = make_double2((double)pt.x, (double)pt.y);
       C2<T> pe;
       pe.x = (T)(p.x - half_eps * gg.x);
@@ -264,10 +300,11 @@
         C2<T> t;
         t.x = (T)p.x;
         t.y = (T)p.y;
-        bx_store(p_out + idx, t);
+        if (XT) bx_store(bx_at(pt_out, tb), t);
+        else bx_store(p_out + idx, t);
       }
       if (wM) {
-        const double w = bx_load(wM + idx);
+        const double w = XT ? w2.y : bx_load(wM + idx);
         q.x += eps * (w * p.x);
         q.y += eps * (w * p.y);
       }
@@ -275,7 +312,8 @@
         C2<T> t;
         t.x = (T)q.x;
         t.y = (T)q.y;
-        bx_store(q_out + idx, t);
+        if (XT) bx_store(bx_at(qt_out, tb), t);
+        else bx_store(q_out + idx, t);
       }
     }
     qkeep[m].x = (T)q.x;
@@ -426,12 +464,12 @@
   }
 }
 
-template <typename T, int NT, int PER>
+template <typename T, int NT, int PER, bool XT = false>
 __global__ void __launch_bounds__(NT, BCHMC_BX_WAVES)
 k_step_boundary_x2(Geo g, int log2n, const C2<T> *__restrict__ twiddle, C2<T> *Ck, const C2<T> *q_in, const C2<T> *p_in,
                    C2<T> *q_out, C2<T> *p_out, const double *__restrict__ wS, const double *__restrict__ wM, double a,
                    double b, double half_eps, double eps, double c_za, double *guard_slot, StepCtl ctl, bool pair = false,
-                   bool vpair = false) {
+                   bool vpair = false, const double2 *__restrict__ wpair = nullptr) {
   constexpr int KB = 128 / (int)sizeof(C2<T>);
   extern __shared__ __attribute__((aligned(16))) unsigned char s_raw_x2[];
   __shared__ double red[NT / 64];
@@ -473,6 +511,13 @@
     return reinterpret_cast<const double *>(reinterpret_cast<const char *>(base) + off);
   };
   C2<T> *const Ck1 = Ck + g.Nhp, *const Ck2 = Ck + 2 * g.Nhp;
+  const long long tbase = XT ? (long long)bid * n * KB : 0;
+  const C2<T> *const qt_in = q_in + tbase, *const pt_in = p_in + tbase;
+  C2<T> *const qt_out = q_out + tbase, *const pt_out = p_out + tbase;
+  const double2 *const wt = wpair + tbase;
+  unsigned toff[PER];
+#pragma unroll
+  for (int m = 0; m < PER; m++) toff[m] = XT ? (unsigned)(((irow + rows * m) * KB + c) * (int)sizeof(C2<T>)) : boff[m];
   {
     C2<T> vx[PER], vy[PER], vz[PER];
 #pragma unroll
@@ -494,10 +539,15 @@
 #pragma unroll
   for (int m = 0; m < PER; m++) {
     const unsigned woff = sizeof(C2<T>) == 16 ? boff[m] / 2 : boff[m];
-    qv[m] = bx_load(at_c(q_in, boff[m]));
-    pv[m] = bx_load(at_c(p_in, boff[m]));
-    ws[m] = (a != 0.) ? bx_load(at_d(wS, woff)) : 0.;
-    wm[m] = wM ? bx_load(at_d(wM, woff)) : 0.;
+    qv[m] = bx_load(at_c(qt_in, toff[m]));
+    pv[m] = bx_load(at_c(pt_in, toff[m]));
+    if (XT) {
+      const double2 w2 = bx_load(bx_at(wt, sizeof(C2<T>) == 16 ? toff[m] : toff[m] * 2));
+      ws[m] = w2.x, wm[m] = w2.y;
+    } else {
+      ws[m] = (a != 0.) ? bx_load(at_d(wS, woff)) : 0.;
+      wm[m] = wM ? bx_load(at_d(wM, woff)) : 0.;
+    }
   }
   __syncthreads();
   xfft_inplace2<T, false>(sa, sb, tw, n, log2n, KB);
@@ -545,7 +595,7 @@
       C2<T> t;
       t.x = (T)p.x;
       t.y = (T)p.y;
-      bx_store(at_cw(p_out, boff[m]), t);
+      bx_store(at_cw(pt_out, toff[m]), t);
     }
     if (wM) {
       q.x += eps * (wm[m] * p.x);
@@ -554,7 +604,7 @@
     C2<T> qs;
     qs.x = (T)q.x;
     qs.y = (T)q.y;
-    bx_store(at_cw(q_out, boff[m]), qs);
+    bx_store(at_cw(qt_out, toff[m]), qs);
     C2<T> o, o2;
     o.x = o.y = o2.x = o2.y = T(0);
     if (ksq > 1.e-14 && !nyq) {
diff --git a/barcode_amd/csrc/xtile.hpp b/barcode_amd/csrc/xtile.hpp
--- /dev/null
+++ b/barcode_amd/csrc/xtile.hpp
@@ -0,0 +1,82 @@
+#pragma once
+
+#include "eval_plan.hpp"
+
+#ifdef __HIPCC__
+#define BCHMC_XTILE_FN __host__ __device__
+#else
+#define BCHMC_XTILE_FN
+#endif
+
+namespace bchmc {
+
+BCHMC_XTILE_FN constexpr long long xtile_index(int n, int nhp, int kb, int i, int j, int k) {
+  const long long t = (long long)j * (nhp / kb) + k / kb;
+  return (t * n + i) * kb + k % kb;
+}
+BCHMC_XTILE_FN constexpr long long xtile_of(int n, int nhp, int kb, long long idx) {
+  const int k = (int)(idx % nhp);
+  const long long ij = idx / nhp;
+  return xtile_index(n, nhp, kb, (int)(ij / n), (int)(ij % n), k);
+}
+BCHMC_XTILE_FN constexpr long long xtile_inverse(int n, int nhp, int kb, long long e) {
+  const int c = (int)(e % kb);
+  const long long r = e / kb;
+  const int i = (int)(r % n);
+  const long long t = r / n;
+  const int ntk = nhp / kb;
+  const int j = (int)(t / ntk), k = (int)(t % ntk) * kb + c;
+  return ((long long)i * n + j) * nhp + k;
+}
+
+constexpr bool x_tiles(const PathFacts &f, const PathSwitches &s, const TrajPlan &tp) {
+  return !s.no_xtile && planes_at_ends(f, s) && tp.fused && tp.fused_za && !tp.alpt_x && f.mass_fs &&
+         (f.n == 128 || f.n == 256);
+}
+
+enum class XLayout : unsigned char { kNatural, kTiled, kDead };
+
+constexpr bool closing_is_x(Closing c) {
+  return c == Closing::kBxLast || c == Closing::kBxInterior || c == Closing::kBxInteriorTwoTile;
+}
+
+struct XPairs {
+  XLayout q[2] = {XLayout::kNatural, XLayout::kDead}, p[2] = {XLayout::kNatural, XLayout::kDead};
+  int cur = 0;
+
+  constexpr bool open(bool xt, bool opening_is_bx_first) {
+    if (q[0] != XLayout::kNatural || p[0] != XLayout::kNatural) return false;
+    if (xt && !opening_is_bx_first) return false;
+    cur = xt ? 1 : 0;
+    q[cur] = p[cur] = xt ? XLayout::kTiled : XLayout::kNatural;
+    return true;
+  }
+  constexpr int dst(bool xt, bool last) const { return last && !xt ? cur : cur ^ 1; }
+  constexpr bool close(bool xt, Closing c, bool last) {
+    const XLayout want = xt && closing_is_x(c) ? XLayout::kTiled : XLayout::kNatural;
+    if (xt && !closing_is_x(c)) return false;
+    if (q[cur] != want || p[cur] != want) return false;
+    const int d = dst(xt, last);
+    if (last) {
+      p[d] = XLayout::kNatural;
+    } else {
+      q[d] = p[d] = want;
+      cur ^= 1;
+    }
+    return true;
+  }
+  constexpr int result(bool xt) const { return xt ? cur ^ 1 : cur; }
+  constexpr bool finish(bool xt) {
+    const int r = result(xt);
+    if (xt) {
+      if (q[cur] != XLayout::kTiled) return false;
+      q[r] = XLayout::kNatural;
+      q[cur] = p[cur] = XLayout::kDead;
+    } else {
+      q[r ^ 1] = p[r ^ 1] = XLayout::kDead;
+    }
+    return q[r] == XLayout::kNatural && p[r] == XLayout::kNatural;
+  }
+};
+
+}
diff --git a/barcode_amd/csrc/xtile_kernels.hpp b/barcode_amd/csrc/xtile_kernels.hpp
--- /dev/null
+++ b/barcode_amd/csrc/xtile_kernels.hpp
@@ -0,0 +1,56 @@
+#pragma once
+#include "common.hpp"
+#include "xtile.hpp"
+
+namespace bchmc {
+
+__global__ void __launch_bounds__(256)
+k_xtile_weights(Geo g, int kb, const double *__restrict__ wS, const double *__restrict__ wM, double2 *__restrict__ pair) {
+  for (long long e = blockIdx.x * (long long)blockDim.x + threadIdx.x; e < g.Nhp; e += (long long)gridDim.x * blockDim.x) {
+    const long long idx = xtile_inverse(g.n, g.nhp, kb, e);
+    pair[e] = make_double2(wS[idx], wM[idx]);
+  }
+}
+
+template <typename T>
+__global__ void __launch_bounds__(256)
+k_xtile_finish(Geo g, const int *__restrict__ stop, const unsigned long long *__restrict__ steps_done, const C2<T> *q0,
+               const C2<T> *p0, const C2<T> *q1, const C2<T> *p1, int fin, C2<T> *q_dst, C2<T> *sq, C2<T> *sp) {
+  constexpr int KB = 128 / (int)sizeof(C2<T>);
+  const bool stopped = *stop != 0;
+  const unsigned long long s = *steps_done;
+  const bool read_is_0 = stopped ? (s & 1) == 0 : fin == 0;
+  const C2<T> *qr = read_is_0 ? q0 : q1, *pr = read_is_0 ? p0 : p1, *pw = read_is_0 ? p1 : p0;
+  C2<T> *qd = stopped ? sq : q_dst;
+  for (long long i = blockIdx.x * (long long)blockDim.x + threadIdx.x; i < g.Nhp; i += (long long)gridDim.x * blockDim.x) {
+    const long long e = xtile_of(g.n, g.nhp, KB, i);
+    const double2 q = ld2<T>(qr, e);
+    st2<T>(qd, i, q.x, q.y);
+    if (stopped) {
+      const double2 a = ld2<T>(pr, e), b = ld2<T>(pw, e);
+      st2<T>(sp, i, 0.5 * a.x + 0.5 * b.x, 0.5 * a.y + 0.5 * b.y);
+    }
+  }
+}
+template <typename T>
+__global__ void __launch_bounds__(256)
+k_xtile_restore(long long n, const int *__restrict__ stop, const C2<T> *__restrict__ sq, const C2<T> *__restrict__ sp,
+                C2<T> *__restrict__ q_dst, C2<T> *__restrict__ p_dst) {
+  if (!*stop) return;
+  for (long long i = blockIdx.x * (long long)blockDim.x + threadIdx.x; i < n; i += (long long)gridDim.x * blockDim.x) {
+    q_dst[i] = sq[i];
+    p_dst[i] = sp[i];
+  }
+}
+
+template <typename T>
+__global__ void __launch_bounds__(256)
+k_xtile_scale_c(Geo g, const C2<T> *__restrict__ in, C2<T> *__restrict__ out, double s) {
+  constexpr int KB = 128 / (int)sizeof(C2<T>);
+  for (long long i = blockIdx.x * (long long)blockDim.x + threadIdx.x; i < g.Nhp; i += (long long)gridDim.x * blockDim.x) {
+    const double2 v = ld2<T>(in, xtile_of(g.n, g.nhp, KB, i));
+    st2<T>(out, i, v.x * s, v.y * s);
+  }
+}
+
+}
```
